# Lymphatus/caesium-clt

Measured on AMD Instinct MI355X. Metric: megapixels/sec JPEG q=80 1920x1080 batch, higher is better.
Workload: dtype int32

## Files before the change

caesium-clt_amd/binding.py:

```python
import ctypes as C
import os

_HERE = os.path.dirname(os.path.abspath(__file__))
NPHASES = 8
NKERNELS = 36
PHASE_NAMES = ["decode", "pixel", "masks_flags_runs", "stats_tables", "sizes_scan", "pack", "stuff_assemble", "reserved"]


class CCSParameters(C.Structure):
    _fields_ = [("keep_metadata", C.c_bool), ("jpeg_quality", C.c_uint32), ("jpeg_chroma_subsampling", C.c_uint32),
                ("jpeg_progressive", C.c_bool), ("jpeg_optimize", C.c_bool), ("jpeg_preserve_icc", C.c_bool),
                ("png_quality", C.c_uint32), ("png_optimization_level", C.c_uint32), ("png_force_zopfli", C.c_bool),
                ("png_optimize", C.c_bool), ("gif_quality", C.c_uint32), ("webp_quality", C.c_uint32), ("webp_lossless", C.c_bool),
                ("tiff_compression", C.c_uint32), ("tiff_deflate_level", C.c_uint32), ("width", C.c_uint32), ("height", C.c_uint32)]


class CCSResult(C.Structure):
    _fields_ = [("success", C.c_bool), ("code", C.c_uint32), ("error_message", C.c_char_p)]


class CByteArray(C.Structure):
    _fields_ = [("data", C.POINTER(C.c_uint8)), ("length", C.c_size_t)]


class Timing(C.Structure):
    _fields_ = [("total_ms", C.c_float), ("phase_ms", C.c_float * NPHASES), ("kernel_ms", C.c_float * NKERNELS), ("in_bytes", C.c_uint64), ("out_bytes", C.c_uint64),
                ("pixels", C.c_uint64), ("coef_bytes", C.c_uint64), ("n_images", C.c_uint32), ("n_failed", C.c_uint32), ("n_seq_decoded", C.c_uint32), ("n_par_fallback", C.c_uint32), ("n_par_short", C.c_uint32), ("n_prog_decoded", C.c_uint32), ("n_refine_chains", C.c_uint32), ("n_search_extra", C.c_uint32)]


class PngTiming(C.Structure):
    _fields_ = [("total_ms", C.c_float), ("kernel_ms", C.c_float * 16), ("in_bytes", C.c_uint64), ("out_bytes", C.c_uint64), ("pixels", C.c_uint64),
                ("raw_bytes", C.c_uint64), ("n_images", C.c_uint32), ("n_failed", C.c_uint32), ("n_trials", C.c_uint32)]


class CaesiumError(RuntimeError):
    def __init__(self, code, message):
        super().__init__(f"[{code}] {message}")
        self.code = code


def library_path():
    return os.path.join(_HERE, "libcaesium_hip.so")


EXPORTS = ["cs_default_parameters", "cs_compress_in_memory", "cs_compress_to_size_in_memory", "cs_convert_in_memory",
           "cs_batch_compress", "cs_batch_extent", "cs_free_bytes", "cs_free_result", "csh_device_count", "csh_last_error", "csh_kernel_name", "csh_kernel_name_webp", "csh_release_cached_memory", "csh_warmup", "csh_batch_create",
           "csh_batch_run", "csh_batch_fetch", "csh_batch_destroy", "csh_batch_retain_dct", "csh_batch_set_quality", "csh_batch_rerun_encode", "cs_batch_compress_to_size", "csh_batch_geometry", "csh_batch_read_coefs",
           "csp_kernel_name", "csp_batch_create", "csp_batch_create_webp", "csp_batch_create_pixels", "csh_batch_create_pixels", "csh_batch_pixels", "csh_batch_create_from_pixels", "csp_png_to_jpeg", "csp_png_to_lossless_webp", "csp_batch_run", "csp_batch_fetch", "csp_batch_destroy", "csp_batch_geometry", "csp_batch_read_rows", "csp_batch_read_stream",
           "csp_batch_trials", "csp_batch_read_scores", "csp_batch_chunk_bits", "csh_batch_create_webp", "cs_batch_convert",
           "cswd_batch_create", "cswd_batch_run", "cswd_batch_pixels", "cswd_batch_read_pixels", "cswd_batch_alpha", "cswd_batch_read_rgba", "cswd_batch_destroy", "cswd_rgba_join", "cswd_rgba_destroy", "csh_batch_create_webp_from_pixels", "csh_batch_create_from_pixels_rgb", "csl_encode_pixels", "csl_attach_alpha"]


def _declare(L):
    P = C.POINTER
    L.cs_default_parameters.argtypes = [P(CCSParameters)]
    L.cs_default_parameters.restype = None
    L.cs_compress_in_memory.argtypes = [C.c_char_p, C.c_size_t, P(CCSParameters), P(CByteArray)]
    L.cs_compress_in_memory.restype = CCSResult
    L.cs_compress_to_size_in_memory.argtypes = [C.c_char_p, C.c_size_t, P(CCSParameters), C.c_size_t, C.c_bool, P(CByteArray)]
    L.cs_compress_to_size_in_memory.restype = CCSResult
    L.cs_convert_in_memory.argtypes = [C.c_char_p, C.c_size_t, P(CCSParameters), C.c_uint32, P(CByteArray)]
    L.cs_convert_in_memory.restype = CCSResult
    L.cs_batch_compress.argtypes = [P(CByteArray), C.c_size_t, P(CCSParameters), C.c_int, P(CByteArray), P(CCSResult)]
    L.cs_batch_extent.argtypes = [P(CByteArray), C.c_size_t]
    L.cs_batch_extent.restype = C.c_size_t
    L.cs_free_bytes.argtypes = [P(CByteArray)]
    L.cs_free_bytes.restype = None
    L.cs_free_result.argtypes = [P(CCSResult)]
    L.cs_free_result.restype = None
    L.csh_last_error.restype = C.c_char_p
    L.csh_kernel_name.argtypes = [C.c_int]
    L.csh_kernel_name.restype = C.c_char_p
    L.csh_kernel_name_webp.argtypes = [C.c_int]
    L.csh_kernel_name_webp.restype = C.c_char_p
    L.csh_batch_create.argtypes = [P(CByteArray), C.c_size_t, P(CCSParameters), C.c_int, P(C.c_void_p)]
    L.csh_batch_run.argtypes = [C.c_void_p, P(Timing)]
    L.csh_batch_fetch.argtypes = [C.c_void_p, P(CByteArray), P(CCSResult)]
    L.csh_batch_retain_dct.argtypes = [C.c_void_p, C.c_int]
    L.csh_batch_set_quality.argtypes = [C.c_void_p, P(C.c_uint32)]
    L.csh_batch_rerun_encode.argtypes = [C.c_void_p, P(Timing)]
# ... 374 lines not shown
```

caesium-clt_amd/csrc/batch.hpp:

```cpp
#pragma once
#include <array>
#include <chrono>
#include <map>
#include <string>
#include <vector>

#include "../../include/caesium_hip.h"
#include "devmem.hpp"
#include "jpeg_host.hpp"
#include "kernels.h"
#include "webp_kernels.h"

namespace csh {

struct Item {
    int code = 0;
    std::string msg;
    JpegInfo in;
    JpegInfo out;
    int image = -1;
    size_t file_size = 0;
    std::vector<uint8_t> meta_out;
};

// ... 1 lines not shown
    PinnedBytes bits_pool;
    std::vector<DecScan> dscans;
    std::vector<DevHuffSet> hsets;
    std::vector<ParHuffSet> phsets;
    std::vector<char> phset_fits;
    std::vector<ParHuffSet4> phsets4;
    std::vector<std::array<int8_t, 8>> slot4;
    bool use4 = true;
    std::vector<ParScan> pscans;
    std::vector<uint32_t> need_seq_init;
    std::vector<ProgChain> chains;
    std::vector<int> chain_scans;
    std::vector<RefineUnit> refine_units;
    uint32_t refine_hist = 0, refine_pos = 0, refine_max_blocks = 0;
    uint32_t total_sub = 0, max_sub = 0, max_par_blocks = 0, dc_total = 0;

    DevBuf<uint8_t> d_bits, d_clean;
    DevBuf<ParScan> d_pscans;
    DevBuf<uint64_t> d_pstate, d_relax_list[2], d_unstuff_off, d_blk_off, d_dc_off;
    DevBuf<uint32_t> d_unstuff_cnt, d_nblk, d_need_seq, d_need_seq_init, d_relax_cnt, d_scan_pending, d_cut_block, d_claim;
    DevBuf<uint16_t> d_hyp;
    DevBuf<int32_t> d_dcdiff;
    DevBuf<DecScan> d_dscans;
    DevBuf<ProgChain> d_chains;
    DevBuf<int> d_chain_scans;
    DevBuf<uint64_t> d_refine_hist;
    DevBuf<uint32_t> d_refine_pos, d_refine_prog;
    DevBuf<RefineUnit> d_refine_units;
    DevBuf<DevHuffSet> d_hsets;
    DevBuf<ParHuffSet> d_phsets;
    DevBuf<ParHuffSet4> d_phsets4;
};

struct PixelPlan {
    std::vector<PlaneWork> pwork;
    std::vector<ResizeWork> rwork;
    std::vector<ResizeTap> rtaps;
    std::vector<float> rweights;
    uint64_t rgb_bytes = 0, tmp_floats = 0, max_tmp = 0, max_dst = 0;
    uint32_t max_row_in = 0, max_out_w = 0, max_nh = 0;
    uint32_t max_src_px = 0;
    uint64_t plane_bytes = 0, oplane_bytes = 0;
    uint32_t max_quads = 0;
    bool any_layout = false, any_layout_rgb = false;

    DevBuf<uint8_t> d_planes, d_oplanes, d_rgb;
    DevBuf<PlaneWork> d_pwork;
    DevBuf<ResizeWork> d_rwork;
    DevBuf<ResizeTap> d_rtaps;
    DevBuf<float> d_rweights, d_rtmp;
    DevBuf<int16_t> d_dct_raw;
};

struct Stage { uint32_t work0 = 0, nwork = 0, slot0 = 0, nslots = 0, ech0 = 0, nech = 0, table0 = 0, ntables = 0, plan0 = 0, nplans = 0, nzc0 = 0, nnzc = 0, ls0 = 0, nls = 0, ts0 = 0, nts = 0; };
struct SearchImg {
    int cand_work[64]; int ncand;
    int Al_luma = 0, Al_chroma = 0;
    uint64_t best_luma = 0, best_chroma = 0;
    int split_luma = 0, split_chroma = 0;
    bool luma_on = false, chroma_on = false;
};

struct EncodePlan {
    std::vector<EncScan> script;
    std::vector<ScanWork> swork;
    uint32_t nslots = 0, nlist_slots = 0, ntok_slots = 0;
    uint64_t total_corr = 0;
    uint64_t total_units = 0, total_words = 0;
    uint32_t max_units = 0;
    int ntables = 0;
    std::vector<TokPlan> plans;
    std::vector<int> plan_comp, plan_image;
    std::vector<EChunk> echunks;
    uint64_t tok_cap = 0;
    uint32_t tok_scale = 1;
    std::vector<TokRegion> regions;
    std::vector<uint32_t> region_est;
    uint32_t hist_rows = 0;
    std::vector<NzList> nzlists;
    std::vector<NzSet> nzsets;
    std::vector<int> nzset_of;
    std::vector<uint32_t> nzset_built;
    std::vector<int> nzset_comp, nzset_image;
    std::vector<NzChunk> nzchunks;
    std::vector<uint32_t> nz_est, nz_worst;
    uint32_t nz_nrec = 0;
    uint64_t nz_cap = 0;
    bool search = false;
    enum { ST_1 = 0, ST_1B = 1, ST_2 = 2, ST_2B = 3, ST_2C = 4, ST_N = 5 };
    Stage stage[ST_N];
    void stage_begin(Stage &sg) {
        sg.work0 = uint32_t(swork.size()); sg.slot0 = nslots; sg.ech0 = uint32_t(echunks.size()); sg.table0 = uint32_t(ntables); sg.plan0 = uint32_t(plans.size());
        sg.nzc0 = uint32_t(nzchunks.size()); sg.ls0 = nlist_slots; sg.ts0 = ntok_slots;
    }
    void stage_end(Stage &sg) {
        sg.nwork = uint32_t(swork.size()) - sg.work0; sg.nslots = nslots - sg.slot0; sg.nech = uint32_t(echunks.size()) - sg.ech0;
        sg.ntables = uint32_t(ntables) - sg.table0; sg.nplans = uint32_t(plans.size()) - sg.plan0;
        sg.nnzc = uint32_t(nzchunks.size()) - sg.nzc0; sg.nls = nlist_slots - sg.ls0; sg.nts = ntok_slots - sg.ts0;
    }
    std::vector<SearchImg> simg;
    std::vector<uint8_t> work_active;
    uint32_t n_gated_runs = 0;
    std::vector<uint32_t> img_list, img_nlist, h_cost;
    std::map<std::array<int, 5>, int> cand_script;
    std::vector<uint8_t> hdr_pool;
    std::vector<uint32_t> hdr_off;

    DevBuf<uint8_t> d_hdr, d_tail, d_scan_tmp, d_work_active;
    DevBuf<EncScan> d_script;
    DevBuf<ScanWork> d_swork;
    DevBuf<uint32_t> d_slot_work;
    DevBuf<EChunk> d_echunks;
    DevBuf<SlotRec> d_slots;
    DevBuf<TokPlan> d_plans;
    DevBuf<uint64_t> d_corr, d_symbits, d_eobbits, d_tok_off, d_chunk_off, d_scan_raw_off;
    DevBuf<uint32_t> d_tok_cursor;
    DevBuf<TokRegion> d_regions;
    DevBuf<uint16_t> d_eobrun, d_slot_hist;
    DevBuf<uint32_t> d_img_list, d_img_nlist, d_scan_cost, d_slot_raw, d_slot_eobh, d_long_runs, d_long_cnt, d_tokens, d_chunk_ntok, d_chunk_bits, d_raw, d_scan_pad, d_chunk_ff, d_hdr_off;
    DevBuf<DevEncTable> d_tables;
    DevBuf<NzList> d_nzlists;
    DevBuf<NzSet> d_nzsets;
    DevBuf<NzChunk> d_nzchunks;
    DevBuf<uint32_t> d_nz_pool, d_nz_cursor, d_nz_chunk_off, d_nz_chunk_cnt, d_list_slots, d_tok_slots;
};

struct TrellisPlan {
    bool trellis = false, dering = false;
    Stage tstage;
    std::vector<TrellisWork> twork;
    std::vector<TrellisRun> truns;
    uint32_t t_units = 0, t_max_rows = 0;
    std::vector<uint32_t> trows;
    bool t_sort = false;
    bool nz_once = false;

    DevBuf<TrellisWork> d_twork;
    DevBuf<TrellisRun> d_truns;
    DevBuf<uint32_t> d_tqueue, d_trows, d_tperm, d_tspill;
    DevBuf<uint8_t> d_tblk_cnt;
    DevBuf<uint16_t> d_tblk_off;
    DevBuf<uint64_t> d_tlambda, d_tdcbt;
};

struct WebpTail {
    uint32_t webp_mb_bytes = 768;
    std::vector<csw::WebpImg> wimgs;
    uint64_t wwork_bytes = 0, wlevels = 0;
    uint32_t wmax_luma = 0, wmax_mbh = 0;

    DevBuf<csw::WebpImg> d_wimgs;
    DevBuf<uint8_t> d_wwork, d_wscratch, d_wprobs, d_wupdate;
    DevBuf<uint32_t> d_wpart, d_wstats;
    DevBuf<int16_t> d_wlevels;
};

struct Outputs {
    uint64_t raw_bytes_cap = 0, out_cap = 0;
    DevBuf<uint8_t> d_out;
    DevBuf<uint64_t> d_img_off;
    DevBuf<uint32_t> d_img_size, d_img_size_pad, d_status, d_overflow;
    std::vector<uint32_t> h_img_size;
    std::vector<uint64_t> h_img_off;
    std::vector<uint32_t> h_status;
    bool ran = false;
};

}

struct csh_batch {
    int device = 0;
    hipStream_t stream = 0;
    bool have_stream = false;
    CCSParameters params;
    std::vector<csh::Item> items;
    int nimg = 0;
// ... 9 lines not shown
    std::vector<csh::ImgDesc> imgs;
    std::vector<csh::DevQuant> quants;
    uint32_t ntiles = 0, ntiles_in = 0, ntiles_out = 0, max_tiles = 0, max_dummy = 0;
    csh::DevBuf<csh::ImgDesc> d_imgs;
    csh::DevBuf<csh::DevQuant> d_quants;
    csh::DevBuf<int16_t> d_coef;

    csh::DecodePlan dec;
    csh::PixelPlan pix;
    csh::EncodePlan enc;
    csh::TrellisPlan tr;
    csh::WebpTail wp;
    csh::Outputs out;

    ~csh_batch() { if (have_stream) { (void)hipStreamSynchronize(stream); (void)hipStreamDestroy(stream); } }
};

namespace csh {

enum KernelSlot {
    KS_MEMSET_COEF, KS_UNSTUFF, KS_DEC_SPEC, KS_DEC_RELAX0, KS_DEC_RELAX, KS_DEC_WRITE, KS_DC_SCATTER, KS_REFINE_CHAINS, KS_DECODE_PROG_SEQ,
    KS_IDCT_PLANE, KS_RESIZE, KS_XFORM_DIRECT, KS_RESAMPLE_FDCT, KS_FIX_DUMMY, KS_MEMSET_ENC, KS_TRELLIS_STATS, KS_TRELLIS_AC, KS_TRELLIS_DC,
    KS_NZLIST, KS_TOKENS, KS_LIST_STATS, KS_AC_RUNS, KS_GEN_TABLES, KS_CHUNK_SIZES, KS_SCAN_CHUNK_BITS, KS_SCAN_LAYOUT, KS_PACK, KS_LIST_PACK,
    KS_FF_COUNT, KS_SCAN_SEARCH, KS_LAYOUT, KS_SCAN_IMAGES, KS_EMIT, KS_SPARE0, KS_SPARE1, KS_SPARE2, KS_COUNT,
    KS_WEBP_YUV = KS_XFORM_DIRECT, KS_WEBP_ENCODE = KS_RESAMPLE_FDCT, KS_WEBP_ASSEMBLE = KS_FIX_DUMMY
};
struct KernelSlotRow { KernelSlot slot; const char *name; int phase; };
constexpr KernelSlotRow kKernelSlots[] = {
    {KS_MEMSET_COEF, "memset_coef", 0},        {KS_UNSTUFF, "unstuff", 0},                 {KS_DEC_SPEC, "k_dec_spec", 0},
    {KS_DEC_RELAX0, "k_dec_relax0", 0},        {KS_DEC_RELAX, "k_dec_relax1_4", 0},        {KS_DEC_WRITE, "k_dec_write", 0},
    {KS_DC_SCATTER, "k_dc_scatter", 0},        {KS_REFINE_CHAINS, "k_refine_chains", 0},   {KS_DECODE_PROG_SEQ, "k_decode_prog+seq", 0},
    {KS_IDCT_PLANE, "k_idct_plane", 1},        {KS_RESIZE, "resize", 1},                   {KS_XFORM_DIRECT, "k_xform_direct", 1},
    {KS_RESAMPLE_FDCT, "k_resample+k_plane_fdct", 1}, {KS_FIX_DUMMY, "k_fix_dummy", 1},    {KS_MEMSET_ENC, "memset_enc", 2},
    {KS_TRELLIS_STATS, "trellis_stats", 1},    {KS_TRELLIS_AC, "k_trellis_ac", 1},         {KS_TRELLIS_DC, "k_trellis_dc", 1},
    {KS_NZLIST, "k_nzlist", 2},                {KS_TOKENS, "k_tokens", 2},                 {KS_LIST_STATS, "k_list_stats", 2},
    {KS_AC_RUNS, "k_ac_runs", 2},              {KS_GEN_TABLES, "k_gen_tables", 3},         {KS_CHUNK_SIZES, "k_chunk_sizes", 4},
    {KS_SCAN_CHUNK_BITS, "scan_chunk_bits", 4}, {KS_SCAN_LAYOUT, "scan_layout", 4},        {KS_PACK, "k_pack", 5},
    {KS_LIST_PACK, "k_list_pack", 5},          {KS_FF_COUNT, "k_ff_count", 6},             {KS_SCAN_SEARCH, "scan_search_stage2", 7},
    {KS_LAYOUT, "k_layout", 6},                {KS_SCAN_IMAGES, "scan_images", 6},         {KS_EMIT, "k_emit", 6},
    {KS_SPARE0, "", 7},                        {KS_SPARE1, "", 7},                         {KS_SPARE2, "", 7}};
constexpr bool kernel_slots_in_order() {
    for (int i = 0; i < int(sizeof kKernelSlots / sizeof kKernelSlots[0]); i++) if (kKernelSlots[i].slot != i) return false;
    return true;
}
static_assert(sizeof kKernelSlots / sizeof kKernelSlots[0] == CSH_NKERNELS && int(KS_COUNT) == int(CSH_NKERNELS), "one row per csh_timing.kernel_ms slot");
static_assert(kernel_slots_in_order(), "row i of kKernelSlots describes slot i");

struct PlanSwitches {
    std::string profile;
    bool nz_once = true;
    bool tr_sort = true;
    int prog_par = -1;
    bool fused_420 = true;
    static PlanSwitches read();
};

struct Laps {
    const bool trace;
    std::chrono::steady_clock::time_point at = std::chrono::steady_clock::now();
    std::string text;
    Laps();
    void lap(const char *what);
};

struct BatchPlanner {
    csh_batch *const b;
    const CByteArray *const inputs;
    const size_t count;
    const CCSParameters *const p;
    const csp_pixels *const px;
    const PlanSwitches sw;
    const bool progressive;
    uint16_t qout_nat[64];
    int script_base3 = 0, script_base1 = 0;
    std::vector<std::pair<std::vector<uint8_t>, int>> hset_keys;
    std::map<std::vector<uint16_t>, int> quant_index;
    uint64_t plane_off = 64, oplane_off = 0;

    BatchPlanner(csh_batch *b, const CByteArray *inputs, size_t count, const CCSParameters *p, const csp_pixels *px);
    void begin();
    void parse();
    int reserve_pinned();
    int plan_image(size_t n);
    int plan_search_stages();
    int plan_trellis();
    void finish_descriptors();
    int upload(Laps &laps);

private:
    void image_geometry(Item &it, ImgDesc &im);
    int decode_scans(Item &it, ImgDesc &im, const uint8_t *d);
    int huff_set(const JScan &js);
    void place_blocks(ParScan &ps, const JpegInfo &in, const JScan &js, uint32_t units, bool dc_rows, bool subseqs);
    int sequential_split(const Item &it, const ImgDesc &im, const uint8_t *d, int img_index, bool &par_ok);
    bool progressive_plan(const Item &it, const ImgDesc &im, int img_index);
    void plane_work(ImgDesc &im, const JpegInfo &in, const JpegInfo &o, int img_index, bool resized);
    void resize_work(const JpegInfo &in, const JpegInfo &o, int img_index);
    void output_scans(Item &it, ImgDesc &im, int img_index, size_t in_len);
    void frame_header(Item &it);
    template <class Fill> int enc_scan(const std::array<int, 5> &key, Fill fill);
    int cand_index(int comp, int Ss, int Se, int Ah, int Al);
    int dc_scan_index(int ncomp);
    int seq1_index(int comp);
    uint32_t nz_list(int img_index, int comp, int Al, const ImgDesc &im, size_t in_len);
    void add_works(Item &it, ImgDesc &im, int img_index, const std::vector<int> &list, size_t in_len, const JpegInfo &o, bool stats_only = false);
    template <class Make> void add_stage(int sid, Make make);
// ... 14 lines not shown
```

caesium-clt_amd/csrc/batch_plan.cpp:

```cpp
#include <algorithm>
#include <atomic>
#include <cmath>
#include <thread>

#include "batch.hpp"
#include "resize_host.h"

namespace csh {

static void build_dev_huff(const HuffSpec &h, DevHuff &d) {
    memset(&d, 0, sizeof d);
    for (int l = 0; l < 18; l++) d.maxcode[l] = -1;
    if (!h.present) return;
    int code = 0, p = 0;
    for (int l = 1; l <= 16; l++) {
        if (h.bits[l]) {
            d.valptr[l] = p - code;
            for (int i = 0; i < h.bits[l]; i++, p++, code++)
                if (l <= 9) {
                    int base = code << (9 - l);
                    for (int k = 0; k < (1 << (9 - l)); k++) d.look[(base + k) & 511] = uint16_t((l << 8) | h.vals[p]);
                }
            d.maxcode[l] = code - 1;
        }
// ... 139 lines not shown
    if (lossless) {
        for (int c = 0; c < in.ncomp; c++) o.comp[c] = in.comp[c];
        jpeg_geometry(o);
        return 0;
    }
    int ss = int(p.jpeg_chroma_subsampling);
    if (ss == 0) ss = 420;
    for (int c = 0; c < in.ncomp; c++) { o.comp[c].id = c + 1; o.comp[c].h = o.comp[c].v = 1; o.comp[c].tq = c ? 1 : 0; }
    if (in.ncomp == 3) {
        int blocks = 0;
        for (int c = 0; c < 3; c++) {
            const JComp &k = in.comp[c];
            blocks += k.h * k.v;
            if (in.hmax % k.h || in.vmax % k.v) { it.msg = "fractional chroma sampling ratio (component factors do not divide the largest ones)"; return CS_ERR_JPEG_FEATURE; }
            if (in.hmax / k.h > 4 || in.vmax / k.v > 4) { it.msg = "chroma sampling ratio above 4"; return CS_ERR_JPEG_FEATURE; }
        }
        if (blocks > 10) { it.msg = "more than 10 blocks per MCU"; return CS_ERR_JPEG_FEATURE; }
        if (ss == 420) { o.comp[0].h = 2; o.comp[0].v = 2; }
        else if (ss == 422) { o.comp[0].h = 2; o.comp[0].v = 1; }
        else if (ss == 411) { o.comp[0].h = 4; o.comp[0].v = 1; }
        else if (ss != 444) { it.msg = "unknown output chroma subsampling"; return CS_ERR_JPEG_FEATURE; }
    }
    jpeg_geometry(o);
    return 0;
}

void layout_token_pool(csh_batch *b) {
    b->enc.regions.resize(b->enc.region_est.size());
    if (b->test_pool_shift < 0) b->test_pool_shift = getenv("CSH_TEST_POOL_SHIFT") ? std::min(16, std::max(0, atoi(getenv("CSH_TEST_POOL_SHIFT")))) : 0;
    const int shift = b->test_pool_shift;
    uint64_t at = 0;
    for (size_t i = 0; i < b->enc.regions.size(); i++) {
        const uint64_t cap = std::min<uint64_t>(std::max<uint64_t>((uint64_t(b->enc.region_est[i]) * b->enc.tok_scale) >> shift, 64), 0xFFFFFFF0ull);
        b->enc.regions[i].base = at; b->enc.regions[i].cap = uint32_t(cap); b->enc.regions[i].pad = 0;
        at += (cap + 3) & ~uint64_t(3);
    }
    b->enc.tok_cap = at + 64;
    at = 0;
    for (size_t i = 0; i < b->enc.nzlists.size(); i++) {
        const uint64_t cap = std::min<uint64_t>(std::max<uint64_t>((uint64_t(b->enc.nz_est[i]) * b->enc.tok_scale) >> shift, 64), b->enc.nz_worst[i]);
        b->enc.nzlists[i].base = at; b->enc.nzlists[i].cap = uint32_t(cap);
        at += (cap + 3) & ~uint64_t(3);
    }
    b->enc.nz_cap = at + 64;
}

PlanSwitches PlanSwitches::read() {
    auto is = [](const char *name, const char *v) { const char *e = getenv(name); return e && !strcmp(e, v); };
    PlanSwitches s;
    const char *penv = getenv("CSH_PROFILE");
    s.profile = penv && *penv ? penv : "mozjpeg";
    s.nz_once = !is("CSH_NZ_ONCE", "0");
    s.tr_sort = !is("CSH_TR_SORT", "0");
    const char *pp = getenv("CSH_PROG_PAR");
    s.prog_par = pp && !strcmp(pp, "0") ? 0 : (pp && !strcmp(pp, "1") ? 1 : -1);
    s.fused_420 = !getenv("CSH_NO_FUSED_420");
    return s;
}

Laps::Laps() : trace(getenv("CSH_TRACE") != nullptr) {}
void Laps::lap(const char *what) {
    if (!trace) return;
    const auto now = std::chrono::steady_clock::now();
    char buf[64];
    snprintf(buf, sizeof buf, " %s %.1f", what, std::chrono::duration<double, std::milli>(now - at).count());
    text += buf; at = now;
}

BatchPlanner::BatchPlanner(csh_batch *b_, const CByteArray *inputs_, size_t count_, const CCSParameters *p_, const csp_pixels *px_)
    : b(b_), inputs(inputs_), count(count_), p(p_), px(px_), sw(PlanSwitches::read()), progressive(p_->jpeg_progressive) {}

void BatchPlanner::begin() {
    b->items.resize(count);
    quality_table(int(p->jpeg_quality), qout_nat);
    DevQuant qo; make_quant(qout_nat, qo);
    b->quants.push_back(qo);
    b->q_base = int(b->quants.size()) - 1;
    for (int q = 1; q <= 100; q++) { uint16_t tq[64]; quality_table(q, tq); DevQuant dq; make_quant(tq, dq); b->quants.push_back(dq); }
    b->progressive = progressive;

    add_script(b->enc.script, 3, true);
    add_script(b->enc.script, 1, true);
    add_script(b->enc.script, 3, false);
    add_script(b->enc.script, 1, false);
    script_base3 = progressive ? 0 : 16; script_base1 = progressive ? 10 : 17;
    const bool webp = b->webp, rgb_out = b->rgb_out;
    const std::string &profile = sw.profile;
    b->enc.search = progressive && !webp && !rgb_out && profile != "plain";
    const bool lossy_jpeg = !b->lossless && !webp && !rgb_out;
    b->tr.trellis = lossy_jpeg && (profile == "mozjpeg" || profile == "mozjpeg-trellis");
    b->tr.dering = lossy_jpeg && (profile == "mozjpeg" || profile == "mozjpeg-dering");
    b->tr.nz_once = b->tr.trellis && progressive && sw.nz_once && sw.tr_sort;
}

template <class Fill>
int BatchPlanner::enc_scan(const std::array<int, 5> &key, Fill fill) {
    auto f = b->enc.cand_script.find(key);
    if (f != b->enc.cand_script.end()) return f->second;
    EncScan e;
    memset(&e, 0, sizeof e);
    fill(e);
    b->enc.script.push_back(e);
    return b->enc.cand_script[key] = int(b->enc.script.size()) - 1;
}
int BatchPlanner::cand_index(int comp, int Ss, int Se, int Ah, int Al) {
    return enc_scan({comp, Ss, Se, Ah, Al}, [&](EncScan &e) {
// ... 379 lines not shown
bool BatchPlanner::progressive_plan(const Item &it, const ImgDesc &im, int img_index) {
    const JpegInfo &in = it.in;
    bool prog_ok = in.progressive && in.restart_interval == 0;
    for (size_t s = 0; s < in.scans.size(); s++) {
        const JScan &js = in.scans[s];
        if (js.has_marker || js.data_len >= (1u << 28) || !b->dec.phset_fits[b->dec.dscans[im.first_scan + s].huff_set]) prog_ok = false;
    }
    if (!prog_ok) return false;
    const bool par_first = regular_progression(in) && sw.prog_par != 0 && uint64_t(in.mcus_x) * uint64_t(in.mcus_y) * 10 < (1u << 24);
    for (size_t s = 0; s < in.scans.size(); s++) {
        const JScan &js = in.scans[s];
        DecScan &ds = b->dec.dscans[im.first_scan + s];
        ParScan ps;
        memset(&ps, 0, sizeof ps);
        ps.bits_off = ds.bits_off; ps.bits_len = ds.bits_len; ps.huff_set = ds.huff_set; ps.image = img_index; ps.ncomp = ds.ncomp; ps.nb_mcu = 1;
        ps.Ss = js.Ss; ps.Se = js.Se; ps.Al = js.Al;
        ps.kind = !par_first ? CSH_PS_UNSTUFF : js.Ss == 0 ? (js.Ah == 0 ? CSH_PS_DC_FIRST : CSH_PS_DC_REFINE) : (js.Ah == 0 ? CSH_PS_AC_FIRST : CSH_PS_UNSTUFF);
        ps.sub_base = b->dec.total_sub; ps.par_index = uint32_t(b->dec.pscans.size());
        if (ps.kind != CSH_PS_UNSTUFF) place_blocks(ps, in, js, scan_units(in, js), ps.kind == CSH_PS_DC_FIRST, ps.kind != CSH_PS_DC_REFINE);
        ds.par_index = int(b->dec.pscans.size());
        b->dec.pscans.push_back(ps);
    }
    const bool refine_split = par_first && sw.prog_par != 1;
    for (int chain = 0; chain <= in.ncomp; chain++) {
        ProgChain pc;
        memset(&pc, 0, sizeof pc);
        pc.image = img_index; pc.first = int(b->dec.chain_scans.size());
        bool all_refine = chain != 0;
        for (size_t s = 0; s < in.scans.size(); s++) {
            const JScan &js = in.scans[s];
            const bool mine = chain == 0 ? js.Ss == 0 : (js.Ss != 0 && js.comp_idx[0] == chain - 1);
            if (mine && b->dec.pscans[size_t(b->dec.dscans[im.first_scan + s].par_index)].kind == CSH_PS_UNSTUFF) {
                b->dec.chain_scans.push_back(im.first_scan + int(s)); pc.count++;
                if (js.Ah == 0 || js.data_len >= (1u << 27)) all_refine = false;
            }
        }
        if (pc.count && refine_split && all_refine) {
            const JComp &jc = in.comp[chain - 1];
            const uint64_t nblocks = uint64_t(jc.real_bw) * uint64_t(jc.real_bh);
            if (nblocks && uint64_t(b->dec.refine_pos) + nblocks * uint64_t(pc.count) < (1ull << 32)) {
                pc.refine = 1; pc.comp = chain - 1; pc.nblocks = uint32_t(nblocks);
                pc.hist_off = b->dec.refine_hist; pc.pos_off = b->dec.refine_pos;
                b->dec.refine_hist += pc.nblocks; b->dec.refine_pos += pc.nblocks * uint32_t(pc.count);
                b->dec.refine_max_blocks = std::max(b->dec.refine_max_blocks, pc.nblocks);
            }
        }
        if (pc.count) b->dec.chains.push_back(pc);
    }
    return true;
}

void BatchPlanner::plane_work(ImgDesc &im, const JpegInfo &in, const JpegInfo &o, int img_index, bool resized) {
    for (int c = 0; c < in.ncomp; c++) {
        PlaneWork w; w.image = img_index; w.comp = c;
        w.up = resized ? up_desc(1, 1, 0) : up_desc(in.hmax / in.comp[c].h, in.vmax / in.comp[c].v, in.comp[c].comp_w);
        w.dn = dn_kind(o.hmax / o.comp[c].h, o.vmax / o.comp[c].v);
        const int in_kind = (w.up.hx == 1 && w.up.vx == 1) ? 0 : (w.up.hx == 2 && w.up.vx == 2) ? 1 : (w.up.hx == 2 && w.up.vx == 1) ? 2 : -1;
        if (in_kind < 0 || w.dn == CSH_DN_H4V1) w.mode = CSH_MODE_ANY;
        else if (resized) w.mode = 1 + w.dn;
        else w.mode = (in_kind == 0 && w.dn == CSH_DN_FULL) ? 0 : 1 + 3 * in_kind + w.dn;
        if (w.mode == CSH_MODE_ANY) b->pix.any_layout = true;
        const bool fused = w.mode == 5 && !resized && im.in[c].comp_w > 2 && im.in[c].real_bw == im.out[c].real_bw && im.in[c].real_bh == im.out[c].real_bh &&
                           im.in[c].comp_w == im.out[c].comp_w && im.in[c].comp_h == im.out[c].comp_h && sw.fused_420;
        if (fused) w.mode = 10;
        if (w.mode) {
            im.plane_off[c] = plane_off;
            plane_off += uint64_t(im.in[c].real_bw * 8) * uint64_t(im.in[c].real_bh * 8);
            plane_off = (plane_off + 63u) & ~uint64_t(63);
            im.splane_off[c] = im.plane_off[c];
            if (resized) {
                JComp full; full.h = full.v = 1;
                JpegInfo tmpj; tmpj.width = o.width; tmpj.height = o.height; tmpj.ncomp = 1; tmpj.comp[0] = full; jpeg_geometry(tmpj);
                uint32_t dummy = 0; fill_geom(tmpj.comp[0], im.src[c], dummy);
                im.splane_off[c] = plane_off;
                plane_off += uint64_t(im.src[c].real_bw * 8) * uint64_t(im.src[c].real_bh * 8);
                plane_off = (plane_off + 63u) & ~uint64_t(63);
            }
            im.oplane_off[c] = oplane_off;
            const uint64_t osz = fused ? 0 : uint64_t(im.out[c].real_bw) * 8 * uint64_t(im.out[c].real_bh) * 8;
            oplane_off = (oplane_off + osz + 63u) & ~uint64_t(63);
            b->pix.max_quads = std::max(b->pix.max_quads, uint32_t(osz / 4));
        }
        b->pix.pwork.push_back(w);
    }
}

void BatchPlanner::resize_work(const JpegInfo &in, const JpegInfo &o, int img_index) {
    ResizeWork rw;
    memset(&rw, 0, sizeof rw);
    rw.image = img_index; rw.nw = o.width; rw.nh = o.height;
    rw.in_kind = in.ncomp == 1 ? 0 : ((in.comp[1].h == in.hmax && in.comp[1].v == in.vmax) ? 0 : (in.comp[1].v == in.vmax ? 2 : 1));
    for (int c = 0; c < in.ncomp; c++) rw.up[c] = up_desc(in.hmax / in.comp[c].h, in.vmax / in.comp[c].v, in.comp[c].comp_w);
    if (in.ncomp == 3) {
        auto same = [&](int c, int hx, int vx) { return rw.up[c].hx == hx && rw.up[c].vx == vx; };
        const bool legacy = same(0, 1, 1) && rw.up[1].hx == rw.up[2].hx && rw.up[1].vx == rw.up[2].vx &&
                            (same(1, 1, 1) || same(1, 2, 2) || same(1, 2, 1));
        if (!legacy) { rw.in_kind = CSH_RZ_ANY; b->pix.any_layout_rgb = true; }
    }
    if (px) rw.in_kind = -1;
    const uint64_t src_bytes = uint64_t(in.width) * in.height * in.ncomp, dst_bytes = uint64_t(o.width) * o.height * in.ncomp;
    rw.rgb_src_off = b->pix.rgb_bytes; b->pix.rgb_bytes += (src_bytes + 63) & ~uint64_t(63);
    rw.rgb_dst_off = b->pix.rgb_bytes; b->pix.rgb_bytes += (dst_bytes + 63) & ~uint64_t(63);
    const uint64_t tmpn = uint64_t(o.height) * in.width * in.ncomp;
    rw.tmp_off = b->pix.tmp_floats; b->pix.tmp_floats += tmpn;
    const bool same = o.width == in.width && o.height == in.height;
    rw.vtap_base = uint32_t(b->pix.rtaps.size()); csh_lanczos_axis(in.height, o.height, same, b->pix.rtaps, b->pix.rweights);
    rw.htap_base = uint32_t(b->pix.rtaps.size()); csh_lanczos_axis(in.width, o.width, same, b->pix.rtaps, b->pix.rweights);
// ... 164 lines not shown
        if (it.image < 0) continue;
        ImgDesc &im = b->imgs[size_t(it.image)];
        std::vector<int> list;
        for (int c = 0; c < im.ncomp; c++) list.push_back(progressive ? cand_index(c, 1, 63, 0, 0) : seq1_index(c));
        const size_t first = b->enc.swork.size();
        add_works(it, im, it.image, list, inputs[n].length, it.out, true);
        for (int c = 0; c < im.ncomp; c++) {
            const ScanWork &w = b->enc.swork[first + size_t(c)];
            TrellisWork tw;
            memset(&tw, 0, sizeof tw);
            tw.image = it.image; tw.comp = c;
            tw.table_ac = w.table_base + (progressive ? 0u : 1u);
            tw.table_dc = progressive ? -1 : int32_t(w.table_base);
            tw.nunits = w.nunits; tw.unit_base = b->tr.t_units;
            b->tr.t_units += w.nunits;
            b->tr.t_max_rows = std::max<uint32_t>(b->tr.t_max_rows, uint32_t((im.out[c].real_bh + im.out[c].v - 1) / im.out[c].v));
            tw.nzset = 0xFFFFFFFFu;
            if (progressive) {
                const int si = b->enc.nzset_of[size_t(it.image) * CSH_MAX_COMPS + size_t(c)];
                b->enc.nzsets[size_t(si)].cnt_base = tw.unit_base;
                if (b->tr.nz_once) tw.nzset = uint32_t(si);
            }
            b->tr.twork.push_back(tw);
        }
    }
    b->enc.stage_end(tg);
    {
        std::vector<uint32_t> nch(b->tr.twork.size());
        uint32_t most = 0;
        for (size_t wi = 0; wi < b->tr.twork.size(); wi++) { nch[wi] = (b->tr.twork[wi].nunits + CSH_TR_WG - 1) / CSH_TR_WG; most = std::max(most, nch[wi]); }
        for (uint32_t j = 0; j < most; j += CSH_TR_RUN)
            for (size_t wi = 0; wi < b->tr.twork.size(); wi++)
                if (j < nch[wi]) b->tr.truns.push_back(TrellisRun{uint32_t(wi), j, std::min<uint32_t>(CSH_TR_RUN, nch[wi] - j)});
    }
    {
        b->tr.t_sort = progressive && sw.tr_sort;
        std::vector<std::pair<uint32_t, uint32_t>> rows;
        for (size_t wi = 0; wi < b->tr.twork.size(); wi++) {
            const CompGeom &g = b->imgs[size_t(b->tr.twork[wi].image)].out[b->tr.twork[wi].comp];
            for (int r = 0; r < (g.real_bh + g.v - 1) / g.v; r++) rows.push_back({uint32_t(g.real_bw * g.v), uint32_t(wi << 16) | uint32_t(r)});
        }
        std::stable_sort(rows.begin(), rows.end(), [](const auto &a, const auto &b2) { return a.first > b2.first; });
        for (const auto &r : rows) b->tr.trows.push_back(r.second);
    }
    if (b->enc.total_units > 0xFFFFFFF0ull) { csh_set_error("csh_batch_create: batch too large (fewer files per batch)"); return CS_ERR_POOL_OVERFLOW; }
    return 0;
}

void BatchPlanner::finish_descriptors() {
    if (!b->lossless)
        for (ImgDesc &im : b->imgs) for (int c = 0; c < im.ncomp; c++) im.out[c].tile_base += b->ntiles_in;
    for (size_t i = 0; i < b->enc.plans.size(); i++) b->enc.plans[i].tile_base = b->imgs[size_t(b->enc.plan_image[i])].out[b->enc.plan_comp[i]].tile_base;
    for (size_t i = 0; i < b->enc.nzsets.size(); i++) b->enc.nzsets[i].tile_base = b->imgs[size_t(b->enc.nzset_image[i])].out[b->enc.nzset_comp[i]].tile_base;
    for (ParScan &ps : b->dec.pscans)
        for (int m = 0; m < ps.nb_mcu && m < 10; m++) {
            int dcs = ps.dct[m] & 3, acs = 4 + (ps.act[m] & 3);
            if (b->dec.use4) { dcs = std::max<int>(0, b->dec.slot4[ps.huff_set][dcs]); acs = std::max<int>(0, b->dec.slot4[ps.huff_set][acs]); }
            ps.sel |= uint64_t(dcs | (acs << 3)) << (6 * m);
        }
    {
        std::vector<int> last(b->dec.chains.size(), -1);
        for (int s = 0;; s++) {
            bool any = false;
            for (size_t c = 0; c < b->dec.chains.size(); c++)
                if (b->dec.chains[c].refine && b->dec.chains[c].count > s) {
                    RefineUnit u; u.chain = int(c); u.s = s; u.prev = last[c];
                    last[c] = int(b->dec.refine_units.size());
                    b->dec.refine_units.push_back(u);
                    any = true;
                }
            if (!any) break;
        }
    }
    b->ntiles = b->ntiles_in + b->ntiles_out;
    b->pix.plane_bytes = plane_off;
    b->pix.oplane_bytes = oplane_off;
    b->out.out_cap = b->out.raw_bytes_cap;
    layout_token_pool(b);
}

int BatchPlanner::upload(Laps &laps) {
    hipStream_t st = b->stream;
    if (!b->nimg) return 0;
    b->dec.bits_pool.flush_copies();
    laps.lap("copy_in");
    if (b->dec.d_bits.alloc(b->dec.bits_pool.size()) || (b->dec.bits_pool.size() && hipMemcpyAsync(b->dec.d_bits.p, b->dec.bits_pool.p, b->dec.bits_pool.size(), hipMemcpyHostToDevice, st) != hipSuccess) ||
        b->d_imgs.upload(b->imgs, st) || b->dec.d_dscans.upload(b->dec.dscans, st) || b->dec.d_chains.upload(b->dec.chains, st) || b->dec.d_chain_scans.upload(b->dec.chain_scans, st) ||
        b->dec.d_hsets.upload(b->dec.hsets, st) || b->dec.d_phsets.upload(b->dec.phsets, st) || (b->dec.use4 && b->dec.d_phsets4.upload(b->dec.phsets4, st)) || b->d_quants.upload(b->quants, st) || b->pix.d_pwork.upload(b->pix.pwork, st) ||
        b->enc.d_script.upload(b->enc.script, st) || b->enc.d_swork.upload(b->enc.swork, st) || b->enc.d_slot_work.alloc(size_t(b->enc.nslots) + 1) || b->enc.d_slots.alloc(size_t(b->enc.nslots) + 1) || b->enc.d_plans.upload(b->enc.plans, st) || b->enc.d_echunks.upload(b->enc.echunks, st) || b->enc.d_hdr.upload(b->enc.hdr_pool, st) ||
        b->enc.d_hdr_off.upload(b->enc.hdr_off, st) || b->dec.d_pscans.upload(b->dec.pscans, st) || b->pix.d_rwork.upload(b->pix.rwork, st) || b->pix.d_rtaps.upload(b->pix.rtaps, st) ||
        b->pix.d_rweights.upload(b->pix.rweights, st) || b->pix.d_rgb.alloc(b->pix.rgb_bytes + 64) || b->pix.d_rtmp.alloc((resize_is_fused(b->pix.max_row_in) ? 0 : b->pix.tmp_floats) + 16) || b->dec.d_need_seq_init.upload(b->dec.need_seq_init, st))
        return CS_ERR_NO_DEVICE;
    size_t nchunks = b->dec.bits_pool.size() / 64 + 1, nst = size_t(b->dec.total_sub) + b->dec.pscans.size() + 1;
    if (b->dec.d_clean.alloc(b->dec.bits_pool.size() + 64) || b->dec.d_unstuff_cnt.alloc(nchunks + 1) || b->dec.d_unstuff_off.alloc(nchunks + 2) ||
        b->dec.d_pstate.alloc(nst) || b->dec.d_relax_list[0].alloc(nst) || b->dec.d_relax_list[1].alloc(nst) || b->dec.d_relax_cnt.alloc(512) || b->dec.d_scan_pending.alloc(b->dec.pscans.size() + 1) || b->dec.d_cut_block.alloc(b->dec.pscans.size() + 1) || b->dec.d_claim.alloc(size_t(b->dec.total_sub) + 1) || b->dec.d_hyp.alloc((size_t(b->dec.total_sub) + 1) * 10) ||
        b->dec.d_nblk.alloc(size_t(b->dec.total_sub) + 1) || b->dec.d_blk_off.alloc(size_t(b->dec.total_sub) + 2) || b->dec.d_need_seq.alloc(b->nimg + 1) ||
        b->dec.d_dcdiff.alloc(size_t(b->dec.dc_total) + 1) || b->dec.d_dc_off.alloc(size_t(b->dec.dc_total) + 2) ||
        b->dec.d_refine_hist.alloc(size_t(b->dec.refine_hist) + 1) || b->dec.d_refine_pos.alloc(size_t(b->dec.refine_pos) + 1) || b->dec.d_refine_units.upload(b->dec.refine_units, st) ||
        b->dec.d_refine_prog.alloc(b->dec.refine_units.size() + 1))
        return CS_ERR_NO_DEVICE;
    if (b->d_coef.alloc(size_t(b->ntiles) * CSH_TILE_I16) || b->pix.d_planes.alloc(b->pix.plane_bytes + 64) || b->pix.d_oplanes.alloc(b->pix.oplane_bytes + 64) ||
        b->enc.d_symbits.alloc(b->enc.total_words + 1) || b->enc.d_eobbits.alloc(b->enc.total_words + 1) ||
        b->enc.d_long_runs.alloc(2 * (b->enc.total_units / 512 + b->enc.swork.size() + 16)) || b->enc.d_long_cnt.alloc(4) || b->enc.d_tail.alloc(b->enc.total_units + 1) || b->enc.d_eobrun.alloc(b->enc.total_units + 1) || b->enc.d_corr.alloc(b->enc.total_corr + 1) ||
        b->enc.d_tok_off.alloc(4 * size_t(b->enc.nslots) + 4) || b->enc.d_chunk_ntok.alloc(4 * size_t(b->enc.nslots) + 4) || b->enc.d_slot_hist.alloc(size_t(b->enc.hist_rows) * 256 + 256) ||
        b->enc.d_slot_raw.alloc(size_t(b->enc.nslots) + 1) || b->enc.d_img_list.upload(b->enc.img_list, st) || b->enc.d_img_nlist.upload(b->enc.img_nlist, st) || b->enc.d_scan_cost.alloc(b->enc.swork.size() + 1) || b->enc.d_slot_eobh.alloc(16 * size_t(b->enc.nslots) + 16) || b->enc.d_chunk_bits.alloc(size_t(b->enc.nslots) + 1) || b->enc.d_chunk_off.alloc(size_t(b->enc.nslots) + 2) || b->enc.d_tok_cursor.alloc(b->enc.region_est.size() + 1) || b->enc.d_regions.upload(b->enc.regions, st) ||
        b->enc.d_tables.alloc(b->enc.ntables) || b->enc.d_scan_pad.alloc(b->enc.swork.size() + 1) ||
        b->enc.d_nzlists.upload(b->enc.nzlists, st) || b->enc.d_nzsets.upload(b->enc.nzsets, st) || b->enc.d_nzchunks.upload(b->enc.nzchunks, st) || b->enc.d_list_slots.alloc(size_t(b->enc.nlist_slots) + 1) || b->enc.d_tok_slots.alloc(size_t(b->enc.ntok_slots) + 1) ||
        b->enc.d_nz_cursor.alloc(b->enc.nzlists.size() + 1) || b->enc.d_nz_chunk_off.alloc(size_t(b->enc.nz_nrec) + 1) || b->enc.d_nz_chunk_cnt.alloc(size_t(b->enc.nz_nrec) + 1) ||
        b->enc.d_scan_raw_off.alloc(b->enc.swork.size() + 2) || b->out.d_img_size.alloc(b->nimg + 1) || b->out.d_img_size_pad.alloc(b->nimg + 1) ||
        b->out.d_img_off.alloc(b->nimg + 2) || b->out.d_status.alloc(b->nimg) || b->out.d_overflow.alloc(4))
        return CS_ERR_NO_DEVICE;
    if (hipMemsetAsync(b->enc.d_slots.p, 0, (size_t(b->enc.nslots) + 1) * sizeof(SlotRec), st) != hipSuccess ||
        hipMemsetAsync(b->enc.d_slot_work.p, 0, (size_t(b->enc.nslots) + 1) * sizeof(uint32_t), st) != hipSuccess) { csh_set_error("hipMemsetAsync failed"); return CS_ERR_NO_DEVICE; }
    launch_make_slots(st, b->enc.d_swork.p, uint32_t(b->enc.swork.size()), b->enc.d_script.p, b->enc.d_nzlists.p, b->enc.d_slots.p, b->enc.d_slot_work.p, b->enc.d_list_slots.p, b->enc.d_tok_slots.p);
    if (b->tr.trellis && (b->tr.d_trows.upload(b->tr.trows, st) || (b->tr.t_sort && (b->tr.d_tperm.alloc(size_t(b->tr.t_units) + 1) || b->tr.d_tblk_cnt.alloc(size_t(b->tr.t_units) + 1) || (b->tr.nz_once && b->tr.d_tblk_off.alloc(size_t(b->tr.t_units) + 1)))))) return CS_ERR_NO_DEVICE;
    if (b->tr.trellis && (b->tr.d_twork.upload(b->tr.twork, st) || b->tr.d_truns.upload(b->tr.truns, st) || b->tr.d_tqueue.alloc(1) || b->tr.d_tlambda.alloc(size_t(b->tr.t_units) + 1) || b->tr.d_tdcbt.alloc(size_t(b->tr.t_units) + 1) ||
                       b->tr.d_tspill.alloc(trellis_spill_words(trellis_ac_slots())) || b->pix.d_dct_raw.alloc(size_t(b->ntiles_out) * CSH_TILE_I16)))
        return CS_ERR_NO_DEVICE;
    for (size_t n = 0; px && n < count; n++) {
        const Item &it = b->items[n];
        if (it.image < 0) continue;
        const ResizeWork &rw = b->pix.rwork[size_t(it.image)];
        if (rw.image != it.image) { csh_set_error("internal: resize work out of order"); return CS_ERR_NO_DEVICE; }
        if (hipMemcpyAsync(b->pix.d_rgb.p + rw.rgb_src_off, px[n].device_pixels, size_t(px[n].width) * px[n].height * px[n].channels, hipMemcpyDeviceToDevice, st) != hipSuccess) { csh_set_error("pixel copy failed"); return CS_ERR_NO_DEVICE; }
    }
    laps.lap("alloc+enqueue");
    if (hipStreamSynchronize(st) != hipSuccess) { csh_set_error("upload failed"); return CS_ERR_NO_DEVICE; }
    laps.lap("upload_wait");
    return 0;
}

}
```

caesium-clt_amd/csrc/batch_run.cpp:

```cpp
#include <algorithm>

#include "batch.hpp"

namespace csh {
namespace {

class KernelMarks {
    hipEvent_t ev[CSH_NKERNELS + 1];
    int created = 0, next = 0;
    const hipStream_t st;

public:
    explicit KernelMarks(hipStream_t s) : st(s) {}
    KernelMarks(const KernelMarks &) = delete;
    KernelMarks &operator=(const KernelMarks &) = delete;
    ~KernelMarks() { for (int i = 0; i < created; i++) (void)hipEventDestroy(ev[i]); }
    int start() {
        for (; created <= CSH_NKERNELS; created++) CSH_CHECK(hipEventCreate(&ev[created]));
        CSH_CHECK(hipEventRecord(ev[0], st));
        return 0;
    }
    int claim(KernelSlot slot, hipEvent_t *e) {
        if (int(slot) != next || next >= CSH_NKERNELS) {
            csh_set_error("internal: timing mark '%s' out of order (slot %d is next)", slot < KS_COUNT ? kKernelSlots[slot].name : "?", next);
            return -1;
        }
        *e = ev[++next];
        return 0;
    }
    int mark(KernelSlot slot) {
        hipEvent_t e;
        if (claim(slot, &e)) return -1;
        CSH_CHECK(hipEventRecord(e, st));
        return 0;
    }
    int skip_to(KernelSlot slot) {
        while (next < int(slot)) if (mark(KernelSlot(next))) return -1;
        return int(slot) == next ? 0 : mark(slot);
    }
    int read(csh_timing *t, bool phases) const {
        if (phases) {
            for (int i = 0; i < CSH_NPHASES; i++) t->phase_ms[i] = 0;
            for (int i = 0; i < CSH_NKERNELS; i++) t->kernel_ms[i] = 0;
        }
        for (int i = 0; i < next; i++) {
            CSH_CHECK(hipEventElapsedTime(&t->kernel_ms[i], ev[i], ev[i + 1]));
            if (phases) t->phase_ms[kKernelSlots[i].phase] += t->kernel_ms[i];
        }
        CSH_CHECK(hipEventElapsedTime(&t->total_ms, ev[0], ev[next]));
        return 0;
    }
};
#define MARK(slot) do { if (marks.mark(slot)) return -1; } while (0)

struct Run {
    csh_batch *const b;
    csh_timing *const t;
    const hipStream_t st;
    const int nimg;
    KernelMarks marks;
    uint64_t raw_chunks = 0;
    bool eobrun_cleared = false;
    EncCtx c;
    AsmCtx a;

    Run(csh_batch *b_, csh_timing *t_) : b(b_), t(t_), st(b_->stream), nimg(b_->nimg), marks(b_->stream) {}

    int pools() {
        raw_chunks = (b->out.raw_bytes_cap + 63) / 64;
        if (b->enc.d_raw.n != raw_chunks * 16) {
            if (b->enc.d_raw.alloc(raw_chunks * 16) || b->enc.d_chunk_ff.alloc(raw_chunks + 1) || b->out.d_out.alloc(b->out.out_cap + 64))
                return -1;
            const uint64_t longest = std::max({uint64_t(size_t(b->enc.nslots)), uint64_t(b->enc.swork.size()), uint64_t(b->dec.dc_total), uint64_t(b->dec.total_sub), uint64_t(b->dec.bits_pool.size() / 64), uint64_t(nimg)});
            size_t tmp = exclusive_scan_tmp_bytes(longest + 1);
            if (b->enc.d_scan_tmp.alloc(tmp)) return -1;
        }
        if (b->enc.d_tokens.n < b->enc.tok_cap && b->enc.d_tokens.alloc(b->enc.tok_cap)) return -1;
        if (b->enc.d_nz_pool.n < b->enc.nz_cap && b->enc.d_nz_pool.alloc(b->enc.nz_cap)) return -1;
        return 0;
    }

    int requant() {
        if (b->out.d_status.zero(st) || b->out.d_overflow.zero(st)) return -1;
        launch_requant(st, b->d_imgs.p, b->pix.d_pwork.p, int(b->pix.pwork.size()), b->max_tiles, b->d_quants.p, b->pix.d_dct_raw.p, b->ntiles_in, b->d_coef.p);
        launch_fix_dummy(st, b->d_imgs.p, nimg, b->max_dummy, b->d_coef.p);
        return marks.skip_to(KS_MEMSET_ENC);
    }
    int skip_decode() {
        if (b->out.d_status.zero(st) || b->out.d_overflow.zero(st)) return -1;
        return marks.skip_to(KS_IDCT_PLANE);
    }

    int decode() {
        const bool zero_in_spec = !b->dec.pscans.empty() && b->dec.max_sub != 0;
        if (!zero_in_spec) CSH_CHECK(hipMemsetAsync(b->d_coef.p, 0, size_t(b->ntiles_in) * CSH_TILE_I16 * sizeof(int16_t), st));
        if (b->out.d_status.zero(st) || b->out.d_overflow.zero(st)) return -1;
        CSH_CHECK(hipMemcpyAsync(b->dec.d_need_seq.p, b->dec.d_need_seq_init.p, size_t(nimg) * sizeof(uint32_t), hipMemcpyDeviceToDevice, st));
        MARK(KS_MEMSET_COEF);
        {
            int nps = int(b->dec.pscans.size());
            uint32_t nchunks = uint32_t(b->dec.bits_pool.size() / 64);
            if (nps) {
                launch_unstuff_count(st, b->dec.d_bits.p, b->dec.d_pscans.p, nps, nchunks, b->dec.d_unstuff_cnt.p);
                launch_exclusive_scan(st, b->dec.d_unstuff_cnt.p, b->dec.d_unstuff_off.p, nchunks, b->enc.d_scan_tmp.p, b->enc.d_scan_tmp.n);
                launch_unstuff_copy(st, b->dec.d_bits.p, b->dec.d_clean.p, b->dec.d_pscans.p, nps, nchunks, b->dec.d_unstuff_off.p);
            }
            MARK(KS_UNSTUFF);
            DenseArgs da;
            memset(&da, 0, sizeof da);
            da.clean = b->dec.d_clean.p; da.pss = b->dec.d_pscans.p; da.huffs = b->dec.use4 ? static_cast<const void *>(b->dec.d_phsets4.p) : static_cast<const void *>(b->dec.d_phsets.p); da.compact = b->dec.use4 ? 1 : 0; da.state = b->dec.d_pstate.p; da.nblk = b->dec.d_nblk.p;
            da.list_out = b->dec.d_relax_list[0].p; da.cnt_out = b->dec.d_relax_cnt.p; da.blk_off = b->dec.d_blk_off.p; da.imgs = b->d_imgs.p;
            da.coef = b->d_coef.p; da.dcdiff = b->dec.d_dcdiff.p; da.need_seq = b->dec.d_need_seq.p; da.cut_block = b->dec.d_cut_block.p;
            CSH_CHECK(hipMemsetAsync(b->dec.d_cut_block.p, 0xFF, b->dec.d_cut_block.n * sizeof(uint32_t), st));
            const uint64_t zero_all = uint64_t(b->ntiles_in) * CSH_TILE_I16 * sizeof(int16_t), zero_half = (zero_all / 2) & ~uint64_t(15);
            const uint64_t eob_all = (uint64_t(b->enc.d_eobrun.n) * sizeof(uint16_t)) & ~uint64_t(15), eob_half = (eob_all / 2) & ~uint64_t(15);
// ... 11 lines not shown
            }
            launch_dec_dense(st, 1, nps, b->dec.max_sub, da);
            da.zero_bytes = 0; da.zero2_bytes = 0;
            MARK(KS_DEC_RELAX0);
            const int kMaxRounds = int(b->dec.d_relax_cnt.n) - 2;
            int R = 0;
            for (int group = 12; nps && R < kMaxRounds; group = 8) {
                for (int g = 0; g < group && R < kMaxRounds; g++, R++)
                    launch_dec_relax_list(st, b->dec.d_clean.p, b->dec.d_pscans.p, b->dec.total_sub, da.huffs, da.compact, b->dec.d_pstate.p, b->dec.d_nblk.p, b->dec.d_relax_list[R & 1].p,
                                          b->dec.d_relax_cnt.p + R, b->dec.d_relax_list[(R & 1) ^ 1].p, b->dec.d_relax_cnt.p + R + 1, b->dec.d_pstate.n, b->dec.d_claim.p, uint32_t(R + 1));
                uint32_t left = 0;
                CSH_CHECK(hipMemcpyAsync(&left, b->dec.d_relax_cnt.p + R, sizeof left, hipMemcpyDeviceToHost, st));
                CSH_CHECK(hipStreamSynchronize(st));
                if (!left) break;
            }
            if (nps) {
                if (b->dec.d_scan_pending.zero(st)) return -1;
                launch_dec_mark_pending(st, b->dec.d_pscans.p, b->dec.total_sub, b->dec.d_relax_list[R & 1].p, b->dec.d_relax_cnt.p + R, b->dec.d_scan_pending.p);
                da.hyp = b->dec.d_hyp.p; da.scan_pending = b->dec.d_scan_pending.p;
                launch_dec_dense(st, 3, nps, b->dec.max_sub, da);
                launch_dec_chain(st, b->dec.d_pscans.p, nps, b->dec.d_pstate.p, b->dec.d_nblk.p, b->dec.d_hyp.p, b->dec.d_scan_pending.p, b->dec.d_need_seq.p);
            }
            MARK(KS_DEC_RELAX);
            if (nps) launch_exclusive_scan(st, b->dec.d_nblk.p, b->dec.d_blk_off.p, b->dec.total_sub, b->enc.d_scan_tmp.p, b->enc.d_scan_tmp.n);
            launch_dec_dense(st, 2, nps, b->dec.max_sub, da);
            MARK(KS_DEC_WRITE);
            if (nps) launch_exclusive_scan(st, reinterpret_cast<uint32_t *>(b->dec.d_dcdiff.p), b->dec.d_dc_off.p, b->dec.dc_total, b->enc.d_scan_tmp.p, b->enc.d_scan_tmp.n);
            launch_dc_scatter(st, b->dec.d_pscans.p, nps, b->dec.max_par_blocks, b->d_imgs.p, b->dec.d_dc_off.p, b->d_coef.p, b->dec.d_need_seq.p, b->dec.d_cut_block.p);
            launch_dc_refine(st, b->dec.d_clean.p, b->dec.d_pscans.p, nps, b->dec.max_par_blocks, b->d_imgs.p, b->d_coef.p, b->dec.d_need_seq.p);
            MARK(KS_DC_SCATTER);
        }
        launch_refine_chains(st, b->dec.d_clean.p, b->dec.d_pscans.p, b->dec.d_phsets.p, b->dec.d_dscans.p, b->dec.d_chains.p, b->dec.d_chain_scans.p, int(b->dec.chains.size()), b->dec.d_refine_units.p,
                             int(b->dec.refine_units.size()), b->dec.refine_max_blocks, b->d_imgs.p, b->d_coef.p, b->dec.d_need_seq.p, b->dec.d_refine_hist.p, b->dec.d_refine_pos.p, b->dec.d_refine_prog.p);
        MARK(KS_REFINE_CHAINS);
        launch_decode_prog(st, b->dec.d_clean.p, b->dec.d_pscans.p, b->dec.d_phsets.p, b->dec.d_dscans.p, b->dec.d_chains.p, b->dec.d_chain_scans.p, int(b->dec.chains.size()), b->d_imgs.p,
                           b->d_coef.p, b->dec.d_need_seq.p);
        launch_decode_seq(st, b->dec.d_bits.p, b->d_imgs.p, b->dec.d_dscans.p, b->dec.d_hsets.p, b->d_coef.p, nimg, b->dec.d_need_seq.p);
        MARK(KS_DECODE_PROG_SEQ);
        return 0;
    }

    int planes() {
        int nw = b->lossless ? 0 : int(b->pix.pwork.size());
        launch_idct_plane(st, b->d_imgs.p, b->pix.d_pwork.p, nw, b->max_tiles, b->d_quants.p, b->d_coef.p, b->pix.d_planes.p);
        MARK(KS_IDCT_PLANE);
        launch_resize(st, b->d_imgs.p, b->pix.d_rwork.p, int(b->pix.rwork.size()), b->pix.d_rtaps.p, b->pix.d_rweights.p, b->pix.d_planes.p, b->pix.d_rgb.p, b->pix.d_rtmp.p,
                      b->pix.max_src_px, b->pix.max_tmp, b->pix.max_dst, b->pix.max_row_in, b->pix.max_out_w, b->pix.max_nh, !(b->webp || b->rgb_out), b->pix.any_layout_rgb);
        MARK(KS_RESIZE);
        return 0;
    }
    int pixels() {
        const int nw = b->lossless ? 0 : int(b->pix.pwork.size());
        int16_t *rawp = ((b->retain_dct || b->tr.trellis) && !b->lossless) ? b->pix.d_dct_raw.p : nullptr;
        launch_xform_direct(st, b->d_imgs.p, b->pix.d_pwork.p, nw, b->max_tiles, b->d_quants.p, b->d_coef.p, b->d_coef.p, rawp, b->ntiles_in, b->tr.dering);
        MARK(KS_XFORM_DIRECT);
        launch_resample_plane(st, b->d_imgs.p, b->pix.d_pwork.p, nw, b->pix.max_quads, b->pix.d_planes.p, b->pix.d_oplanes.p);
        if (b->pix.any_layout) launch_resample_any(st, b->d_imgs.p, b->pix.d_pwork.p, nw, b->pix.max_quads, b->pix.d_planes.p, b->pix.d_oplanes.p);
        launch_plane_fdct(st, b->d_imgs.p, b->pix.d_pwork.p, nw, b->max_tiles, b->d_quants.p, b->pix.d_oplanes.p, b->d_coef.p, rawp, b->ntiles_in, b->tr.dering);
        launch_resample_fdct_420(st, b->d_imgs.p, b->pix.d_pwork.p, nw, b->max_tiles, b->d_quants.p, b->pix.d_planes.p, b->d_coef.p, rawp, b->ntiles_in, b->tr.dering);
        MARK(KS_RESAMPLE_FDCT);
        if (!b->lossless) launch_fix_dummy(st, b->d_imgs.p, nimg, b->max_dummy, b->d_coef.p);
        MARK(KS_FIX_DUMMY);
        return 0;
    }

    void fill_enc_ctx() {
        memset(&c, 0, sizeof c);
        c.imgs = b->d_imgs.p; c.script = b->enc.d_script.p; c.work = b->enc.d_swork.p; c.nwork = int(b->enc.swork.size());
        c.echunks = b->enc.d_echunks.p; c.plans = b->enc.d_plans.p; c.nechunks = uint32_t(b->enc.echunks.size()); c.slot_work = b->enc.d_slot_work.p; c.slots = b->enc.d_slots.p; c.nslots = b->enc.nslots;
        c.coef = b->d_coef.p; c.sym_bits = b->enc.d_symbits.p; c.eob_bits = b->enc.d_eobbits.p; c.tail = b->enc.d_tail.p;
        c.eobrun = b->enc.d_eobrun.p; c.long_runs = b->enc.d_long_runs.p; c.long_cnt = b->enc.d_long_cnt.p; c.corr = b->enc.d_corr.p;
        c.tokens = b->enc.d_tokens.p; c.regions = b->enc.d_regions.p; c.tok_cursor = b->enc.d_tok_cursor.p; c.tok_off = b->enc.d_tok_off.p; c.chunk_ntok = b->enc.d_chunk_ntok.p; c.slot_hist = b->enc.d_slot_hist.p; c.slot_raw = b->enc.d_slot_raw.p; c.slot_eobh = b->enc.d_slot_eobh.p;
        c.chunk_bits = b->enc.d_chunk_bits.p; c.chunk_off = b->enc.d_chunk_off.p; c.tables = b->enc.d_tables.p;
        c.raw = b->enc.d_raw.p; c.raw_words = raw_chunks * 16; c.status = b->out.d_status.p; c.overflow = b->out.d_overflow.p;
        c.nzlists = b->enc.d_nzlists.p; c.nzsets = b->enc.d_nzsets.p; c.nz_pool = b->enc.d_nz_pool.p; c.nz_cursor = b->enc.d_nz_cursor.p; c.nz_chunk_off = b->enc.d_nz_chunk_off.p; c.nz_chunk_cnt = b->enc.d_nz_chunk_cnt.p;
        c.debug = getenv("CSH_DEBUG") ? uint32_t(atoi(getenv("CSH_DEBUG"))) : 0u;
    }
    void fill_asm_ctx() {
        memset(&a, 0, sizeof a);
        a.imgs = b->d_imgs.p; a.script = b->enc.d_script.p; a.work = b->enc.d_swork.p; a.nimg = nimg;
        a.nwork = b->tr.trellis ? int(b->tr.tstage.work0) : c.nwork;
        a.tables = b->enc.d_tables.p; a.chunk_off = b->enc.d_chunk_off.p; a.scan_pad_bytes = b->enc.d_scan_pad.p; a.scan_raw_off = b->enc.d_scan_raw_off.p;
        a.raw = b->enc.d_raw.p; a.raw_chunks = raw_chunks; a.chunk_ff = b->enc.d_chunk_ff.p;
        a.hdr_pool = b->enc.d_hdr.p; a.hdr_off = b->enc.d_hdr_off.p; a.img_size = b->out.d_img_size.p; a.img_size_pad = b->out.d_img_size_pad.p;
        a.img_off = b->out.d_img_off.p; a.out = b->out.d_out.p; a.out_cap = b->out.out_cap; a.status = b->out.d_status.p; a.overflow = b->out.d_overflow.p;
        a.img_list = b->enc.d_img_list.p; a.img_nlist = b->enc.d_img_nlist.p; a.scan_cost = b->enc.d_scan_cost.p;
    }
    void fill_trellis_ctx(TrellisCtx &tc) {
        memset(&tc, 0, sizeof tc);
        tc.imgs = b->d_imgs.p; tc.quant = b->d_quants.p; tc.work = b->tr.d_twork.p; tc.nwork = int(b->tr.twork.size()); tc.runs = b->tr.d_truns.p; tc.nruns = uint32_t(b->tr.truns.size());
        tc.tables = b->enc.d_tables.p; tc.raw = b->pix.d_dct_raw.p; tc.raw_tile0 = b->ntiles_in; tc.coef = b->d_coef.p; tc.dcrec = b->tr.d_tlambda.p; tc.dcbt = b->tr.d_tdcbt.p;
        tc.spill = b->tr.d_tspill.p; tc.nslots = uint32_t(b->tr.d_tspill.n / trellis_spill_words(1)); tc.max_rows = b->tr.t_max_rows;
        tc.queue = b->tr.d_tqueue.p;
        tc.rows = b->tr.d_trows.p; tc.nrows = uint32_t(b->tr.trows.size());
        if (b->tr.t_sort) { tc.blk_cnt = b->tr.d_tblk_cnt.p; tc.perm = b->tr.d_tperm.p; }
        if (b->tr.t_sort && b->tr.nz_once) {
            tc.nz_pool = b->enc.d_nz_pool.p; tc.nzlists = b->enc.d_nzlists.p; tc.nzsets = b->enc.d_nzsets.p; tc.nz_chunk_off = b->enc.d_nz_chunk_off.p; tc.nz_chunk_cnt = b->enc.d_nz_chunk_cnt.p;
            tc.blk_off = b->tr.d_tblk_off.p;
        }
        tc.debug = getenv("CSH_TR_DEBUG") ? uint32_t(atoi(getenv("CSH_TR_DEBUG"))) : 0u;
    }

    int encode_begin() {
        fill_enc_ctx();
        launch_reset_works(st, b->enc.d_swork.p, c.nwork);
        if (b->enc.d_nz_cursor.zero(st) || b->enc.d_nz_chunk_cnt.zero(st)) return -1;
        if (b->enc.d_symbits.zero(st) || b->enc.d_eobbits.zero(st) || (!eobrun_cleared && b->enc.d_eobrun.zero(st)) || b->enc.d_tables.zero(st) || b->enc.d_tok_cursor.zero(st) || b->enc.d_slot_eobh.zero(st) || b->enc.d_scan_pad.zero(st)) return -1;
#ifdef CSH_EMUL
        if (b->enc.d_raw.zero(st)) return -1;
#else
        if ((c.debug & 8192u) && b->enc.d_raw.zero(st)) return -1;
#endif
        MARK(KS_MEMSET_ENC);
        return 0;
    }

    void set_stage(const Stage &sg) {
        c.echunks = b->enc.d_echunks.p + sg.ech0; c.nechunks = sg.nech; c.slot0 = sg.slot0; c.nslots = sg.nslots;
        c.nzchunks = b->enc.d_nzchunks.p + sg.nzc0; c.nnzchunks = sg.nnzc;
        c.list_slots = b->enc.d_list_slots.p + sg.ls0; c.nlist_slots = sg.nls; c.tok_slots = b->enc.d_tok_slots.p + sg.ts0; c.ntok_slots = sg.nts;
    }

    int trellis() {
        const Stage &tg = b->tr.tstage;
        set_stage(tg);
        c.stats_only = 1;
        if (b->enc.d_long_cnt.zero(st)) return -1;
        c.nz_blk_cnt = b->tr.t_sort ? b->tr.d_tblk_cnt.p : nullptr;
        c.nz_blk_off = (b->tr.t_sort && b->tr.nz_once) ? b->tr.d_tblk_off.p : nullptr;
        launch_nzlist(st, c);
        c.nz_blk_cnt = nullptr; c.nz_blk_off = nullptr;
        if (b->tr.t_sort) {
            TrellisCtx ts;
            memset(&ts, 0, sizeof ts);
            ts.work = b->tr.d_twork.p; ts.nwork = int(b->tr.twork.size()); ts.blk_cnt = b->tr.d_tblk_cnt.p; ts.perm = b->tr.d_tperm.p;
            launch_trellis_sort(st, ts);
        }
        launch_tokens(st, c);
        launch_list_stats(st, c);
        launch_ac_runs(st, c);
        launch_gen_tables(st, b->enc.d_tables.p + tg.table0, int(tg.ntables));
        c.stats_only = 0;
        if (b->enc.d_nz_cursor.zero(st)) return -1;
        MARK(KS_TRELLIS_STATS);
        TrellisCtx tc;
        fill_trellis_ctx(tc);
        if (b->tr.d_tqueue.zero(st)) return -1;
        launch_trellis_ac(st, tc);
        MARK(KS_TRELLIS_AC);
        launch_trellis_dc(st, tc);
        launch_fix_dummy(st, b->d_imgs.p, nimg, b->max_dummy, b->d_coef.p);
        MARK(KS_TRELLIS_DC);
        return 0;
    }

    int stage(const Stage &sg, bool mark, bool gate) {
#define SMARK(slot) do { if (mark) MARK(slot); } while (0)
        set_stage(sg);
        c.work_active = gate ? b->enc.d_work_active.p : nullptr;
        a.work0 = int(sg.work0); a.nwork_run = int(sg.nwork);
        if (b->enc.d_long_cnt.zero(st)) return -1;
        launch_nzlist(st, c);
        SMARK(KS_NZLIST);
        launch_tokens(st, c);
        SMARK(KS_TOKENS);
        launch_list_stats(st, c);
        SMARK(KS_LIST_STATS);
        launch_ac_runs(st, c);
        SMARK(KS_AC_RUNS);
        launch_gen_tables(st, b->enc.d_tables.p + sg.table0, int(sg.ntables));
        SMARK(KS_GEN_TABLES);
        launch_chunk_sizes(st, c);
// ... 40 lines not shown
        MARK(KS_LAYOUT);
        launch_exclusive_scan(st, b->out.d_img_size_pad.p, b->out.d_img_off.p, uint64_t(nimg), b->enc.d_scan_tmp.p, b->enc.d_scan_tmp.n);
        MARK(KS_SCAN_IMAGES);
        launch_emit(st, a);
        MARK(KS_EMIT);
        return 0;
    }

    int finish(bool phases) {
        CSH_CHECK(hipStreamSynchronize(st));
        CSH_CHECK(hipGetLastError());
        if (t && marks.read(t, phases)) return -1;
        if (t && !phases) t->n_images = uint32_t(nimg);
        return 0;
    }

    int webp() {
        const int nwimg = int(b->wp.wimgs.size());
        uint64_t out_bytes = 0;
        std::vector<uint64_t> off(size_t(b->nimg) + 1, 0);
        for (auto &wi : b->wp.wimgs) {
            const uint64_t cap = 4096 + uint64_t(wi.mbw) * wi.mbh * (b->wp.webp_mb_bytes + 2);
            wi.out_cap = uint32_t(std::min<uint64_t>(cap, 0xFFFFFF00u)); wi.out_off = out_bytes;
            off[wi.image] = out_bytes;
            out_bytes += (wi.out_cap + 63) & ~uint64_t(63);
            const int q = int(b->params.webp_quality);
            wi.quality = q < 0 ? 0 : q > 100 ? 100 : q;
        }
        off[b->nimg] = out_bytes;
        if (b->out.d_out.n < out_bytes + 64 && b->out.d_out.alloc(out_bytes + 64)) return -1;
        if ((b->wp.d_wscratch.n < out_bytes + 64 && b->wp.d_wscratch.alloc(out_bytes + 64)) || (b->wp.d_wpart.n < size_t(b->nimg) * 9 + 9 && b->wp.d_wpart.alloc(size_t(b->nimg) * 9 + 9)) ||
            (b->wp.d_wstats.n < size_t(b->nimg) * 2112 + 8 && (b->wp.d_wstats.alloc(size_t(b->nimg) * 2112 + 8) || b->wp.d_wprobs.alloc(size_t(b->nimg) * 1056 + 8) || b->wp.d_wupdate.alloc(size_t(b->nimg) * 1056 + 8))))
            return -1;
        if (b->wp.d_wstats.zero(st)) return -1;
        if (b->wp.d_wimgs.upload(b->wp.wimgs, st) || (b->wp.d_wwork.n < b->wp.wwork_bytes + 64 && b->wp.d_wwork.alloc(b->wp.wwork_bytes + 64)) ||
            (b->wp.d_wlevels.n < b->wp.wlevels + 64 && b->wp.d_wlevels.alloc(b->wp.wlevels + 64)))
            return -1;
        CSH_CHECK(hipMemcpyAsync(b->out.d_img_off.p, off.data(), off.size() * sizeof(uint64_t), hipMemcpyHostToDevice, st));
        if (b->out.d_img_size.zero(st)) return -1;
        csw::launch_webp_yuv(st, b->wp.d_wimgs.p, nwimg, b->wp.wmax_luma, b->pix.d_rgb.p, b->wp.d_wwork.p);
        MARK(KS_WEBP_YUV);
        hipEvent_t mid;
        if (marks.claim(KS_WEBP_ENCODE, &mid)) return -1;
        if (csw::launch_webp_encode(st, b->wp.wimgs.data(), nwimg, b->wp.d_wimgs.p, b->wp.d_wwork.p, b->wp.d_wlevels.p, b->wp.d_wscratch.p, b->wp.d_wpart.p, b->out.d_out.p, b->out.d_img_size.p, b->out.d_status.p, mid)) return -1;
        MARK(KS_WEBP_ASSEMBLE);
        return finish(false);
    }
};

}

int run_once(csh_batch *b, csh_timing *t, bool requant_only) {
    Run r(b, t);
    if (r.pools() || r.marks.start()) return -1;
    const bool from_pixels = requant_only && b->tr.dering;
    if (requant_only && !from_pixels) {
        if (r.requant()) return -1;
    } else {
        if (from_pixels ? r.skip_decode() : r.decode()) return -1;
        if (r.planes()) return -1;
        if (b->webp) return r.webp();
        if (b->rgb_out) return (r.marks.mark(KS_XFORM_DIRECT) || r.finish(false)) ? -1 : 0;
        if (r.pixels()) return -1;
    }
    if (r.encode_begin()) return -1;
    if (b->tr.trellis ? r.trellis() : r.marks.skip_to(KS_NZLIST)) return -1;
    r.fill_asm_ctx();
    if (r.stage(b->enc.stage[0], true, false)) return -1;
    if (b->enc.search && r.search()) return -1;
    return (r.emit() || r.finish(true)) ? -1 : 0;
}

}
```

caesium-clt_amd/csrc/k_aclist.hip:

```cpp
#include "kernels.h"
#include "wave.h"

namespace csh {

#define CSH_LP_WORDS 1024

__device__ __forceinline__ static uint32_t lbitlen(uint32_t v) { return 32u - uint32_t(__clz(v)); }
__device__ __forceinline__ static int lwave() { return int(threadIdx.x) / CSP_WAVE_THREADS; }

#define CSH_NZ_HALF 16
__device__ __forceinline__ static uint4 nz_load(const EncCtx &c, const NzSet &S, uint32_t u, int bx, int by, uint32_t oct) {
    uint4 q; q.x = q.y = q.z = q.w = 0u;
    if (u < S.nunits) {
        const int b = by * S.bw + bx;
        q = *reinterpret_cast<const uint4 *>(c.coef + (size_t(S.tile_base) + size_t(b >> 6)) * CSH_TILE_I16 + size_t((b & 63) * CSH_BLK_STRIDE) + size_t(oct) * CSH_OCT_STRIDE);
    }
    return q;
}
__device__ __forceinline__ static uint32_t nz_mask8(const uint4 &q, uint32_t oct) {
    uint32_t m = 0;
    m |= (q.x & 0xFFFFu) ? 1u : 0u;   m |= (q.x >> 16) ? 2u : 0u;
    m |= (q.y & 0xFFFFu) ? 4u : 0u;   m |= (q.y >> 16) ? 8u : 0u;
    m |= (q.z & 0xFFFFu) ? 16u : 0u;  m |= (q.z >> 16) ? 32u : 0u;
    m |= (q.w & 0xFFFFu) ? 64u : 0u;  m |= (q.w >> 16) ? 128u : 0u;
// ... 340 lines not shown
                } else if (ev.term) {
                    const uint32_t run = eobrun[ev.blk];
                    if (run) {
                        const uint32_t nb = lbitlen(run) - 1u, t = lut[nb << 4];
                        v[q] = ((t & 0xFFFFu) << nb) | (run & ((1u << nb) - 1u)); n[q] = (t >> 16) + nb;
                    }
                }
                ln += n[q];
            }
            v0[l] = v[0]; v1[l] = v[1]; v2[l] = v[2]; v3[l] = v[3]; n0[l] = n[0]; n1[l] = n[1]; n2[l] = n[2]; n3[l] = n[3]; z[l] = zz; len[l] = ln;
        }
        uint32_t tot;
        const LV<uint32_t> ex = lscan(len, tot);
        LFOR(l) {
            uint64_t at = pos + ex[l] - uint64_t(ww) * 32u;
            const uint32_t v[4] = {v0[l], v1[l], v2[l], v3[l]}, n[4] = {n0[l], n1[l], n2[l], n3[l]};
            CSH_UNROLL
            for (int q = 0; q < 4; q++) {
                for (uint32_t t = (z[l] >> (2 * q)) & 3u; t; t--) { lor_bits(buf, at, zc, zl); at += zl; }
                if (n[q]) { lor_bits(buf, at, v[q], n[q]); at += n[q]; }
            }
        }
        pos += tot;
        const uint32_t done = uint32_t(pos >> 5) - ww;
        if (done > CSH_LP_WORDS - 640) {
            CSP_WAVE_SYNC();
            LFOR(l) for (uint32_t q = uint32_t(l); q < done; q += 64) {
                const uint32_t v = buf[q];
                if (first_flush && q == 0) { if (v) atomicOr(out + ww, v); } else out[ww + q] = v;
            }
            const uint32_t partial = buf[done];
            CSP_WAVE_SYNC();
            LFOR(l) for (int q = l; q < CSH_LP_WORDS; q += 64) buf[q] = (q == 0) ? partial : 0u;
            CSP_WAVE_SYNC();
            ww += done; first_flush = false;
        }
    }
    CSP_WAVE_SYNC();
    const uint32_t last = uint32_t((pos + 31) >> 5) - ww;
    LFOR(l) for (uint32_t q = uint32_t(l); q < last; q += 64) {
        const uint32_t v = buf[q];
        if ((first_flush && q == 0) || q == last - 1) { if (v) atomicOr(out + ww + q, v); } else out[ww + q] = v;
    }
}

__global__ void k_reset_works(ScanWork *work, int nwork) {
    const int j = int(blockIdx.x * blockDim.x + threadIdx.x);
    if (j >= nwork) return;
    work[j].out_off = 0xFFFFFFFFu; work[j].raw_bytes = 0; work[j].hdr_bytes = 0; work[j].ff_bytes = 0; work[j].no_room = 0;
}

void launch_nzlist(hipStream_t st, const EncCtx &c) {
    if (!c.nnzchunks) return;
    CSH_LAUNCH_PHASED(k_nzlist, 3, dim3(c.nnzchunks), dim3(2 * CSP_WAVE_THREADS), st, c);
    CSH_LAUNCH(k_nzfilter, dim3(c.nnzchunks), dim3(CSP_WAVE_THREADS), st, c);
}
void launch_list_stats(hipStream_t st, const EncCtx &c) { if (c.nlist_slots) CSH_LAUNCH(k_list_stats, dim3((c.nlist_slots + 3) / 4), dim3(4 * CSP_WAVE_THREADS), st, c); }
void launch_list_pack(hipStream_t st, const EncCtx &c) { if (c.nlist_slots) CSH_LAUNCH(k_list_pack, dim3((c.nlist_slots + 3) / 4), dim3(4 * CSP_WAVE_THREADS), st, c); }
__global__ void __launch_bounds__(64) k_make_slots(const ScanWork *works, uint32_t nworks, const EncScan *script, const NzList *nzlists, SlotRec *slots, uint32_t *slot_work, uint32_t *list_slots,
                                                   uint32_t *tok_slots) {
    const uint32_t wi = blockIdx.x;
    if (wi >= nworks) return;
    const ScanWork &w = works[wi];
    const EncScan &e = script[w.scan];
    const uint32_t nch = (w.nunits + 255u) / 256u;
    const bool prog_ac = e.Ss > 0 && !e.sequential, listed = w.list != 0xFFFFFFFFu;
    for (uint32_t j = threadIdx.x; j < nch; j += blockDim.x) {
        SlotRec r;
        r.work = wi; r.j = j; r.nch = nch; r.first_chunk = w.first_chunk; r.unit0 = w.unit_base + 256u * j;
        r.nun = w.nunits - 256u * j < 256u ? w.nunits - 256u * j : 256u; r.table_base = w.table_base; r.ntables = uint16_t(e.ntables);
        r.flags = uint16_t((prog_ac ? 1 : 0) | (prog_ac && e.Ah ? 2 : 0) | (listed ? 4 : 0));
        r.hist_row = w.hist_row0 + j * uint32_t(e.ntables);
        r.word_base = w.word_base; r.unit_base = w.unit_base; r.nunits_work = w.nunits;
        r.Ss = uint8_t(e.Ss); r.Se = uint8_t(e.Se); r.Ah = uint8_t(e.Ah); r.Al = uint8_t(e.Al); r.corr0 = w.corr_base == 0xFFFFFFFFu ? 0u : w.corr_base + 256u * j;
        r.nzlist = listed ? w.list : 0u; r.nzrec = listed ? nzlists[w.list].chunk0 + j : 0u;
        slots[w.first_chunk + j] = r;
        slot_work[w.first_chunk + j] = wi;
        (listed ? list_slots : tok_slots)[w.ls_base + j] = w.first_chunk + j;
    }
}
__global__ void __launch_bounds__(64) k_rebind_slots(const ScanWork *works, uint32_t nworks, const NzList *nzlists, SlotRec *slots) {
    const uint32_t wi = blockIdx.x;
    if (wi >= nworks) return;
    const ScanWork &w = works[wi];
    if (w.list == 0xFFFFFFFFu) return;
    const uint32_t nch = (w.nunits + 255u) / 256u, chunk0 = nzlists[w.list].chunk0;
    for (uint32_t j = threadIdx.x; j < nch; j += blockDim.x) { slots[w.first_chunk + j].nzlist = w.list; slots[w.first_chunk + j].nzrec = chunk0 + j; }
}
void launch_rebind_slots(hipStream_t st, const ScanWork *works, uint32_t nworks, const NzList *nzlists, SlotRec *slots) {
    if (nworks) CSH_LAUNCH(k_rebind_slots, dim3(nworks), dim3(64), st, works, nworks, nzlists, slots);
}
void launch_make_slots(hipStream_t st, const ScanWork *works, uint32_t nworks, const EncScan *script, const NzList *nzlists, SlotRec *slots, uint32_t *slot_work, uint32_t *list_slots,
                       uint32_t *tok_slots) {
    if (!nworks) return;
    CSH_LAUNCH(k_make_slots, dim3(nworks), dim3(64), st, works, nworks, script, nzlists, slots, slot_work, list_slots, tok_slots);
}

void launch_reset_works(hipStream_t st, ScanWork *work, int nwork) { if (nwork) CSH_LAUNCH(k_reset_works, dim3((nwork + 255) / 256), dim3(256), st, work, nwork); }

}
```

caesium-clt_amd/csrc/k_pixel.hip:

```cpp
#include <cmath>
#include <utility>

#include "kernels.h"

namespace csh {

static constexpr uint8_t kZ2N[64] = {0,  1,  8,  16, 9,  2,  3,  10, 17, 24, 32, 25, 18, 11, 4,  5,  12, 19, 26, 33, 40, 48,
                                     41, 34, 27, 20, 13, 6,  7,  14, 21, 28, 35, 42, 49, 56, 57, 50, 43, 36, 29, 22, 15, 23,
                                     30, 37, 44, 51, 58, 59, 52, 45, 38, 31, 39, 46, 53, 60, 61, 54, 47, 55, 62, 63};
template <int I>
__device__ __forceinline__ static int half_of(const uint4 &v) {
    uint32_t w = (I / 2 == 0) ? v.x : (I / 2 == 1) ? v.y : (I / 2 == 2) ? v.z : v.w;
    return (I & 1) ? (int(w) >> 16) : (int(w << 16) >> 16);
}
using Oct = std::integer_sequence<int, 0, 1, 2, 3, 4, 5, 6, 7>;
#ifndef CSH_EMUL
typedef uint32_t nt_u32x4 __attribute__((ext_vector_type(4)));
__device__ __forceinline__ static void nt_store16(void *p, const uint4 &v) { nt_u32x4 x; x.x = v.x; x.y = v.y; x.z = v.z; x.w = v.w; __builtin_nontemporal_store(x, reinterpret_cast<nt_u32x4 *>(p)); }
__device__ __forceinline__ static uint4 nt_load16(const void *p) { const nt_u32x4 x = __builtin_nontemporal_load(reinterpret_cast<const nt_u32x4 *>(p)); uint4 v; v.x = x.x; v.y = x.y; v.z = x.z; v.w = x.w; return v; }
#else
__device__ __forceinline__ static void nt_store16(void *p, const uint4 &v) { *reinterpret_cast<uint4 *>(p) = v; }
__device__ __forceinline__ static uint4 nt_load16(const void *p) { return *reinterpret_cast<const uint4 *>(p); }
#endif


#define FIX_0_298 2446
#define FIX_0_390 3196
#define FIX_0_541 4433
#define FIX_0_765 6270
#define FIX_0_899 7373
#define FIX_1_175 9633
#define FIX_1_501 12299
#define FIX_1_847 15137
#define FIX_1_961 16069
#define FIX_2_053 16819
#define FIX_2_562 20995
#define FIX_3_072 25172
#define MUL(a, c) __mul24((a), (c))
#define MAD(a, c, b) (__mul24((a), (c)) + (b))


template <int SH>
__device__ __forceinline__ static void idct1d(int &x0, int &x1, int &x2, int &x3, int &x4, int &x5, int &x6, int &x7) {
    const int R = 1 << (SH - 1);
    const int z1 = MUL(x2 + x6, FIX_0_541), tmp2 = MAD(x6, -FIX_1_847, z1), tmp3 = MAD(x2, FIX_0_765, z1);
    const int tmp0 = ((x0 + x4) << 13) + R, tmp1 = ((x0 - x4) << 13) + R;
    const int t10 = tmp0 + tmp3, t13 = tmp0 - tmp3, t11 = tmp1 + tmp2, t12 = tmp1 - tmp2;
    int a0 = x7, a1 = x5, a2 = x3, a3 = x1;
    const int y1 = a0 + a3, y2 = a1 + a2;
    int y3 = a0 + a2, y4 = a1 + a3;
    const int y5 = MUL(y3 + y4, FIX_1_175);
    y3 = MAD(y3, -FIX_1_961, y5); y4 = MAD(y4, -FIX_0_390, y5);
    const int p1 = MUL(y1, -FIX_0_899), p2 = MUL(y2, -FIX_2_562);
    a0 = MAD(a0, FIX_0_298, p1) + y3; a1 = MAD(a1, FIX_2_053, p2) + y4; a2 = MAD(a2, FIX_3_072, p2) + y3; a3 = MAD(a3, FIX_1_501, p1) + y4;
    x0 = (t10 + a3) >> SH; x7 = (t10 - a3) >> SH;
    x1 = (t11 + a2) >> SH; x6 = (t11 - a2) >> SH;
// ... 28 lines not shown
    return __builtin_amdgcn_perm(hi, lo, 0x05040100u);
#endif
}
__device__ __forceinline__ static uint32_t float_bits(float f) { uint32_t u; __builtin_memcpy(&u, &f, 4); return u; }

template <int J, int... I>
__device__ __forceinline__ static void dequant_octet(int x[64], const uint4 &v, const DevQuant &q, std::integer_sequence<int, I...>) {
    ((x[kZ2N[8 * J + I]] = MUL(half_of<I>(v), int(q.q[8 * J + I]))), ...);
}
template <int... J>
__device__ __forceinline__ static void load_dequant(const int16_t *__restrict__ blk, const DevQuant &q, int x[64], std::integer_sequence<int, J...>) {
    const uint4 v[8] = {nt_load16(blk + CSH_OCT_STRIDE * J)...};
    (dequant_octet<J>(x, v[J], q, Oct()), ...);
}
template <bool CENTRED = false>
__device__ __forceinline__ static void load_idct(const int16_t *__restrict__ blk, const DevQuant &q, int x[64]) {
    load_dequant(blk, q, x, Oct());
    CSH_SCHED_FENCE();
    CSH_UNROLL
    for (int c = 0; c < 8; c++) idct1d<11>(x[c], x[8 + c], x[16 + c], x[24 + c], x[32 + c], x[40 + c], x[48 + c], x[56 + c]);
    CSH_SCHED_FENCE();
    CSH_UNROLL
    for (int r = 0; r < 8; r++) {
        idct1d<18>(x[8 * r], x[8 * r + 1], x[8 * r + 2], x[8 * r + 3], x[8 * r + 4], x[8 * r + 5], x[8 * r + 6], x[8 * r + 7]);
        CSH_UNROLL
        for (int c = 0; c < 8; c++) {
            if (CENTRED) { const int v = x[8 * r + c]; x[8 * r + c] = v < -128 ? -128 : (v > 127 ? 127 : v); }
            else { const int v = x[8 * r + c] + 128; x[8 * r + c] = v < 0 ? 0 : (v > 255 ? 255 : v); }
        }
    }
    CSH_SCHED_FENCE();
}

__device__ __forceinline__ static void replicate_edges(int x[64], int vc, int vr) {
    CSH_UNROLL
    for (int c = 1; c < 8; c++) {
        const bool keep = c < vc;
        CSH_UNROLL
        for (int r = 0; r < 8; r++) x[8 * r + c] = keep ? x[8 * r + c] : x[8 * r + c - 1];
    }
    CSH_UNROLL
    for (int r = 1; r < 8; r++) {
        const bool keep = r < vr;
        CSH_UNROLL
        for (int c = 0; c < 8; c++) x[8 * r + c] = keep ? x[8 * r + c] : x[8 * (r - 1) + c];
    }
}

template <int K>
__device__ __forceinline__ static uint32_t quant_one(const int x[64], const DevQuant &q) {
    return float_bits(__builtin_fmaf(float(x[kZ2N[K]]), q.rcp[K], 12582912.0f));
}
template <int J>
__device__ __forceinline__ static void quant_store_octet(const int x[64], const DevQuant &q, int16_t *__restrict__ blk) {
    uint4 v;
    v.x = pack_halves(quant_one<8 * J + 0>(x, q), quant_one<8 * J + 1>(x, q));
    v.y = pack_halves(quant_one<8 * J + 2>(x, q), quant_one<8 * J + 3>(x, q));
    v.z = pack_halves(quant_one<8 * J + 4>(x, q), quant_one<8 * J + 5>(x, q));
    v.w = pack_halves(quant_one<8 * J + 6>(x, q), quant_one<8 * J + 7>(x, q));
    nt_store16(blk + CSH_OCT_STRIDE * J, v);
}
template <int... J>
__device__ __forceinline__ static void quant_store_all(const int x[64], const DevQuant &q, int16_t *__restrict__ blk, std::integer_sequence<int, J...>) {
    ((quant_store_octet<J>(x, q, blk), CSH_SCHED_FENCE()), ...);
}
template <int J>
__device__ __forceinline__ static void raw_store_octet(const int x[64], int16_t *__restrict__ raw) {
    uint4 v;
    v.x = pack_halves(uint32_t(x[kZ2N[8 * J + 0]]), uint32_t(x[kZ2N[8 * J + 1]]));
    v.y = pack_halves(uint32_t(x[kZ2N[8 * J + 2]]), uint32_t(x[kZ2N[8 * J + 3]]));
    v.z = pack_halves(uint32_t(x[kZ2N[8 * J + 4]]), uint32_t(x[kZ2N[8 * J + 5]]));
    v.w = pack_halves(uint32_t(x[kZ2N[8 * J + 6]]), uint32_t(x[kZ2N[8 * J + 7]]));
    *reinterpret_cast<uint4 *>(raw + CSH_RAW_OCT * J) = v;
}
template <int... J>
__device__ __forceinline__ static void raw_store_all(const int x[64], int16_t *__restrict__ raw, std::integer_sequence<int, J...>) {
    (raw_store_octet<J>(x, raw), ...);
}
#ifdef CSH_EMUL
#define CSH_RAW_VIA_LDS 0
#else
#define CSH_RAW_VIA_LDS 1
#endif
template <int J>
__device__ __forceinline__ static void raw_put_octet(const int x[64], int16_t (*tr)[256], int tid) {
    uint4 v;
    v.x = pack_halves(uint32_t(x[kZ2N[8 * J + 0]]), uint32_t(x[kZ2N[8 * J + 1]]));
    v.y = pack_halves(uint32_t(x[kZ2N[8 * J + 2]]), uint32_t(x[kZ2N[8 * J + 3]]));
    v.z = pack_halves(uint32_t(x[kZ2N[8 * J + 4]]), uint32_t(x[kZ2N[8 * J + 5]]));
    v.w = pack_halves(uint32_t(x[kZ2N[8 * J + 6]]), uint32_t(x[kZ2N[8 * J + 7]]));
    const int l = tid & 63;
    *reinterpret_cast<uint4 *>(&tr[l][(tid & ~63) + 8 * (J ^ (l & 7))]) = v;
}
template <int... J>
__device__ __forceinline__ static void raw_put_all(const int x[64], int16_t (*tr)[256], int tid, std::integer_sequence<int, J...>) {
    (raw_put_octet<J>(x, tr, tid), ...);
}
__device__ __forceinline__ static void raw_copy_out(int16_t *__restrict__ tile_raw, bool has_raw, int16_t (*tr)[256], int tid) {
#if CSH_RAW_VIA_LDS
    const uint64_t mask = __ballot(has_raw);
    if (!mask) return;
    __builtin_amdgcn_fence(__ATOMIC_ACQ_REL, "wavefront");
    __builtin_amdgcn_wave_barrier();
    const int l = tid & 63;
    CSH_UNROLL
    for (int j = 0; j < 8; j++) {
        const int src = 8 * j + (l >> 3);
        if ((mask >> src) & 1ull) {
            const uint4 v = *reinterpret_cast<const uint4 *>(&tr[src][(tid & ~63) + 8 * ((l & 7) ^ (src & 7))]);
            nt_store16(tile_raw + src * 64 + (l & 7) * CSH_RAW_OCT, v);
        }
    }
#else
    (void)tile_raw; (void)has_raw; (void)tr; (void)tid;
#endif
}
#define CSH_DERING_LDS int16_t (*dr_col)[256]
// ... 75 lines not shown
#ifdef CSH_EMUL
    o0 = dot2(P, KE0P, dot2(Q, KE0Q, R0)); o4 = dot2(P, KE4P, dot2(Q, KE4Q, R4));
    o2 = dot2(P, KE2P, dot2(Q, KE2Q, R)); o6 = dot2(P, KE6P, dot2(Q, KE6Q, R));
    o7 = dot2(M, PK(kO7[3], kO7[2]), dot2(N, PK(kO7[1], kO7[0]), R));
    o5 = dot2(M, PK(kO5[3], kO5[2]), dot2(N, PK(kO5[1], kO5[0]), R));
    o3 = dot2(M, PK(kO3[3], kO3[2]), dot2(N, PK(kO3[1], kO3[0]), R));
    o1 = dot2(M, PK(kO1[3], kO1[2]), dot2(N, PK(kO1[1], kO1[0]), R));
#else
    asm("v_dot2_i32_i16 %0, %5, %8, %11\n\tv_dot2_i32_i16 %1, %5, %10, %12\n\tv_dot2_i32_i16 %2, %5, %14, %7\n\tv_dot2_i32_i16 %3, %5, %16, %7\n\t"
        "v_dot2_i32_i16 %0, %4, %6, %0\n\tv_dot2_i32_i16 %1, %4, %9, %1\n\tv_dot2_i32_i16 %2, %4, %13, %2\n\tv_dot2_i32_i16 %3, %4, %15, %3\n\ts_nop 2"
        : "=&v"(o0), "=&v"(o4), "=&v"(o2), "=&v"(o6)
        : "v"(P), "v"(Q), "s"(KE0P), "v"(R), "s"(KE0Q), "s"(KE4P), "s"(KE4Q), "v"(R0), "v"(R4), "s"(KE2P), "s"(KE2Q), "s"(KE6P), "s"(KE6Q));
    asm("v_dot2_i32_i16 %0, %5, %8, %6\n\tv_dot2_i32_i16 %1, %5, %10, %6\n\tv_dot2_i32_i16 %2, %5, %12, %6\n\tv_dot2_i32_i16 %3, %5, %14, %6\n\t"
        "v_dot2_i32_i16 %0, %4, %7, %0\n\tv_dot2_i32_i16 %1, %4, %9, %1\n\tv_dot2_i32_i16 %2, %4, %11, %2\n\tv_dot2_i32_i16 %3, %4, %13, %3\n\ts_nop 2"
        : "=&v"(o7), "=&v"(o5), "=&v"(o3), "=&v"(o1)
        : "v"(M), "v"(N), "v"(R), "s"(PK(kO7[3], kO7[2])), "s"(PK(kO7[1], kO7[0])), "s"(PK(kO5[3], kO5[2])), "s"(PK(kO5[1], kO5[0])),
          "s"(PK(kO3[3], kO3[2])), "s"(PK(kO3[1], kO3[0])), "s"(PK(kO1[3], kO1[2])), "s"(PK(kO1[1], kO1[0])));
#endif
    if (!FIRST) { o0 >>= 2; o4 >>= 2; }
    o2 >>= SH; o6 >>= SH; o7 >>= SH; o5 >>= SH; o3 >>= SH; o1 >>= SH;
}
template <bool CENTRED>
__device__ __forceinline__ static void dering_block_pk(uint32_t pr[8][4], int dc_quant, CSH_DERING_LDS) {
    uint32_t m = pr[0][0];
    CSH_UNROLL
    for (int i = 1; i < 32; i++) m = pk_max(m, pr[i >> 2][i & 3]);
    const int top = CENTRED ? 127 : 255, off = CENTRED ? 0 : 128;
    const bool any = int(int16_t(m)) >= top || int(int16_t(m >> 16)) >= top;
#ifndef CSH_EMUL
    if (!__ballot(any)) return;
#endif
    if (!any) return;
    int x[64];
    CSH_UNROLL
    for (int r = 0; r < 8; r++) {
        const uint32_t A = pr[r][0], B = pr[r][1], C = pr[r][2], D = pr[r][3];
        x[8 * r + 0] = int(int16_t(A)) - off; x[8 * r + 1] = int(int16_t(A >> 16)) - off; x[8 * r + 2] = int(int16_t(C)) - off; x[8 * r + 3] = int(int16_t(C >> 16)) - off;
        x[8 * r + 4] = int(int16_t(D >> 16)) - off; x[8 * r + 5] = int(int16_t(D)) - off; x[8 * r + 6] = int(int16_t(B >> 16)) - off; x[8 * r + 7] = int(int16_t(B)) - off;
    }
    int cnt = 0, sum = 0;
    CSH_UNROLL
    for (int i = 0; i < 64; i++) { sum += x[i]; cnt += x[i] >= 127 ? 1 : 0; }
    if (cnt == 64) return;
    int16_t *col = &dr_col[0][threadIdx.x];
    CSH_UNROLL
    for (int i = 0; i < 64; i++) col[i * 256] = int16_t(x[i]);
    dering_walk(col, dc_quant, cnt, sum);
    CSH_UNROLL
    for (int r = 0; r < 8; r++) {
        auto at = [&](int c) { return uint32_t(int(col[(8 * r + c) * 256]) + off); };
        pr[r][0] = pack_halves(at(0), at(1)); pr[r][1] = pack_halves(at(7), at(6)); pr[r][2] = pack_halves(at(2), at(3)); pr[r][3] = pack_halves(at(5), at(4));
    }
}
template <bool DERING, bool CENTRED>
__device__ __forceinline__ static void fdct_quant_store_pk(uint32_t pr[8][4], const DevQuant &q, int16_t *__restrict__ blk, int16_t *__restrict__ raw, CSH_DERING_LDS) {
    CSH_SCHED_FENCE();
    if (DERING) { dering_block_pk<CENTRED>(pr, int(q.q[0]), dr_col); CSH_SCHED_FENCE(); }
    int x[64];
    int R = 1 << 10, Z = 0;
    CSH_PIN(R); CSH_PIN(Z);
    CSH_UNROLL
    for (int r = 0; r < 8; r++)
        fdct1d_pk<true>(pr[r][0], pr[r][1], pr[r][2], pr[r][3], R, Z, Z, x[8 * r], x[8 * r + 1], x[8 * r + 2], x[8 * r + 3], x[8 * r + 4], x[8 * r + 5], x[8 * r + 6], x[8 * r + 7]);
    CSH_SCHED_FENCE();
    int R2 = 1 << 14, TWO = 2, RDC = 2 - 32768;
    CSH_PIN(R2); CSH_PIN(TWO); CSH_PIN(RDC);
    CSH_UNROLL
    for (int c = 0; c < 8; c++) {
        const uint32_t A = pack_halves(uint32_t(x[c]), uint32_t(x[8 + c])), B = pack_halves(uint32_t(x[56 + c]), uint32_t(x[48 + c]));
        const uint32_t C = pack_halves(uint32_t(x[16 + c]), uint32_t(x[24 + c])), D = pack_halves(uint32_t(x[40 + c]), uint32_t(x[32 + c]));
        fdct1d_pk<false>(A, B, C, D, R2, (c == 0 && !CENTRED) ? RDC : TWO, TWO, x[c], x[8 + c], x[16 + c], x[24 + c], x[32 + c], x[40 + c], x[48 + c], x[56 + c]);
    }
    CSH_SCHED_FENCE();
    if (raw) {
        if (CSH_RAW_VIA_LDS) raw_put_all(x, dr_col, int(threadIdx.x), Oct()); else raw_store_all(x, raw, Oct());
    }
    quant_store_all(x, q, blk, Oct());
}
__device__ __forceinline__ static void pack_rows(const int x[64], uint32_t pr[8][4]) {
    CSH_UNROLL
    for (int r = 0; r < 8; r++) {
        pr[r][0] = pack_halves(uint32_t(x[8 * r]), uint32_t(x[8 * r + 1])); pr[r][1] = pack_halves(uint32_t(x[8 * r + 7]), uint32_t(x[8 * r + 6]));
        pr[r][2] = pack_halves(uint32_t(x[8 * r + 2]), uint32_t(x[8 * r + 3])); pr[r][3] = pack_halves(uint32_t(x[8 * r + 5]), uint32_t(x[8 * r + 4]));
    }
}
template <bool DERING, bool CENTRED = false>
__device__ __forceinline__ static void fdct_quant_store(int x[64], const DevQuant &q, int16_t *__restrict__ blk, int16_t *__restrict__ raw, CSH_DERING_LDS) {
    uint32_t pr[8][4];
    pack_rows(x, pr);
    fdct_quant_store_pk<DERING, CENTRED>(pr, q, blk, raw, dr_col);
}

template <int J, int... I>
__device__ __forceinline__ static void raw_to_nat(int x[64], const uint4 &v, std::integer_sequence<int, I...>) {
    ((x[kZ2N[8 * J + I]] = half_of<I>(v)), ...);
}
template <int... J>
__device__ __forceinline__ static void requant_block(const int16_t *__restrict__ raw, const DevQuant &q, int16_t *__restrict__ blk, std::integer_sequence<int, J...>) {
    const uint4 v[8] = {*reinterpret_cast<const uint4 *>(raw + CSH_RAW_OCT * J)...};
    int x[64];
    (raw_to_nat<J>(x, v[J], Oct()), ...);
    quant_store_all(x, q, blk, Oct());
}

__device__ __forceinline__ static void store_zero_block(int16_t *__restrict__ blk) {
    uint4 z; z.x = z.y = z.z = z.w = 0;
    CSH_UNROLL
    for (int j = 0; j < 8; j++) *reinterpret_cast<uint4 *>(blk + CSH_OCT_STRIDE * j) = z;
}

template <bool DERING>
__global__ void __launch_bounds__(256) k_xform_direct(const ImgDesc *__restrict__ imgs, const PlaneWork *__restrict__ work, const DevQuant *__restrict__ quant,
                                                       const int16_t *__restrict__ coef_in, int16_t *__restrict__ coef_out, int16_t *__restrict__ dct_raw, uint32_t raw_tile0) {
    CSH_SHARED int16_t s_dr[64][256];
    const PlaneWork w = work[blockIdx.y];
    if (w.mode != 0) return;
    const ImgDesc &im = imgs[w.image];
    const CompGeom gi = im.in[w.comp], go = im.out[w.comp];
    int tile = blockIdx.x * (blockDim.x >> 6) + (threadIdx.x >> 6);
    int lane = threadIdx.x & 63;
    int b = tile * 64 + lane;
    bool has_raw = false;
    do {
        if (b >= go.bw * go.bh) break;
        int by = b / go.bw, bx = b - by * go.bw;
        int16_t *dst = coef_out + coef_index(go.tile_base, b, 0);
        if (by >= go.real_bh || bx >= go.real_bw) { store_zero_block(dst); break; }
        int x[64];
        load_idct<true>(coef_in + coef_index(gi.tile_base, by * gi.bw + bx, 0), quant[CSH_UNIFORM(im.qt_in[w.comp])], x);
        int vc = gi.comp_w - bx * 8, vr = gi.comp_h - by * 8;
        if (vc < 8 || vr < 8) replicate_edges(x, vc, vr);
        fdct_quant_store<DERING, true>(x, quant[CSH_UNIFORM(im.qt_out[w.comp])], dst, dct_raw ? dct_raw + raw_index(go.tile_base - raw_tile0, b) : nullptr, s_dr);
        has_raw = dct_raw != nullptr;
    } while (0);
    if (dct_raw) raw_copy_out(dct_raw + raw_index(go.tile_base - raw_tile0, tile * 64), has_raw, s_dr, int(threadIdx.x));
}

__global__ void __launch_bounds__(256) k_idct_plane(const ImgDesc *__restrict__ imgs, const PlaneWork *__restrict__ work, const DevQuant *__restrict__ quant,
                                                     const int16_t *__restrict__ coef_in, uint8_t *__restrict__ planes) {
    const PlaneWork w = work[blockIdx.y];
    if (w.mode == 0) return;
    const ImgDesc &im = imgs[w.image];
    const CompGeom gi = im.in[w.comp];
    int tile = blockIdx.x * (blockDim.x >> 6) + (threadIdx.x >> 6);
    int lane = threadIdx.x & 63;
    int b = tile * 64 + lane;
    if (b >= gi.bw * gi.bh) return;
    int by = b / gi.bw, bx = b - by * gi.bw;
    if (by >= gi.real_bh || bx >= gi.real_bw) return;
    int x[64];
    load_idct(coef_in + coef_index(gi.tile_base, b, 0), quant[CSH_UNIFORM(im.qt_in[w.comp])], x);
    int vc = gi.comp_w - bx * 8, vr = gi.comp_h - by * 8;
    if (vc < 8 || vr < 8) replicate_edges(x, vc, vr);
    int pitch = gi.real_bw * 8;
    uint8_t *p = planes + im.plane_off[w.comp] + size_t(by * 8) * pitch + bx * 8;
    CSH_UNROLL
    for (int r = 0; r < 8; r++) {
        uint32_t lo = uint32_t(x[8 * r]) | (uint32_t(x[8 * r + 1]) << 8) | (uint32_t(x[8 * r + 2]) << 16) | (uint32_t(x[8 * r + 3]) << 24);
        uint32_t hi = uint32_t(x[8 * r + 4]) | (uint32_t(x[8 * r + 5]) << 8) | (uint32_t(x[8 * r + 6]) << 16) | (uint32_t(x[8 * r + 7]) << 24);
        uint2 v; v.x = lo; v.y = hi;
        *reinterpret_cast<uint2 *>(p + size_t(r) * pitch) = v;
    }
}

struct PlaneView { const uint8_t *p; int pitch, cw, ch; };

__device__ __forceinline__ static int pv(const PlaneView &v, int y, int x) {
    y = y < 0 ? 0 : (y > v.ch - 1 ? v.ch - 1 : y);
    x = x < 0 ? 0 : (x > v.cw - 1 ? v.cw - 1 : x);
    return v.p[size_t(y) * v.pitch + x];
}
__device__ static int up_h2v2(const PlaneView &v, int r, int xx) {
    int cy = r >> 1, cx = xx >> 1;
    if (v.cw <= 2) return pv(v, cy, cx);
    int fy = (r & 1) ? cy + 1 : cy - 1;
    int nb = (xx & 1) ? cx + 1 : cx - 1;
    int cs = 3 * pv(v, cy, cx) + pv(v, fy, cx);
    int cn = 3 * pv(v, cy, nb) + pv(v, fy, nb);
    return (3 * cs + cn + ((xx & 1) ? 7 : 8)) >> 4;
}

__device__ static int up_h2v1(const PlaneView &v, int r, int xx) {
    int cx = xx >> 1;
    if (v.cw <= 2) return pv(v, r, cx);
    int nb = (xx & 1) ? cx + 1 : cx - 1;
    return (3 * pv(v, r, cx) + pv(v, r, nb) + ((xx & 1) ? 2 : 1)) >> 2;
}

// ... 135 lines not shown
    const bool last = 2 * x0 + 8 >= v.pitch;
    Quad420 n[2], f[2];
    {
        const uint32_t *rp = reinterpret_cast<const uint32_t *>(v.p + size_t(cy) * v.pitch + 2 * x0);
        const uint32_t a = rp[-1], b = rp[0], c = rp[1], d = last ? c >> 24 : rp[2];
        n[0] = quad420_fields(a, b, c); n[1] = quad420_fields(b, c, d);
    }
    {
        const uint32_t *rp = reinterpret_cast<const uint32_t *>(v.p + size_t(fy) * v.pitch + 2 * x0);
        const uint32_t a = rp[-1], b = rp[0], c = rp[1], d = last ? c >> 24 : rp[2];
        f[0] = quad420_fields(a, b, c); f[1] = quad420_fields(b, c, d);
    }
    const uint32_t M = 0x00FF00FFu;
    uint32_t res[2];
    CSH_UNROLL
    for (int k = 0; k < 2; k++) {
        const uint32_t E = 3u * n[k].E + f[k].E, O = 3u * n[k].O + f[k].O, L = 3u * n[k].L + f[k].L, R = 3u * n[k].R + f[k].R;
        const uint32_t s = ((3u * E + L + 0x00080008u) >> 4 & M) + ((3u * E + O + 0x00070007u) >> 4 & M) +
                           ((3u * O + E + 0x00080008u) >> 4 & M) + ((3u * O + R + 0x00070007u) >> 4 & M);
        res[k] = ((s + 0x00020002u) >> 2) & M;
    }
    return (res[0] & 0xFFu) | ((res[0] >> 8) & 0xFF00u) | ((res[1] & 0xFFu) << 16) | ((res[1] << 8) & 0xFF000000u);
}
__global__ void __launch_bounds__(256) k_resample_any(const ImgDesc *imgs, const PlaneWork *work, const uint8_t *planes, uint8_t *oplanes) {
    const PlaneWork w = work[blockIdx.y];
    if (w.mode != CSH_MODE_ANY) return;
    const ImgDesc &im = imgs[w.image];
    const CompGeom gi = im.src[w.comp], go = im.out[w.comp];
    const int pitch_o = go.real_bw * 8, rows_o = go.real_bh * 8;
    int q = blockIdx.x * blockDim.x + threadIdx.x;
    if (q >= (pitch_o >> 2) * rows_o) return;
    int y = q / (pitch_o >> 2), x0 = (q - y * (pitch_o >> 2)) * 4;
    PlaneView v;
    v.p = planes + im.splane_off[w.comp]; v.pitch = gi.real_bw * 8; v.cw = gi.comp_w; v.ch = gi.comp_h;
    const int W = im.enc_w, H = im.enc_h, och = go.comp_h;
    const UpDesc u = w.up;
    uint32_t out;
    if (u.cls == CSH_UP_H2V2 && w.dn == CSH_DN_H4V1 && x0 >= 4 && 2 * x0 + 8 <= v.pitch && 4 * x0 + 15 <= W - 1) {
        const int ye = y < och - 1 ? y : och - 1;
        out = resample_quad_420_411(v, ye > H - 1 ? H - 1 : ye, x0);
    } else {
        switch (w.dn) {
        case CSH_DN_FULL: out = resample_any_quad<CSH_DN_FULL>(v, u, W, H, och, y, x0); break;
        case CSH_DN_H2V2: out = resample_any_quad<CSH_DN_H2V2>(v, u, W, H, och, y, x0); break;
        case CSH_DN_H2V1: out = resample_any_quad<CSH_DN_H2V1>(v, u, W, H, och, y, x0); break;
        default: out = resample_any_quad<CSH_DN_H4V1>(v, u, W, H, och, y, x0); break;
        }
    }
    *reinterpret_cast<uint32_t *>(oplanes + im.oplane_off[w.comp] + size_t(y) * pitch_o + x0) = out;
}

template <bool DERING>
__global__ void __launch_bounds__(256) k_plane_fdct(const ImgDesc *__restrict__ imgs, const PlaneWork *__restrict__ work, const DevQuant *__restrict__ quant, const uint8_t *__restrict__ oplanes,
                                                     int16_t *__restrict__ coef_out, int16_t *__restrict__ dct_raw, uint32_t raw_tile0) {
    CSH_SHARED int16_t s_dr[64][256];
    const PlaneWork w = work[blockIdx.y];
    if (w.mode == 0 || w.mode == 10) return;
    const ImgDesc &im = imgs[w.image];
    const CompGeom go = im.out[w.comp];
    int tile = blockIdx.x * (blockDim.x >> 6) + (threadIdx.x >> 6);
    int lane = threadIdx.x & 63;
    int b = tile * 64 + lane;
    bool has_raw = false;
    do {
    if (b >= go.bw * go.bh) break;
    int by = b / go.bw, bx = b - by * go.bw;
    int16_t *dst = coef_out + coef_index(go.tile_base, b, 0);
    if (by >= go.real_bh || bx >= go.real_bw) { store_zero_block(dst); break; }
    const int pitch = go.real_bw * 8;
    const uint8_t *p = oplanes + im.oplane_off[w.comp] + size_t(by * 8) * pitch + bx * 8;
    uint32_t pr[8][4];
    CSH_UNROLL
    for (int r = 0; r < 8; r++) {
        const uint2 v = *reinterpret_cast<const uint2 *>(p + size_t(r) * pitch);
        pr[r][0] = bytes_to_halves<0, 1>(v.x); pr[r][2] = bytes_to_halves<2, 3>(v.x); pr[r][1] = bytes_to_halves<3, 2>(v.y); pr[r][3] = bytes_to_halves<1, 0>(v.y);
    }
    fdct_quant_store_pk<DERING, false>(pr, quant[CSH_UNIFORM(im.qt_out[w.comp])], dst, dct_raw ? dct_raw + raw_index(go.tile_base - raw_tile0, b) : nullptr, s_dr);
    has_raw = dct_raw != nullptr;
    } while (0);
    if (dct_raw) raw_copy_out(dct_raw + raw_index(go.tile_base - raw_tile0, tile * 64), has_raw, s_dr, int(threadIdx.x));
}

struct Row16 { uint32_t a, b, c, d; };
__device__ __forceinline__ static Row16 load_row16(const uint8_t *p) {
    Row16 r;
#ifdef CSH_EMUL
    __builtin_memcpy(&r, p, 16);
#else
    typedef uint32_t u32x4_a4 __attribute__((ext_vector_type(4), aligned(4)));
    const u32x4_a4 v = *reinterpret_cast<const u32x4_a4 *>(p);
    r.a = v.x; r.b = v.y; r.c = v.z; r.d = v.w;
#endif
    return r;
}
template <bool DERING>
__global__ void __launch_bounds__(256) k_resample_fdct_420(const ImgDesc *__restrict__ imgs, const PlaneWork *__restrict__ work, const DevQuant *__restrict__ quant, const uint8_t *__restrict__ planes,
                                                            int16_t *__restrict__ coef_out, int16_t *__restrict__ dct_raw, uint32_t raw_tile0) {
    CSH_SHARED int16_t s_dr[64][256];
    const PlaneWork w = work[blockIdx.y];
    if (w.mode != 10) return;
    const ImgDesc &im = imgs[w.image];
    const CompGeom gi = im.src[w.comp], go = im.out[w.comp];
    int tile = blockIdx.x * (blockDim.x >> 6) + (threadIdx.x >> 6);
    int lane = threadIdx.x & 63;
    int b = tile * 64 + lane;
    bool has_raw = false;
    do {
    if (b >= go.bw * go.bh) break;
    int by = b / go.bw, bx = b - by * go.bw;
    int16_t *dst = coef_out + coef_index(go.tile_base, b, 0);
    if (by >= go.real_bh || bx >= go.real_bw) { store_zero_block(dst); break; }
    const int pitch = gi.real_bw * 8, rows_alloc = gi.real_bh * 8;
    const uint8_t *pl = planes + im.splane_off[w.comp];
    const int x0 = bx * 8, y0 = by * 8, W = im.enc_w, H = im.enc_h, och = go.comp_h;
    const bool first = bx == 0, last = x0 + 12 > pitch, hodd = (H & 1) != 0;
    const int kt = ((W - 1) >> 1) - x0;
    uint32_t mA[2], mB[2], mC[2], mD[2];
    const bool wodd = (W & 1) != 0;
    CSH_UNROLL
    for (int q = 0; q < 2; q++) {
        auto even_gone = [&](int k) { return k > kt ? 0xFFFFu : 0u; };
        auto odd_gone = [&](int k) { return (k > kt || (wodd && k == kt)) ? 0xFFFFu : 0u; };
        mA[q] = even_gone(4 * q) | (even_gone(4 * q + 2) << 16);
        mB[q] = odd_gone(4 * q) | (odd_gone(4 * q + 2) << 16);
        mC[q] = even_gone(4 * q + 1) | (even_gone(4 * q + 3) << 16);
        mD[q] = odd_gone(4 * q + 1) | (odd_gone(4 * q + 3) << 16);
    }
    Row16 rows[10];
    CSH_UNROLL
    for (int j = 0; j < 10; j++) {
        int yy = y0 - 1 + j;
        if (hodd && yy == och) yy = och - 2;
        yy = yy < 0 ? 0 : (yy > rows_alloc - 1 ? rows_alloc - 1 : yy);
        rows[j] = load_row16(pl + size_t(yy) * pitch + x0 - 4);
    }
    const bool patch = kt < 8 && ((mA[0] | mB[0] | mC[0] | mD[0] | mA[1] | mB[1] | mC[1] | mD[1]) != 0u);
#ifdef CSH_EMUL
    const bool any_patch = patch;
#else
    const bool any_patch = __ballot(patch) != 0ull;
#endif
    uint32_t pr[8][4];
    Quad420 win[3][2];
    auto row_fields = [&](int j, Quad420 out[2]) {
        const uint32_t bq = rows[j].b, cq = rows[j].c;
        const uint32_t aq = first ? bq << 24 : rows[j].a;
        const uint32_t dq = last ? cq >> 24 : rows[j].d;
        out[0] = quad420_fields(aq, bq, cq);
        out[1] = quad420_fields(bq, cq, dq);
    };
    row_fields(0, win[0]);
    row_fields(1, win[1]);
    CSH_UNROLL
    for (int r = 0; r < 8; r++) {
        Quad420 *p = win[r % 3], *c = win[(r + 1) % 3], *n = win[(r + 2) % 3];
        row_fields(r + 2, n);
        Sums420 s[2] = {quad420_sums(p[0], c[0], n[0]), quad420_sums(p[1], c[1], n[1])};
        if (any_patch && patch) {
            const int odd_col = kt & 1;
            const Sums420 &sq = (kt >> 2) ? s[1] : s[0];
            const uint32_t sqA = (kt >> 2) ? s[1].A : s[0].A, sqB = (kt >> 2) ? s[1].B : s[0].B, sqC = (kt >> 2) ? s[1].C : s[0].C, sqD = (kt >> 2) ? s[1].D : s[0].D;
            (void)sq;
            uint32_t sl = wodd ? (odd_col ? sqC : sqA) : (odd_col ? sqD : sqB);
            sl = (kt & 2) ? sl >> 16 : sl & 0xFFFFu;
            sl |= sl << 16;
            CSH_UNROLL
            for (int qq = 0; qq < 2; qq++) {
                s[qq].A = (s[qq].A & ~mA[qq]) | (sl & mA[qq]);
                s[qq].B = (s[qq].B & ~mB[qq]) | (sl & mB[qq]);
                s[qq].C = (s[qq].C & ~mC[qq]) | (sl & mC[qq]);
                s[qq].D = (s[qq].D & ~mD[qq]) | (sl & mD[qq]);
            }
        }
        uint32_t e0, o0, e1, o1;
        quad420_finish(s[0], e0, o0);
        quad420_finish(s[1], e1, o1);
        pr[r][0] = pack_halves(e0, o0); pr[r][2] = pack_hi_halves(e0, o0); pr[r][1] = pack_hi_halves(o1, e1); pr[r][3] = pack_halves(o1, e1);
    }
    const int ylast = och - 1 - y0;
    if (ylast < 7) {
        CSH_UNROLL
        for (int r = 1; r < 8; r++)
            if (r > ylast) {
                CSH_UNROLL
                for (int cc = 0; cc < 4; cc++) pr[r][cc] = pr[r - 1][cc];
            }
    }
    fdct_quant_store_pk<DERING, false>(pr, quant[CSH_UNIFORM(im.qt_out[w.comp])], dst, dct_raw ? dct_raw + raw_index(go.tile_base - raw_tile0, b) : nullptr, s_dr);
    has_raw = dct_raw != nullptr;
    } while (0);
    if (dct_raw) raw_copy_out(dct_raw + raw_index(go.tile_base - raw_tile0, tile * 64), has_raw, s_dr, int(threadIdx.x));
}

__global__ void __launch_bounds__(256) k_requant(const ImgDesc *__restrict__ imgs, const PlaneWork *__restrict__ work, const DevQuant *__restrict__ quant, const int16_t *__restrict__ dct_raw, uint32_t raw_tile0,
                                                  int16_t *__restrict__ coef_out) {
    const PlaneWork w = work[blockIdx.y];
    const ImgDesc &im = imgs[w.image];
    const CompGeom go = im.out[w.comp];
    int tile = blockIdx.x * (blockDim.x >> 6) + (threadIdx.x >> 6);
    int lane = threadIdx.x & 63;
    int b = tile * 64 + lane;
    if (b >= go.bw * go.bh) return;
    int by = b / go.bw, bx = b - by * go.bw;
    if (by >= go.real_bh || bx >= go.real_bw) return;
    requant_block(dct_raw + raw_index(go.tile_base - raw_tile0, b), quant[CSH_UNIFORM(im.qt_out[w.comp])], coef_out + coef_index(go.tile_base, b, 0), Oct());
}

__global__ void k_fix_dummy(const ImgDesc *imgs, int nimg, int16_t *coef_out) {
    int i = blockIdx.y;
    if (i >= nimg) return;
    const ImgDesc &im = imgs[i];
    int t = blockIdx.x * blockDim.x + threadIdx.x;
    for (int c = 0; c < im.ncomp; c++) {
        const CompGeom &g = im.out[c];
        int ndummy_cols = g.bw - g.real_bw, ndummy_rows = g.bh - g.real_bh;
        int n_right = ndummy_cols * g.real_bh, n_bottom = ndummy_rows * g.bw;
        if (t < n_right) {
            int by = t / ndummy_cols, bx = g.real_bw + t % ndummy_cols;
            coef_out[coef_index(g.tile_base, by * g.bw + bx, 0)] = coef_out[coef_index(g.tile_base, by * g.bw + g.real_bw - 1, 0)];
        } else if (t - n_right < n_bottom) {
            int u = t - n_right;
            int by = g.real_bh + u / g.bw, bx = u % g.bw;
            int sx = (bx / g.h) * g.h + g.h - 1;
            if (sx > g.real_bw - 1) sx = g.real_bw - 1;
            coef_out[coef_index(g.tile_base, by * g.bw + bx, 0)] = coef_out[coef_index(g.tile_base, (g.real_bh - 1) * g.bw + sx, 0)];
        }
    }
}

static dim3 tile_grid(int max_tiles, int nwork) { return dim3((max_tiles + 3) / 4, nwork); }

void launch_xform_direct(hipStream_t st, const ImgDesc *imgs, const PlaneWork *work, int nwork, int max_tiles, const DevQuant *quant,
                         const int16_t *coef_in, int16_t *coef_out, int16_t *dct_raw, uint32_t raw_tile0, bool dering) {
    if (!nwork) return;
    if (dering) CSH_LAUNCH(k_xform_direct<true>, tile_grid(max_tiles, nwork), dim3(256), st, imgs, work, quant, coef_in, coef_out, dct_raw, raw_tile0);
    else CSH_LAUNCH(k_xform_direct<false>, tile_grid(max_tiles, nwork), dim3(256), st, imgs, work, quant, coef_in, coef_out, dct_raw, raw_tile0);
}
void launch_idct_plane(hipStream_t st, const ImgDesc *imgs, const PlaneWork *work, int nwork, int max_tiles, const DevQuant *quant,
                       const int16_t *coef_in, uint8_t *planes) {
    if (nwork) CSH_LAUNCH(k_idct_plane, tile_grid(max_tiles, nwork), dim3(256), st, imgs, work, quant, coef_in, planes);
}
void launch_resample_plane(hipStream_t st, const ImgDesc *imgs, const PlaneWork *work, int nwork, uint32_t max_quads, const uint8_t *planes, uint8_t *oplanes) {
    if (nwork && max_quads) CSH_LAUNCH(k_resample_plane, dim3((max_quads + 255) / 256, nwork), dim3(256), st, imgs, work, planes, oplanes);
}
void launch_resample_any(hipStream_t st, const ImgDesc *imgs, const PlaneWork *work, int nwork, uint32_t max_quads, const uint8_t *planes, uint8_t *oplanes) {
    if (nwork && max_quads) CSH_LAUNCH(k_resample_any, dim3((max_quads + 255) / 256, nwork), dim3(256), st, imgs, work, planes, oplanes);
}
void launch_plane_fdct(hipStream_t st, const ImgDesc *imgs, const PlaneWork *work, int nwork, int max_tiles, const DevQuant *quant,
                       const uint8_t *oplanes, int16_t *coef_out, int16_t *dct_raw, uint32_t raw_tile0, bool dering) {
    if (!nwork) return;
    if (dering) CSH_LAUNCH(k_plane_fdct<true>, tile_grid(max_tiles, nwork), dim3(256), st, imgs, work, quant, oplanes, coef_out, dct_raw, raw_tile0);
    else CSH_LAUNCH(k_plane_fdct<false>, tile_grid(max_tiles, nwork), dim3(256), st, imgs, work, quant, oplanes, coef_out, dct_raw, raw_tile0);
}
void launch_resample_fdct_420(hipStream_t st, const ImgDesc *imgs, const PlaneWork *work, int nwork, int max_tiles, const DevQuant *quant,
                              const uint8_t *planes, int16_t *coef_out, int16_t *dct_raw, uint32_t raw_tile0, bool dering) {
    if (!nwork) return;
    if (dering) CSH_LAUNCH(k_resample_fdct_420<true>, tile_grid(max_tiles, nwork), dim3(256), st, imgs, work, quant, planes, coef_out, dct_raw, raw_tile0);
    else CSH_LAUNCH(k_resample_fdct_420<false>, tile_grid(max_tiles, nwork), dim3(256), st, imgs, work, quant, planes, coef_out, dct_raw, raw_tile0);
}
void launch_requant(hipStream_t st, const ImgDesc *imgs, const PlaneWork *work, int nwork, int max_tiles, const DevQuant *quant, const int16_t *dct_raw,
                    uint32_t raw_tile0, int16_t *coef_out) {
    if (nwork) CSH_LAUNCH(k_requant, tile_grid(max_tiles, nwork), dim3(256), st, imgs, work, quant, dct_raw, raw_tile0, coef_out);
}
void launch_fix_dummy(hipStream_t st, const ImgDesc *imgs, int nimg, int max_blocks, int16_t *coef_out) {
    if (nimg && max_blocks) CSH_LAUNCH(k_fix_dummy, dim3((max_blocks + 255) / 256, nimg), dim3(256), st, imgs, nimg, coef_out);
}

}
```

caesium-clt_amd/csrc/kernels.h:

```cpp
#pragma once
#include "gpu_rt.h"
#include "types.h"

namespace csh {

__host__ __device__ static inline int coef_off(int k) { return (k >> 3) * CSH_OCT_STRIDE + (k & 7); }
__host__ __device__ static inline size_t coef_index(uint32_t tile_base, int b, int k) {
    return (size_t(tile_base) + size_t(b >> 6)) * CSH_TILE_I16 + size_t((b & 63) * CSH_BLK_STRIDE) + size_t(coef_off(k));
}

#define CSH_RAW_OCT 8
__host__ __device__ static inline size_t raw_index(uint32_t tile_base, int b) { return size_t(tile_base) * CSH_TILE_I16 + size_t(b) * 64; }

__device__ __forceinline__ static int csh_plane_at(const uint8_t *p, int pitch, int cw, int ch, int y, int x) {
    y = y < 0 ? 0 : (y > ch - 1 ? ch - 1 : y);
    x = x < 0 ? 0 : (x > cw - 1 ? cw - 1 : x);
    return p[size_t(y) * pitch + x];
}
__device__ __forceinline__ static int csh_upsample_at(const uint8_t *p, int pitch, int cw, int ch, UpDesc u, int r, int xx) {
    switch (u.cls) {
    case CSH_UP_COPY: return csh_plane_at(p, pitch, cw, ch, r, xx);
    case CSH_UP_H2V1: {
        const int cx = xx >> 1, nb = (xx & 1) ? cx + 1 : cx - 1;
        return (3 * csh_plane_at(p, pitch, cw, ch, r, cx) + csh_plane_at(p, pitch, cw, ch, r, nb) + ((xx & 1) ? 2 : 1)) >> 2;
    }
    case CSH_UP_H1V2: {
        const int cy = r >> 1, fy = (r & 1) ? cy + 1 : cy - 1;
        return (3 * csh_plane_at(p, pitch, cw, ch, cy, xx) + csh_plane_at(p, pitch, cw, ch, fy, xx) + ((r & 1) ? 2 : 1)) >> 2;
    }
    case CSH_UP_H2V2: {
        const int cy = r >> 1, cx = xx >> 1, fy = (r & 1) ? cy + 1 : cy - 1, nb = (xx & 1) ? cx + 1 : cx - 1;
        const int cs = 3 * csh_plane_at(p, pitch, cw, ch, cy, cx) + csh_plane_at(p, pitch, cw, ch, fy, cx);
        const int cn = 3 * csh_plane_at(p, pitch, cw, ch, cy, nb) + csh_plane_at(p, pitch, cw, ch, fy, nb);
        return (3 * cs + cn + ((xx & 1) ? 7 : 8)) >> 4;
    }
    default: return csh_plane_at(p, pitch, cw, ch, r / int(u.vx), xx / int(u.hx));
    }
}

void launch_decode_seq(hipStream_t st, const uint8_t *bits, ImgDesc *imgs, const DecScan *scans, const DevHuffSet *huffs,
                       int16_t *coef, int nimg, const uint32_t *need_seq);

void launch_unstuff_count(hipStream_t st, const uint8_t *raw, const ParScan *ps, int nps, uint32_t nchunks, uint32_t *cnt);
void launch_unstuff_copy(hipStream_t st, const uint8_t *raw, uint8_t *clean, ParScan *ps, int nps, uint32_t nchunks, const uint64_t *off);
struct DenseArgs {
    const uint8_t *clean; const ParScan *pss; const void *huffs; int compact;
    uint64_t *state; uint32_t *nblk; uint64_t *list_out; uint32_t *cnt_out;
    uint16_t *hyp; const uint32_t *scan_pending;
    const uint64_t *blk_off; const ImgDesc *imgs; int16_t *coef; int32_t *dcdiff; uint32_t *need_seq;
    uint32_t *cut_block;
    uint8_t *zero_ptr; uint64_t zero_bytes;
    uint8_t *zero2_ptr; uint64_t zero2_bytes;
};
void launch_dec_dense(hipStream_t st, int mode , int nps, uint32_t max_sub, const DenseArgs &a);
void launch_dec_relax_list(hipStream_t st, const uint8_t *clean, const ParScan *ps, uint32_t total_sub, const void *huffs, int compact, uint64_t *state, uint32_t *nblk,
                           const uint64_t *list_in, const uint32_t *cnt_in, uint64_t *list_out, uint32_t *cnt_out, size_t nstate, uint32_t *claim, uint32_t epoch);
void launch_refine_chains(hipStream_t st, const uint8_t *clean, const ParScan *pss, const ParHuffSet *huffs, const DecScan *scans, const ProgChain *chains,
                          const int *chain_scans, int nchains, const RefineUnit *units, int nunits, uint32_t max_blocks, const ImgDesc *imgs, int16_t *coef,
                          uint32_t *need_seq, uint64_t *hist, uint32_t *posv, uint32_t *prog);
void launch_rebind_slots(hipStream_t st, const ScanWork *works, uint32_t nworks, const NzList *nzlists, SlotRec *slots);
void launch_make_slots(hipStream_t st, const ScanWork *works, uint32_t nworks, const EncScan *script, const NzList *nzlists, SlotRec *slots, uint32_t *slot_work, uint32_t *list_slots,
                       uint32_t *tok_slots);
void launch_decode_prog(hipStream_t st, const uint8_t *clean, const ParScan *pss, const ParHuffSet *huffs, const DecScan *scans, const ProgChain *chains,
                        const int *chain_scans, int nchains, const ImgDesc *imgs, int16_t *coef, uint32_t *need_seq);
void launch_dec_mark_pending(hipStream_t st, const ParScan *ps, uint32_t total_sub, const uint64_t *list_in, const uint32_t *cnt_in, uint32_t *scan_pending);
void launch_dec_chain(hipStream_t st, const ParScan *ps, int nps, uint64_t *state, uint32_t *nblk, const uint16_t *hyp, const uint32_t *scan_pending, uint32_t *need_seq);
void launch_dc_refine(hipStream_t st, const uint8_t *clean, const ParScan *ps, int nps, uint32_t max_blocks, const ImgDesc *imgs, int16_t *coef, const uint32_t *need_seq);
void launch_dc_scatter(hipStream_t st, const ParScan *ps, int nps, uint32_t max_blocks, const ImgDesc *imgs, const uint64_t *dc_off, int16_t *coef,
                       const uint32_t *need_seq, const uint32_t *cut_block);

void launch_xform_direct(hipStream_t st, const ImgDesc *imgs, const PlaneWork *work, int nwork, int max_tiles, const DevQuant *quant,
                         const int16_t *coef_in, int16_t *coef_out, int16_t *dct_raw, uint32_t raw_tile0, bool dering);
void launch_requant(hipStream_t st, const ImgDesc *imgs, const PlaneWork *work, int nwork, int max_tiles, const DevQuant *quant, const int16_t *dct_raw,
                    uint32_t raw_tile0, int16_t *coef_out);
void launch_idct_plane(hipStream_t st, const ImgDesc *imgs, const PlaneWork *work, int nwork, int max_tiles, const DevQuant *quant,
                       const int16_t *coef_in, uint8_t *planes);
void launch_resample_plane(hipStream_t st, const ImgDesc *imgs, const PlaneWork *work, int nwork, uint32_t max_quads, const uint8_t *planes, uint8_t *oplanes);
void launch_plane_fdct(hipStream_t st, const ImgDesc *imgs, const PlaneWork *work, int nwork, int max_tiles, const DevQuant *quant,
                       const uint8_t *oplanes, int16_t *coef_out, int16_t *dct_raw, uint32_t raw_tile0, bool dering);
void launch_resample_fdct_420(hipStream_t st, const ImgDesc *imgs, const PlaneWork *work, int nwork, int max_tiles, const DevQuant *quant,
                              const uint8_t *planes, int16_t *coef_out, int16_t *dct_raw, uint32_t raw_tile0, bool dering);
void launch_resample_any(hipStream_t st, const ImgDesc *imgs, const PlaneWork *work, int nwork, uint32_t max_quads, const uint8_t *planes, uint8_t *oplanes);
void launch_fix_dummy(hipStream_t st, const ImgDesc *imgs, int nimg, int max_blocks, int16_t *coef_out);

bool resize_is_fused(uint32_t max_row_in);
void launch_resize(hipStream_t st, const ImgDesc *imgs, const ResizeWork *work, int nwork, const ResizeTap *taps, const float *weights,
                   uint8_t *planes, uint8_t *rgb, float *tmp, uint32_t max_src_px, uint64_t max_tmp, uint64_t max_dst, uint32_t max_row_in, uint32_t max_out_w, uint32_t max_nh, bool to_planes,
                   bool any_layout = false);

struct EncCtx {
    const ImgDesc *imgs;
    const EncScan *script;
    const ScanWork *work;
    int nwork;
    const EChunk *echunks;
    uint32_t nechunks;
    const TokPlan *plans;
    const uint32_t *slot_work;
    const SlotRec *slots;
    uint32_t slot0, nslots;
    const int16_t *coef;
    uint64_t *sym_bits;
    uint64_t *eob_bits;
    uint8_t *tail;
    uint16_t *eobrun;
    uint32_t *long_runs, *long_cnt;
    uint64_t *corr;
    uint32_t *tokens;
    const TokRegion *regions;
    uint32_t *tok_cursor;
    uint64_t *tok_off;
    uint32_t *chunk_ntok;
    uint16_t *slot_hist;
    uint32_t *slot_raw;
    uint32_t *slot_eobh;
    uint32_t *chunk_bits;
    const uint64_t *chunk_off;
    DevEncTable *tables;
    uint32_t *raw;
    uint64_t raw_words;
    uint32_t *status;
    uint32_t *overflow;
    uint32_t debug;
    uint32_t stats_only;
    const uint8_t *work_active;
    const NzList *nzlists;
    const NzSet *nzsets;
    const NzChunk *nzchunks;
    uint32_t nnzchunks;
    uint32_t *nz_pool;
    uint32_t *nz_cursor;
    uint32_t *nz_chunk_off;
    uint32_t *nz_chunk_cnt;
    uint8_t *nz_blk_cnt;
    uint16_t *nz_blk_off;
    const uint32_t *list_slots;
    uint32_t nlist_slots;
    const uint32_t *tok_slots;
    uint32_t ntok_slots;
};
void launch_tokens(hipStream_t st, const EncCtx &c);
void launch_ac_runs(hipStream_t st, const EncCtx &c);
void launch_gen_tables(hipStream_t st, DevEncTable *tables, int ntables);
void launch_chunk_sizes(hipStream_t st, const EncCtx &c);
void launch_zero_edges(hipStream_t st, const EncCtx &c);
void launch_pack(hipStream_t st, const EncCtx &c);
void launch_nzlist(hipStream_t st, const EncCtx &c);
void launch_list_stats(hipStream_t st, const EncCtx &c);
void launch_list_pack(hipStream_t st, const EncCtx &c);
void launch_reset_works(hipStream_t st, ScanWork *work, int nwork);

#ifndef CSH_TR_WG
#define CSH_TR_WG 256
#endif
#ifndef CSH_TR_RUN
#define CSH_TR_RUN 8
#endif
struct TrellisCtx {
    const ImgDesc *imgs;
    const DevQuant *quant;
    const TrellisWork *work;
    int nwork;
    const TrellisRun *runs;
    uint32_t nruns;
    uint32_t *queue;
    uint32_t nslots;
    const DevEncTable *tables;
    const int16_t *raw;
    uint32_t raw_tile0;
    int16_t *coef;
    uint64_t *dcrec;
    uint64_t *dcbt;
    uint32_t *spill;
    uint32_t max_rows;
    const uint8_t *blk_cnt;
    uint32_t *perm;
    const uint32_t *rows;
    uint32_t nrows;
    uint32_t debug;
    uint32_t *nz_pool;
    const NzList *nzlists;
    const NzSet *nzsets;
    const uint32_t *nz_chunk_off, *nz_chunk_cnt;
    const uint16_t *blk_off;
};
void launch_trellis_sort(hipStream_t st, const TrellisCtx &c);
void launch_trellis_ac(hipStream_t st, const TrellisCtx &c);
void launch_trellis_dc(hipStream_t st, const TrellisCtx &c);
uint32_t trellis_ac_slots();
size_t trellis_spill_words(uint32_t nslots);

void launch_exclusive_scan(hipStream_t st, const uint32_t *in, uint64_t *out, uint64_t n, void *tmp, size_t tmp_bytes);
// ... 37 lines not shown
```

caesium-clt_amd/csrc/pipeline.cpp:

```cpp
#include <algorithm>
#include <atomic>
#include <cmath>
#include <cstdarg>
#include <memory>
#include <thread>

#include "batch.hpp"
#include "../../include/vp8_tables.h"
#include "resize_host.h"

static thread_local char g_err[512];
void csh_set_error(const char *fmt, ...) {
    va_list ap;
    va_start(ap, fmt);
    vsnprintf(g_err, sizeof g_err, fmt, ap);
    va_end(ap);
}
extern "C" const char *csh_last_error(void) { return g_err; }

#ifdef CSH_EMUL
thread_local dim3 threadIdx, blockIdx, blockDim, gridDim;
int csh_emul_reverse = 0;
thread_local int csh_emul_phase = 0;
extern "C" void csh_emul_set_reverse(int r) { csh_emul_reverse = r; }
// ... 169 lines not shown
    if (hipSetDevice(b->device) != hipSuccess) return -1;
    if (b->d_imgs.upload(b->imgs, b->stream) || b->enc.d_hdr.upload(b->enc.hdr_pool, b->stream) || b->enc.d_hdr_off.upload(b->enc.hdr_off, b->stream)) return -1;
    CSH_CHECK(hipStreamSynchronize(b->stream));
    return 0;
}
extern "C" int csh_batch_rerun_encode(csh_batch *b, csh_timing *t) {
    if (!b->have_dct) { csh_set_error("rerun_encode needs a completed csh_batch_run after csh_batch_retain_dct(1)"); return -1; }
    return batch_run(b, t, true);
}

static int batch_run(csh_batch *b, csh_timing *t, bool requant_only) {
    if (t) memset(t, 0, sizeof *t);
    if (!b->nimg) { b->out.ran = true; return 0; }
    if (hipSetDevice(b->device) != hipSuccess) { csh_set_error("hipSetDevice failed"); return CS_ERR_NO_DEVICE; }
    for (int attempt = 0; attempt < 4; attempt++) {
        if (run_once(b, t, requant_only)) return CS_ERR_NO_DEVICE;
        uint32_t ovf[4] = {0, 0, 0, 0};
        if (csh_copy_wait(ovf, b->out.d_overflow.p, sizeof ovf, hipMemcpyDeviceToHost, b->stream) != hipSuccess) { csh_set_error("D2H failed"); return CS_ERR_NO_DEVICE; }
        b->out.h_status.resize(b->nimg);
        if (csh_copy_wait(b->out.h_status.data(), b->out.d_status.p, b->nimg * sizeof(uint32_t), hipMemcpyDeviceToHost, b->stream) != hipSuccess) return CS_ERR_NO_DEVICE;
        bool pool = ovf[0] != 0;
        if (ovf[1]) {
            pool = true; b->enc.tok_scale *= 4;
            layout_token_pool(b);
            if (b->enc.d_regions.upload(b->enc.regions, b->stream) || b->enc.d_nzlists.upload(b->enc.nzlists, b->stream) || hipStreamSynchronize(b->stream) != hipSuccess) return CS_ERR_NO_DEVICE;
        }
        for (uint32_t s : b->out.h_status) if (s == CS_ERR_POOL_OVERFLOW) pool = true;
        if (!pool) break;
        if (attempt == 3) { csh_set_error("device pools overflowed after 3 retries"); return CS_ERR_POOL_OVERFLOW; }
        b->out.raw_bytes_cap *= 4; b->out.out_cap = b->out.raw_bytes_cap;
        b->wp.webp_mb_bytes *= 4;
    }
    b->out.h_img_size.resize(b->nimg);
    b->out.h_img_off.resize(b->nimg + 1);
    if (csh_copy_wait(b->out.h_img_size.data(), b->out.d_img_size.p, b->nimg * sizeof(uint32_t), hipMemcpyDeviceToHost, b->stream) != hipSuccess ||
        csh_copy_wait(b->out.h_img_off.data(), b->out.d_img_off.p, (b->nimg + 1) * sizeof(uint64_t), hipMemcpyDeviceToHost, b->stream) != hipSuccess) {
        csh_set_error("D2H of sizes failed"); return CS_ERR_NO_DEVICE;
    }
    if (t) {
        std::vector<uint32_t> ns(b->nimg);
        if (csh_copy_wait(ns.data(), b->dec.d_need_seq.p, b->nimg * sizeof(uint32_t), hipMemcpyDeviceToHost, b->stream) != hipSuccess) return CS_ERR_NO_DEVICE;
        if (getenv("CSH_TRACE") && b->dec.d_relax_cnt.n) {
            std::vector<uint32_t> rc(b->dec.d_relax_cnt.n);
            if (csh_copy_wait(rc.data(), b->dec.d_relax_cnt.p, rc.size() * sizeof(uint32_t), hipMemcpyDeviceToHost, b->stream) == hipSuccess) {
                fprintf(stderr, "[csh] relax list sizes (of %u sub-sequences):", b->dec.total_sub);
                for (size_t i = 0; i < rc.size() && (i < 16 || rc[i]); i++) fprintf(stderr, " %u", rc[i]);
                fprintf(stderr, "\n");
            }
        }
        for (const ProgChain &pc : b->dec.chains) if (pc.refine && ns[size_t(pc.image)] == 4) t->n_refine_chains++;
        for (uint32_t v : ns) { if (v == 4) { t->n_prog_decoded++; continue; } if (v) t->n_seq_decoded++; if (v == 2 || v == 3) t->n_par_fallback++; if (v == 3) t->n_par_short++; }
        t->n_images = uint32_t(b->nimg);
        t->n_search_extra = b->enc.search ? b->enc.n_gated_runs : 0u;
        for (const Item &it : b->items) if (it.image < 0) t->n_failed++;
        for (int i = 0; i < b->nimg; i++) { t->out_bytes += b->out.h_img_size[i]; t->pixels += uint64_t(b->imgs[i].width) * b->imgs[i].height; }
        t->in_bytes = b->dec.bits_pool.size();
        uint64_t in_tiles = 0;
        for (const ImgDesc &im : b->imgs) for (int c = 0; c < im.ncomp; c++) in_tiles += im.in[c].ntiles;
        t->coef_bytes = in_tiles * CSH_TILE_I16 * 2;
    }
    b->out.ran = true;
    if (!requant_only) b->have_dct = (b->retain_dct || b->tr.trellis) && !b->lossless;
    return 0;
}

static void set_result(CCSResult *r, int code, const std::string &msg) {
    r->success = code == 0;
    r->code = uint32_t(code);
    r->error_message = nullptr;
    if (code) { char *m = (char *)malloc(msg.size() + 1); memcpy(m, msg.c_str(), msg.size() + 1); r->error_message = m; }
}

extern "C" int csh_batch_pixels(csh_batch *b, size_t image, const uint8_t **device_pixels, uint32_t *width, uint32_t *height, uint32_t *channels, const char **message) {
    *device_pixels = nullptr; *width = *height = *channels = 0;
    if (message) *message = "";
    if (!b || !b->out.ran || !b->rgb_out || image >= b->items.size()) { csh_set_error("csh_batch_pixels: not a pixel batch that has run"); if (message) *message = "not a pixel batch that has run"; return CS_ERR_NO_DEVICE; }
    const Item &it = b->items[image];
    if (it.code) { if (message) *message = it.msg.c_str(); return it.code; }
    if (b->out.h_status[it.image]) { if (message) *message = "device reported a malformed stream"; return int(b->out.h_status[it.image]); }
    if (size_t(it.image) < b->pix.rwork.size() && b->pix.rwork[size_t(it.image)].image == it.image) {
        const ResizeWork &rw = b->pix.rwork[size_t(it.image)];
        *device_pixels = b->pix.d_rgb.p + rw.rgb_dst_off; *width = uint32_t(rw.nw); *height = uint32_t(rw.nh); *channels = uint32_t(b->imgs[it.image].ncomp);
        return 0;
    }
    if (message) *message = "image has no pixel output";
    return CS_ERR_NO_DEVICE;
}

extern "C" int csh_batch_fetch(csh_batch *b, CByteArray *outputs, CCSResult *results) {
    if (!b->out.ran) { csh_set_error("csh_batch_fetch before csh_batch_run"); return -1; }
    if (b->rgb_out) { csh_set_error("csh_batch_fetch: a pixel batch has no files (csh_batch_pixels)"); return -1; }
    struct PinnedOut { uint8_t *p = nullptr; size_t cap = 0; ~PinnedOut() { if (p) pinned_cache().put(p, cap); } uint8_t *data() const { return p; } } host;
    if (b->nimg && b->out.h_img_off[b->nimg]) {
        host.p = static_cast<uint8_t *>(pinned_cache().get(b->out.h_img_off[b->nimg], host.cap));
        if (!host.p) { csh_set_error("out of pinned host memory"); return -1; }
        if (csh_copy_wait(host.p, b->out.d_out.p, b->out.h_img_off[b->nimg], hipMemcpyDeviceToHost, b->stream) != hipSuccess) { csh_set_error("D2H of output failed"); return -1; }
    }
    std::atomic<int> failed{0};
    std::atomic<size_t> next{0};
    auto worker = [&]() {
        for (size_t n; (n = next++) < b->items.size();) {
            Item &it = b->items[n];
            outputs[n].data = nullptr; outputs[n].length = 0;
            int code = it.code;
            std::string msg = it.msg;
            if (!code && it.image >= 0 && b->out.h_status[it.image]) { code = int(b->out.h_status[it.image]); msg = "device reported a malformed stream"; }
// ... 38 lines not shown
```

caesium-clt_amd/csrc/types.h:

```cpp
#pragma once
#include <cstdint>

#define CSH_TILE_BLOCKS 64
#define CSH_TILE_I16 4096
#ifndef CSH_BLOCK_MAJOR
#define CSH_BLOCK_MAJOR 0
#endif
#if CSH_BLOCK_MAJOR
#define CSH_OCT_STRIDE 8
#define CSH_BLK_STRIDE 64
#else
#define CSH_OCT_STRIDE 512
#define CSH_BLK_STRIDE 8
#endif
#define CSH_MAX_COMPS 3
#define CSH_MASK_PLANES 6
#define CSH_MASK_TILE (CSH_MASK_PLANES * 64)
#define CSH_MAX_SCANS 20
#define CSH_LIST_MAX 16

namespace csh {

struct CompGeom {
    int h, v;
// ... 44 lines not shown
    int progressive_in;
    CompGeom in[CSH_MAX_COMPS];
    CompGeom out[CSH_MAX_COMPS];
    int qt_in[CSH_MAX_COMPS];
    int qt_out[CSH_MAX_COMPS];
    uint64_t plane_off[CSH_MAX_COMPS];
    uint64_t oplane_off[CSH_MAX_COMPS];
    CompGeom src[CSH_MAX_COMPS];
    uint64_t splane_off[CSH_MAX_COMPS];
    int enc_w, enc_h;
    int first_scan, nscans_in;
    int comp_id[CSH_MAX_COMPS];
    int first_work, nscans_out;
    uint32_t status;
};

#define CSH_SUBSEQ_BYTES 128
struct ParScan {
    uint32_t bits_off, bits_len;
    uint32_t clean_len;
    int huff_set, image, ncomp;
    int nb_mcu;
    int comp_of[10], by_of[10], bx_of[10], dct[10], act[10];
    uint32_t total_blocks;
    uint32_t sub_base;
    uint32_t par_index;
    uint32_t dc_base[10], dc_per_mcu[10], dc_idx[10];
    uint64_t sel;
    uint32_t first_mcu;
    int kind;
    int Ss, Se, Al;
};
enum { CSH_PS_SEQ = 0, CSH_PS_UNSTUFF = 1, CSH_PS_DC_FIRST = 2, CSH_PS_AC_FIRST = 3, CSH_PS_DC_REFINE = 4 };

struct DevQuant {
    uint16_t q[64];
    int32_t div[64];
    float rcp[64];
    float lt[64];
    uint32_t mul[64];
    uint32_t sh[64];
};

enum { CSH_UP_COPY = 0, CSH_UP_H2V2 = 1, CSH_UP_H2V1 = 2, CSH_UP_H1V2 = 3, CSH_UP_REP = 4 };
enum { CSH_DN_FULL = 0, CSH_DN_H2V2 = 1, CSH_DN_H2V1 = 2, CSH_DN_H4V1 = 3 };
struct UpDesc { uint8_t cls, hx, vx, pad; };

#define CSH_MODE_ANY 11
struct PlaneWork {
    int image, comp;
    int mode;
    UpDesc up;
    int dn;
};

#define CSH_RZ_ANY (-2)
struct ResizeWork {
    int image, in_kind;
    UpDesc up[CSH_MAX_COMPS];
    int nw, nh;
    uint64_t rgb_src_off, rgb_dst_off;
    uint64_t tmp_off;
    uint32_t vtap_base, htap_base;
};
struct ResizeTap { int left, n; uint32_t woff; };

struct EncScan {
    int ncomp, comp[CSH_MAX_COMPS];
    int Ss, Se, Ah, Al;
    int dc_tbl[CSH_MAX_COMPS];
    int ac_tbl[CSH_MAX_COMPS];
    int sequential;
    int ntables;
    int dht_id[4];
    int sos_tdta[CSH_MAX_COMPS];
};

struct ScanWork {
    int image, scan;
    uint32_t nunits;
    uint32_t unit_base;
    uint32_t first_chunk;
    uint32_t word_base;
    uint32_t table_base;
    uint32_t ff_bytes;
    uint64_t raw_off;
    uint32_t raw_bytes;
    uint32_t out_off;
    uint32_t hdr_bytes;
    uint32_t no_room;
    uint32_t list;
    uint32_t corr_base;
    uint32_t hist_row0;
    uint32_t ls_base;
};

struct EChunk { uint32_t a; uint16_t comp, kind; uint32_t j; uint32_t plan; uint32_t region; };
struct TokRegion { uint64_t base; uint32_t cap, pad; };
#define CSH_TK_MAXSLOT 12
struct AcSlot { uint32_t unit_base, word_base, first_chunk, table_base, nunits_work; uint8_t Ss, Se, Ah, Al; uint32_t corr_base, pad; };
struct TokPlan {
    uint32_t nslot, nunits;
    int32_t real_bw, bw;
    uint32_t tile_base;
    uint32_t work0;
    uint32_t pad[2];
// ... 55 lines not shown
```

include/caesium_hip.h:

```cpp
#ifndef CAESIUM_HIP_H
#define CAESIUM_HIP_H
#include <stdbool.h>
#include <stddef.h>
#include <stdint.h>
#ifdef __cplusplus
extern "C" {
#endif

enum { CS_TYPE_JPEG = 0, CS_TYPE_PNG = 1, CS_TYPE_GIF = 2, CS_TYPE_WEBP = 3, CS_TYPE_TIFF = 4, CS_TYPE_UNKN = 5 };

enum {
    CS_OK = 0,
    CS_ERR_NO_DEVICE = 10001,
    CS_ERR_UNKNOWN_TYPE = 10200,
    CS_ERR_UNSUPPORTED = 10201,
    CS_ERR_BAD_JPEG = 20100,
    CS_ERR_JPEG_FEATURE = 20101,
    CS_ERR_POOL_OVERFLOW = 20200,
    CS_ERR_BAD_PNG = 30100,
    CS_ERR_BAD_WEBP = 40100,
    CS_ERR_SAME_FORMAT = 10407,
    CS_ERR_TOO_BIG = 10500
};

// ... 13 lines not shown
    bool webp_lossless;
    uint32_t tiff_compression;
    uint32_t tiff_deflate_level;
    uint32_t width;
    uint32_t height;
} CCSParameters;

typedef struct {
    bool success;
    uint32_t code;
    const char *error_message;
} CCSResult;

typedef struct {
    uint8_t *data;
    size_t length;
} CByteArray;

void cs_default_parameters(CCSParameters *p);

CCSResult cs_compress_in_memory(const uint8_t *in, size_t n, const CCSParameters *p, CByteArray *out);
CCSResult cs_compress_to_size_in_memory(const uint8_t *in, size_t n, CCSParameters *p, size_t max_output_size,
                                        bool return_smallest, CByteArray *out);
CCSResult cs_convert_in_memory(const uint8_t *in, size_t n, const CCSParameters *p, uint32_t format, CByteArray *out);
int cs_batch_convert(const CByteArray *inputs, size_t count, const CCSParameters *p, uint32_t format, int device, CByteArray *outputs, CCSResult *results);

int cs_batch_compress(const CByteArray *inputs, size_t count, const CCSParameters *p, int device,
                      CByteArray *outputs, CCSResult *results);
int cs_batch_compress_to_size(const CByteArray *inputs, size_t count, CCSParameters *p, size_t max_output_size, bool return_smallest,
                              int device, CByteArray *outputs, CCSResult *results);

size_t cs_batch_extent(const CByteArray *inputs, size_t count);

void cs_free_bytes(CByteArray *b);
void cs_free_result(CCSResult *r);

typedef struct csh_batch csh_batch;

enum { CSH_NPHASES = 8, CSH_NKERNELS = 36 };
typedef struct {
    float total_ms;
    float phase_ms[CSH_NPHASES];
    float kernel_ms[CSH_NKERNELS];
    uint64_t in_bytes, out_bytes;
    uint64_t pixels;
    uint64_t coef_bytes;
    uint32_t n_images, n_failed;
    uint32_t n_seq_decoded;
    uint32_t n_par_fallback;
    uint32_t n_par_short;
    uint32_t n_prog_decoded;
    uint32_t n_refine_chains;
    uint32_t n_search_extra;
} csh_timing;

int csh_device_count(void);
const char *csh_last_error(void);
void csh_warmup(int device);
void csh_release_cached_memory(void);
const char *csh_kernel_name(int slot);
const char *csh_kernel_name_webp(int slot);
int csh_batch_create(const CByteArray *inputs, size_t count, const CCSParameters *p, int device, csh_batch **out);
int csh_batch_create_webp(const CByteArray *inputs, size_t count, const CCSParameters *p, int device, csh_batch **out);
int csh_batch_create_pixels(const CByteArray *inputs, size_t count, const CCSParameters *p, int device, csh_batch **out);
int csh_batch_pixels(csh_batch *b, size_t image, const uint8_t **device_pixels, uint32_t *width, uint32_t *height, uint32_t *channels, const char **message);
struct csp_pixels_s;
int csh_batch_create_from_pixels(const struct csp_pixels_s *sources, size_t count, const CCSParameters *p, int device, csh_batch **out);
int csh_batch_run(csh_batch *b, csh_timing *t);
int csh_batch_fetch(csh_batch *b, CByteArray *outputs, CCSResult *results);
void csh_batch_destroy(csh_batch *b);

int csh_batch_retain_dct(csh_batch *b, int on);
int csh_batch_set_quality(csh_batch *b, const uint32_t *quality);
int csh_batch_rerun_encode(csh_batch *b, csh_timing *t);

int csh_batch_geometry(csh_batch *b, size_t image, int comp, int which, int *bw, int *bh, int *real_bw, int *real_bh);
int csh_batch_read_coefs(csh_batch *b, size_t image, int comp, int which, int16_t *dst);

typedef struct csp_batch csp_batch;
enum { CSP_NKERNELS = 16 };
typedef struct {
    float total_ms;
    float kernel_ms[CSP_NKERNELS];
    uint64_t in_bytes, out_bytes;
    uint64_t pixels, raw_bytes;
    uint32_t n_images, n_failed, n_trials;
} csp_timing;
const char *csp_kernel_name(int slot);
int csp_batch_create(const CByteArray *inputs, size_t count, const CCSParameters *p, int device, csp_batch **out);
int csp_batch_create_webp(const CByteArray *inputs, size_t count, const CCSParameters *p, int device, csp_batch **out);
typedef struct csp_pixels_s { const uint8_t *device_pixels; uint32_t width, height, channels; } csp_pixels;
int csp_batch_create_pixels(const csp_pixels *sources, size_t count, const CCSParameters *p, int device, csp_batch **out);
int csp_png_to_jpeg(const CByteArray *inputs, size_t count, const CCSParameters *p, int device, CByteArray *outputs, CCSResult *results);
int csp_png_to_lossless_webp(const CByteArray *inputs, size_t count, const CCSParameters *p, int device, CByteArray *outputs, CCSResult *results);
int csp_batch_run(csp_batch *b, csp_timing *t);
int csp_batch_fetch(csp_batch *b, CByteArray *outputs, CCSResult *results);
void csp_batch_destroy(csp_batch *b);
int csp_batch_geometry(csp_batch *b, size_t image, uint32_t *width, uint32_t *height, uint32_t *rowbytes);
int csp_batch_read_rows(csp_batch *b, size_t image, uint8_t *dst);
int csp_batch_read_stream(csp_batch *b, size_t image, int strategy, uint8_t *dst);
int csp_batch_read_scores(csp_batch *b, size_t image, uint64_t *dst, int *have);
int csp_batch_trials(csp_batch *b, size_t image, int *strategies, uint64_t *zlib_bytes, int *ntrials, int *winner);
int csp_batch_chunk_bits(csp_batch *b, size_t image, int trial, uint64_t *dst, size_t cap, size_t *nchunks);

int csl_encode_pixels(const struct csp_pixels_s *sources, size_t count, int device, CByteArray *outputs, CCSResult *results);
int csl_attach_alpha(CByteArray *lossy, const CByteArray *alpha_vp8l, uint32_t width, uint32_t height);
// ... 20 lines not shown
```

Before: 39940.

## Fuse nonzero-list construction into the FDCT/quantize pixel kernels

Builds each plane's nonzero-coefficient block lists inside the forward-DCT/quantize kernels, using the quantized octets still held in registers. This removes the separate k_nzlist pass, and k_nzfilter when no filtering levels remain, which would otherwise re-read all coefficients. The host planner marks eligible nzsets (full-width, non-lossless, non-webp) and uploads a modified chunk table with the build level cleared. The cost is more register pressure and atomics in the pixel kernels, now launched as phased kernels, and more control paths to keep correct.

```diff
diff --git a/caesium-clt_amd/binding.py b/caesium-clt_amd/binding.py
--- a/caesium-clt_amd/binding.py
+++ b/caesium-clt_amd/binding.py
@@ -25,7 +25,7 @@
 
 class Timing(C.Structure):
     _fields_ = [("total_ms", C.c_float), ("phase_ms", C.c_float * NPHASES), ("kernel_ms", C.c_float * NKERNELS), ("in_bytes", C.c_uint64), ("out_bytes", C.c_uint64),
-                ("pixels", C.c_uint64), ("coef_bytes", C.c_uint64), ("n_images", C.c_uint32), ("n_failed", C.c_uint32), ("n_seq_decoded", C.c_uint32), ("n_par_fallback", C.c_uint32), ("n_par_short", C.c_uint32), ("n_prog_decoded", C.c_uint32), ("n_refine_chains", C.c_uint32), ("n_search_extra", C.c_uint32)]
+                ("pixels", C.c_uint64), ("coef_bytes", C.c_uint64), ("n_images", C.c_uint32), ("n_failed", C.c_uint32), ("n_seq_decoded", C.c_uint32), ("n_par_fallback", C.c_uint32), ("n_par_short", C.c_uint32), ("n_prog_decoded", C.c_uint32), ("n_refine_chains", C.c_uint32), ("n_search_extra", C.c_uint32), ("n_fused_lists", C.c_uint32)]
 
 
 class PngTiming(C.Structure):
diff --git a/caesium-clt_amd/csrc/batch.hpp b/caesium-clt_amd/csrc/batch.hpp
--- a/caesium-clt_amd/csrc/batch.hpp
+++ b/caesium-clt_amd/csrc/batch.hpp
@@ -77,7 +77,10 @@
     DevBuf<int16_t> d_dct_raw;
 };
 
-struct Stage { uint32_t work0 = 0, nwork = 0, slot0 = 0, nslots = 0, ech0 = 0, nech = 0, table0 = 0, ntables = 0, plan0 = 0, nplans = 0, nzc0 = 0, nnzc = 0, ls0 = 0, nls = 0, ts0 = 0, nts = 0; };
+struct Stage {
+    uint32_t work0 = 0, nwork = 0, slot0 = 0, nslots = 0, ech0 = 0, nech = 0, table0 = 0, ntables = 0, plan0 = 0, nplans = 0, nzc0 = 0, nnzc = 0, ls0 = 0, nls = 0, ts0 = 0, nts = 0;
+    bool nz_build[2] = {true, true}, nz_filter[2] = {true, true};
+};
 struct SearchImg {
     int cand_work[64]; int ncand;
     int Al_luma = 0, Al_chroma = 0;
@@ -108,6 +111,9 @@
     std::vector<uint32_t> nzset_built;
     std::vector<int> nzset_comp, nzset_image;
     std::vector<NzChunk> nzchunks;
+    std::vector<NzChunk> nzchunks_fused;
+    uint32_t n_fused = 0;
+    uint32_t last_run_fused = 0;
     std::vector<uint32_t> nz_est, nz_worst;
     uint32_t nz_nrec = 0;
     uint64_t nz_cap = 0;
@@ -146,7 +152,7 @@
     DevBuf<DevEncTable> d_tables;
     DevBuf<NzList> d_nzlists;
     DevBuf<NzSet> d_nzsets;
-    DevBuf<NzChunk> d_nzchunks;
+    DevBuf<NzChunk> d_nzchunks, d_nzchunks_fused;
     DevBuf<uint32_t> d_nz_pool, d_nz_cursor, d_nz_chunk_off, d_nz_chunk_cnt, d_list_slots, d_tok_slots;
 };
 
@@ -262,6 +268,7 @@
     bool tr_sort = true;
     int prog_par = -1;
     bool fused_420 = true;
+    bool nz_fused = true;
     static PlanSwitches read();
 };
 
diff --git a/caesium-clt_amd/csrc/batch_plan.cpp b/caesium-clt_amd/csrc/batch_plan.cpp
--- a/caesium-clt_amd/csrc/batch_plan.cpp
+++ b/caesium-clt_amd/csrc/batch_plan.cpp
@@ -215,6 +215,7 @@
     s.profile = penv && *penv ? penv : "mozjpeg";
     s.nz_once = !is("CSH_NZ_ONCE", "0");
     s.tr_sort = !is("CSH_TR_SORT", "0");
+    s.nz_fused = !is("CSH_NZ_FUSED", "0");
     const char *pp = getenv("CSH_PROG_PAR");
     s.prog_par = pp && !strcmp(pp, "0") ? 0 : (pp && !strcmp(pp, "1") ? 1 : -1);
     s.fused_420 = !getenv("CSH_NO_FUSED_420");
@@ -700,7 +701,7 @@
 
 void BatchPlanner::plane_work(ImgDesc &im, const JpegInfo &in, const JpegInfo &o, int img_index, bool resized) {
     for (int c = 0; c < in.ncomp; c++) {
-        PlaneWork w; w.image = img_index; w.comp = c;
+        PlaneWork w; w.image = img_index; w.comp = c; w.nzset = 0xFFFFFFFFu;
         w.up = resized ? up_desc(1, 1, 0) : up_desc(in.hmax / in.comp[c].h, in.vmax / in.comp[c].v, in.comp[c].comp_w);
         w.dn = dn_kind(o.hmax / o.comp[c].h, o.vmax / o.comp[c].v);
         const int in_kind = (w.up.hx == 1 && w.up.vx == 1) ? 0 : (w.up.hx == 2 && w.up.vx == 2) ? 1 : (w.up.hx == 2 && w.up.vx == 1) ? 2 : -1;
@@ -971,6 +972,29 @@
         for (ImgDesc &im : b->imgs) for (int c = 0; c < im.ncomp; c++) im.out[c].tile_base += b->ntiles_in;
     for (size_t i = 0; i < b->enc.plans.size(); i++) b->enc.plans[i].tile_base = b->imgs[size_t(b->enc.plan_image[i])].out[b->enc.plan_comp[i]].tile_base;
     for (size_t i = 0; i < b->enc.nzsets.size(); i++) b->enc.nzsets[i].tile_base = b->imgs[size_t(b->enc.nzset_image[i])].out[b->enc.nzset_comp[i]].tile_base;
+    {
+        b->enc.nzchunks_fused = b->enc.nzchunks;
+        const bool allowed = sw.nz_fused && !b->lossless && !b->webp && !b->rgb_out && !(b->tr.trellis && progressive && !b->tr.nz_once);
+        std::vector<uint8_t> fused(b->enc.nzsets.size(), 0);
+        for (PlaneWork &w : b->pix.pwork) {
+            const size_t at = size_t(w.image) * CSH_MAX_COMPS + size_t(w.comp);
+            const int si = allowed && at < b->enc.nzset_of.size() ? b->enc.nzset_of[at] : -1;
+            if (si < 0) continue;
+            const NzSet &S = b->enc.nzsets[size_t(si)];
+            if (S.real_bw != S.bw || S.list[0] == 0xFFFFFFFFu) continue;
+            w.nzset = uint32_t(si); fused[size_t(si)] = 1; b->enc.n_fused++;
+        }
+        for (NzChunk &ch : b->enc.nzchunks_fused) if (fused[ch.set]) ch.levels &= ~1u;
+        auto flags = [&](Stage &sg) {
+            for (int f = 0; f < 2; f++) {
+                const std::vector<NzChunk> &v = f ? b->enc.nzchunks_fused : b->enc.nzchunks;
+                sg.nz_build[f] = sg.nz_filter[f] = false;
+                for (uint32_t i = sg.nzc0; i < sg.nzc0 + sg.nnzc; i++) { sg.nz_build[f] |= (v[i].levels & 1u) != 0u; sg.nz_filter[f] |= (v[i].levels & ~1u) != 0u; }
+            }
+        };
+        for (Stage &sg : b->enc.stage) flags(sg);
+        flags(b->tr.tstage);
+    }
     for (ParScan &ps : b->dec.pscans)
         for (int m = 0; m < ps.nb_mcu && m < 10; m++) {
             int dcs = ps.dct[m] & 3, acs = 4 + (ps.act[m] & 3);
@@ -1024,7 +1048,7 @@
         b->enc.d_tok_off.alloc(4 * size_t(b->enc.nslots) + 4) || b->enc.d_chunk_ntok.alloc(4 * size_t(b->enc.nslots) + 4) || b->enc.d_slot_hist.alloc(size_t(b->enc.hist_rows) * 256 + 256) ||
         b->enc.d_slot_raw.alloc(size_t(b->enc.nslots) + 1) || b->enc.d_img_list.upload(b->enc.img_list, st) || b->enc.d_img_nlist.upload(b->enc.img_nlist, st) || b->enc.d_scan_cost.alloc(b->enc.swork.size() + 1) || b->enc.d_slot_eobh.alloc(16 * size_t(b->enc.nslots) + 16) || b->enc.d_chunk_bits.alloc(size_t(b->enc.nslots) + 1) || b->enc.d_chunk_off.alloc(size_t(b->enc.nslots) + 2) || b->enc.d_tok_cursor.alloc(b->enc.region_est.size() + 1) || b->enc.d_regions.upload(b->enc.regions, st) ||
         b->enc.d_tables.alloc(b->enc.ntables) || b->enc.d_scan_pad.alloc(b->enc.swork.size() + 1) ||
-        b->enc.d_nzlists.upload(b->enc.nzlists, st) || b->enc.d_nzsets.upload(b->enc.nzsets, st) || b->enc.d_nzchunks.upload(b->enc.nzchunks, st) || b->enc.d_list_slots.alloc(size_t(b->enc.nlist_slots) + 1) || b->enc.d_tok_slots.alloc(size_t(b->enc.ntok_slots) + 1) ||
+        b->enc.d_nzlists.upload(b->enc.nzlists, st) || b->enc.d_nzsets.upload(b->enc.nzsets, st) || b->enc.d_nzchunks.upload(b->enc.nzchunks, st) || (b->enc.n_fused && b->enc.d_nzchunks_fused.upload(b->enc.nzchunks_fused, st)) || b->enc.d_list_slots.alloc(size_t(b->enc.nlist_slots) + 1) || b->enc.d_tok_slots.alloc(size_t(b->enc.ntok_slots) + 1) ||
         b->enc.d_nz_cursor.alloc(b->enc.nzlists.size() + 1) || b->enc.d_nz_chunk_off.alloc(size_t(b->enc.nz_nrec) + 1) || b->enc.d_nz_chunk_cnt.alloc(size_t(b->enc.nz_nrec) + 1) ||
         b->enc.d_scan_raw_off.alloc(b->enc.swork.size() + 2) || b->out.d_img_size.alloc(b->nimg + 1) || b->out.d_img_size_pad.alloc(b->nimg + 1) ||
         b->out.d_img_off.alloc(b->nimg + 2) || b->out.d_status.alloc(b->nimg) || b->out.d_overflow.alloc(4))
diff --git a/caesium-clt_amd/csrc/batch_run.cpp b/caesium-clt_amd/csrc/batch_run.cpp
--- a/caesium-clt_amd/csrc/batch_run.cpp
+++ b/caesium-clt_amd/csrc/batch_run.cpp
@@ -61,6 +61,7 @@
     KernelMarks marks;
     uint64_t raw_chunks = 0;
     bool eobrun_cleared = false;
+    bool fused = false;
     EncCtx c;
     AsmCtx a;
 
@@ -178,12 +179,22 @@
     int pixels() {
         const int nw = b->lossless ? 0 : int(b->pix.pwork.size());
         int16_t *rawp = ((b->retain_dct || b->tr.trellis) && !b->lossless) ? b->pix.d_dct_raw.p : nullptr;
-        launch_xform_direct(st, b->d_imgs.p, b->pix.d_pwork.p, nw, b->max_tiles, b->d_quants.p, b->d_coef.p, b->d_coef.p, rawp, b->ntiles_in, b->tr.dering);
+        NzFuse nzf;
+        memset(&nzf, 0, sizeof nzf);
+        fused = nw && b->enc.n_fused;
+        if (fused) {
+            if (b->enc.d_nz_cursor.zero(st) || b->enc.d_nz_chunk_cnt.zero(st)) return -1;
+            nzf.nzsets = b->enc.d_nzsets.p; nzf.nzlists = b->enc.d_nzlists.p; nzf.nz_pool = b->enc.d_nz_pool.p; nzf.nz_cursor = b->enc.d_nz_cursor.p;
+            nzf.nz_chunk_off = b->enc.d_nz_chunk_off.p; nzf.nz_chunk_cnt = b->enc.d_nz_chunk_cnt.p; nzf.overflow = b->out.d_overflow.p;
+            nzf.blk_cnt = (b->tr.trellis && b->tr.t_sort) ? b->tr.d_tblk_cnt.p : nullptr;
+            nzf.blk_off = (nzf.blk_cnt && b->tr.nz_once) ? b->tr.d_tblk_off.p : nullptr;
+        }
+        launch_xform_direct(st, b->d_imgs.p, b->pix.d_pwork.p, nw, b->max_tiles, b->d_quants.p, b->d_coef.p, b->d_coef.p, rawp, b->ntiles_in, b->tr.dering, nzf);
         MARK(KS_XFORM_DIRECT);
         launch_resample_plane(st, b->d_imgs.p, b->pix.d_pwork.p, nw, b->pix.max_quads, b->pix.d_planes.p, b->pix.d_oplanes.p);
         if (b->pix.any_layout) launch_resample_any(st, b->d_imgs.p, b->pix.d_pwork.p, nw, b->pix.max_quads, b->pix.d_planes.p, b->pix.d_oplanes.p);
-        launch_plane_fdct(st, b->d_imgs.p, b->pix.d_pwork.p, nw, b->max_tiles, b->d_quants.p, b->pix.d_oplanes.p, b->d_coef.p, rawp, b->ntiles_in, b->tr.dering);
-        launch_resample_fdct_420(st, b->d_imgs.p, b->pix.d_pwork.p, nw, b->max_tiles, b->d_quants.p, b->pix.d_planes.p, b->d_coef.p, rawp, b->ntiles_in, b->tr.dering);
+        launch_plane_fdct(st, b->d_imgs.p, b->pix.d_pwork.p, nw, b->max_tiles, b->d_quants.p, b->pix.d_oplanes.p, b->d_coef.p, rawp, b->ntiles_in, b->tr.dering, nzf);
+        launch_resample_fdct_420(st, b->d_imgs.p, b->pix.d_pwork.p, nw, b->max_tiles, b->d_quants.p, b->pix.d_planes.p, b->d_coef.p, rawp, b->ntiles_in, b->tr.dering, nzf);
         MARK(KS_RESAMPLE_FDCT);
         if (!b->lossless) launch_fix_dummy(st, b->d_imgs.p, nimg, b->max_dummy, b->d_coef.p);
         MARK(KS_FIX_DUMMY);
@@ -230,7 +241,7 @@
     int encode_begin() {
         fill_enc_ctx();
         launch_reset_works(st, b->enc.d_swork.p, c.nwork);
-        if (b->enc.d_nz_cursor.zero(st) || b->enc.d_nz_chunk_cnt.zero(st)) return -1;
+        if (!fused && (b->enc.d_nz_cursor.zero(st) || b->enc.d_nz_chunk_cnt.zero(st))) return -1;
         if (b->enc.d_symbits.zero(st) || b->enc.d_eobbits.zero(st) || (!eobrun_cleared && b->enc.d_eobrun.zero(st)) || b->enc.d_tables.zero(st) || b->enc.d_tok_cursor.zero(st) || b->enc.d_slot_eobh.zero(st) || b->enc.d_scan_pad.zero(st)) return -1;
 #ifdef CSH_EMUL
         if (b->enc.d_raw.zero(st)) return -1;
@@ -243,7 +254,8 @@
 
     void set_stage(const Stage &sg) {
         c.echunks = b->enc.d_echunks.p + sg.ech0; c.nechunks = sg.nech; c.slot0 = sg.slot0; c.nslots = sg.nslots;
-        c.nzchunks = b->enc.d_nzchunks.p + sg.nzc0; c.nnzchunks = sg.nnzc;
+        c.nzchunks = (fused ? b->enc.d_nzchunks_fused.p : b->enc.d_nzchunks.p) + sg.nzc0; c.nnzchunks = sg.nnzc;
+        c.nz_build = sg.nz_build[fused ? 1 : 0]; c.nz_filter = sg.nz_filter[fused ? 1 : 0];
         c.list_slots = b->enc.d_list_slots.p + sg.ls0; c.nlist_slots = sg.nls; c.tok_slots = b->enc.d_tok_slots.p + sg.ts0; c.ntok_slots = sg.nts;
     }
 
@@ -390,6 +402,7 @@
 
 int run_once(csh_batch *b, csh_timing *t, bool requant_only) {
     Run r(b, t);
+    b->enc.last_run_fused = 0;
     if (r.pools() || r.marks.start()) return -1;
     const bool from_pixels = requant_only && b->tr.dering;
     if (requant_only && !from_pixels) {
@@ -402,6 +415,7 @@
         if (r.pixels()) return -1;
     }
     if (r.encode_begin()) return -1;
+    b->enc.last_run_fused = r.fused ? b->enc.n_fused : 0u;
     if (b->tr.trellis ? r.trellis() : r.marks.skip_to(KS_NZLIST)) return -1;
     r.fill_asm_ctx();
     if (r.stage(b->enc.stage[0], true, false)) return -1;
diff --git a/caesium-clt_amd/csrc/k_aclist.hip b/caesium-clt_amd/csrc/k_aclist.hip
--- a/caesium-clt_amd/csrc/k_aclist.hip
+++ b/caesium-clt_amd/csrc/k_aclist.hip
@@ -416,8 +416,8 @@
 
 void launch_nzlist(hipStream_t st, const EncCtx &c) {
     if (!c.nnzchunks) return;
-    CSH_LAUNCH_PHASED(k_nzlist, 3, dim3(c.nnzchunks), dim3(2 * CSP_WAVE_THREADS), st, c);
-    CSH_LAUNCH(k_nzfilter, dim3(c.nnzchunks), dim3(CSP_WAVE_THREADS), st, c);
+    if (c.nz_build) CSH_LAUNCH_PHASED(k_nzlist, 3, dim3(c.nnzchunks), dim3(2 * CSP_WAVE_THREADS), st, c);
+    if (c.nz_filter) CSH_LAUNCH(k_nzfilter, dim3(c.nnzchunks), dim3(CSP_WAVE_THREADS), st, c);
 }
 void launch_list_stats(hipStream_t st, const EncCtx &c) { if (c.nlist_slots) CSH_LAUNCH(k_list_stats, dim3((c.nlist_slots + 3) / 4), dim3(4 * CSP_WAVE_THREADS), st, c); }
 void launch_list_pack(hipStream_t st, const EncCtx &c) { if (c.nlist_slots) CSH_LAUNCH(k_list_pack, dim3((c.nlist_slots + 3) / 4), dim3(4 * CSP_WAVE_THREADS), st, c); }
diff --git a/caesium-clt_amd/csrc/k_pixel.hip b/caesium-clt_amd/csrc/k_pixel.hip
--- a/caesium-clt_amd/csrc/k_pixel.hip
+++ b/caesium-clt_amd/csrc/k_pixel.hip
@@ -2,6 +2,9 @@
 #include <utility>
 
 #include "kernels.h"
+#ifndef CSH_EMUL
+#include "wave.h"
+#endif
 
 namespace csh {
 
@@ -136,17 +139,20 @@
     return float_bits(__builtin_fmaf(float(x[kZ2N[K]]), q.rcp[K], 12582912.0f));
 }
 template <int J>
-__device__ __forceinline__ static void quant_store_octet(const int x[64], const DevQuant &q, int16_t *__restrict__ blk) {
-    uint4 v;
+__device__ __forceinline__ static void quant_store_octet(const int x[64], const DevQuant &q, int16_t *__restrict__ blk , uint4 &v) {
     v.x = pack_halves(quant_one<8 * J + 0>(x, q), quant_one<8 * J + 1>(x, q));
     v.y = pack_halves(quant_one<8 * J + 2>(x, q), quant_one<8 * J + 3>(x, q));
     v.z = pack_halves(quant_one<8 * J + 4>(x, q), quant_one<8 * J + 5>(x, q));
     v.w = pack_halves(quant_one<8 * J + 6>(x, q), quant_one<8 * J + 7>(x, q));
-    nt_store16(blk + CSH_OCT_STRIDE * J, v);
+    nt_store16(blk + CSH_OCT_STRIDE * (J & 3), v);
 }
 template <int... J>
-__device__ __forceinline__ static void quant_store_all(const int x[64], const DevQuant &q, int16_t *__restrict__ blk, std::integer_sequence<int, J...>) {
-    ((quant_store_octet<J>(x, q, blk), CSH_SCHED_FENCE()), ...);
+__device__ __forceinline__ static void quant_store_all(const int x[64], const DevQuant &q, int16_t *__restrict__ blk, uint4 lv[8], std::integer_sequence<int, J...>) {
+    int16_t *hi = blk + 4 * CSH_OCT_STRIDE;
+#ifndef CSH_EMUL
+    asm volatile("" : "+v"(hi));
+#endif
+    ((quant_store_octet<J>(x, q, J < 4 ? blk : hi, lv[J]), CSH_SCHED_FENCE()), ...);
 }
 template <int J>
 __device__ __forceinline__ static void raw_store_octet(const int x[64], int16_t *__restrict__ raw) {
@@ -328,8 +334,9 @@
         pr[r][0] = pack_halves(at(0), at(1)); pr[r][1] = pack_halves(at(7), at(6)); pr[r][2] = pack_halves(at(2), at(3)); pr[r][3] = pack_halves(at(5), at(4));
     }
 }
+struct BlkOut { int16_t *coef_out; uint32_t tile_base; int b; int16_t *dct_raw; uint32_t raw_tile_base; };
 template <bool DERING, bool CENTRED>
-__device__ __forceinline__ static void fdct_quant_store_pk(uint32_t pr[8][4], const DevQuant &q, int16_t *__restrict__ blk, int16_t *__restrict__ raw, CSH_DERING_LDS) {
+__device__ __forceinline__ static void fdct_quant_store_pk(uint32_t pr[8][4], const DevQuant &q, const BlkOut &o, uint4 lv[8], CSH_DERING_LDS) {
     CSH_SCHED_FENCE();
     if (DERING) { dering_block_pk<CENTRED>(pr, int(q.q[0]), dr_col); CSH_SCHED_FENCE(); }
     int x[64];
@@ -348,10 +355,12 @@
         fdct1d_pk<false>(A, B, C, D, R2, (c == 0 && !CENTRED) ? RDC : TWO, TWO, x[c], x[8 + c], x[16 + c], x[24 + c], x[32 + c], x[40 + c], x[48 + c], x[56 + c]);
     }
     CSH_SCHED_FENCE();
-    if (raw) {
-        if (CSH_RAW_VIA_LDS) raw_put_all(x, dr_col, int(threadIdx.x), Oct()); else raw_store_all(x, raw, Oct());
-    }
-    quant_store_all(x, q, blk, Oct());
+    int b = o.b;
+    CSH_PIN(b);
+    if (o.dct_raw) {
+        if (CSH_RAW_VIA_LDS) raw_put_all(x, dr_col, int(threadIdx.x), Oct()); else raw_store_all(x, o.dct_raw + raw_index(o.raw_tile_base, b), Oct());
+    }
+    quant_store_all(x, q, o.coef_out + coef_index(o.tile_base, b, 0), lv, Oct());
 }
 __device__ __forceinline__ static void pack_rows(const int x[64], uint32_t pr[8][4]) {
     CSH_UNROLL
@@ -361,10 +370,15 @@
     }
 }
 template <bool DERING, bool CENTRED = false>
-__device__ __forceinline__ static void fdct_quant_store(int x[64], const DevQuant &q, int16_t *__restrict__ blk, int16_t *__restrict__ raw, CSH_DERING_LDS) {
+__device__ __forceinline__ static void fdct_quant_store(int x[64], const DevQuant &q, const BlkOut &o, uint4 lv[8], CSH_DERING_LDS) {
     uint32_t pr[8][4];
     pack_rows(x, pr);
-    fdct_quant_store_pk<DERING, CENTRED>(pr, q, blk, raw, dr_col);
+    fdct_quant_store_pk<DERING, CENTRED>(pr, q, o, lv, dr_col);
+}
+template <bool DERING, bool CENTRED = false>
+__device__ __forceinline__ static void fdct_quant_store(int x[64], const DevQuant &q, int16_t *__restrict__ blk, int16_t *__restrict__ raw, CSH_DERING_LDS) {
+    uint4 lv[8];
+    fdct_quant_store<DERING, CENTRED>(x, q, BlkOut{blk, 0u, 0, raw, 0u}, lv, dr_col);
 }
 
 template <int J, int... I>
@@ -376,7 +390,8 @@
     const uint4 v[8] = {*reinterpret_cast<const uint4 *>(raw + CSH_RAW_OCT * J)...};
     int x[64];
     (raw_to_nat<J>(x, v[J], Oct()), ...);
-    quant_store_all(x, q, blk, Oct());
+    uint4 lv[8];
+    quant_store_all(x, q, blk, lv, Oct());
 }
 
 __device__ __forceinline__ static void store_zero_block(int16_t *__restrict__ blk) {
@@ -385,10 +400,136 @@
     for (int j = 0; j < 8; j++) *reinterpret_cast<uint4 *>(blk + CSH_OCT_STRIDE * j) = z;
 }
 
+#define CSH_NZF_CAP 2040u
+#define CSH_NZF_CTL (4u * CSH_NZF_CAP)
+#define CSH_NZF_PHASES 4
+__device__ __forceinline__ static uint32_t nzf_ones(uint32_t w, uint32_t ones) {
+#ifdef CSH_EMUL
+    (void)ones;
+    return ((w & 0xFFFFu) ? 1u : 0u) | ((w >> 16) ? 0x10000u : 0u);
+#else
+    uint32_t r;
+    asm("v_pk_min_u16 %0, %1, %2" : "=v"(r) : "v"(w), "v"(ones));
+    return r;
+#endif
+}
+__device__ __forceinline__ static uint32_t nzf_count(const uint4 lv[8]) {
+    uint32_t ones = 0x00010001u;
+    CSH_PIN(ones);
+    uint32_t s = 0;
+    CSH_UNROLL
+    for (int j = 0; j < 8; j++) { s += nzf_ones(lv[j].x, ones); s += nzf_ones(lv[j].y, ones); s += nzf_ones(lv[j].z, ones); s += nzf_ones(lv[j].w, ones); }
+    s -= nzf_ones(lv[0].x, ones) & 1u;
+    return (s & 0xFFFFu) + (s >> 16);
+}
+template <int K>
+__device__ __forceinline__ static void nzf_put(uint32_t w, uint32_t kb, uint32_t *dst, uint32_t &o) {
+    const int h = (K & 1) ? (int(w) >> 16) : (int(w << 16) >> 16);
+    const uint32_t a = uint32_t(h < 0 ? -h : h);
+    dst[o] = (kb | uint32_t(K)) | (h < 0 ? 128u : 0u) | (a << 8);
+    o += h != 0 ? 1u : 0u;
+}
+template <int J>
+__device__ __forceinline__ static void nzf_octet(const uint4 &v, uint32_t kb, uint32_t *dst, uint32_t &o) {
+    uint32_t x = v.x, y = v.y, z = v.z, w = v.w;
+    if ((x | y | z | w) == 0u) return;
+    CSH_PIN(x); CSH_PIN(y); CSH_PIN(z); CSH_PIN(w);
+    if (J) nzf_put<8 * J>(x, kb, dst, o);
+    nzf_put<8 * J + 1>(x, kb, dst, o); nzf_put<8 * J + 2>(y, kb, dst, o); nzf_put<8 * J + 3>(y, kb, dst, o); nzf_put<8 * J + 4>(z, kb, dst, o);
+    nzf_put<8 * J + 5>(z, kb, dst, o); nzf_put<8 * J + 6>(w, kb, dst, o); nzf_put<8 * J + 7>(w, kb, dst, o);
+}
+template <int... J>
+__device__ __forceinline__ static void nzf_walk(const uint4 lv[8], uint32_t blk, bool real, uint32_t *dst, uint32_t o, std::integer_sequence<int, J...>) {
+    if (!real) return;
+    const uint32_t kb = blk << 23;
+    ((nzf_octet<J>(lv[J], kb, dst, o), CSH_SCHED_FENCE()), ...);
+    dst[o] = CSH_NZ_END | kb;
+}
+__device__ __forceinline__ static bool nzf_begin(const NzFuse &f, const PlaneWork &w, NzSet &S) {
+    if (!f.nz_pool || w.nzset == 0xFFFFFFFFu) return false;
+    S = f.nzsets[w.nzset];
+    return blockIdx.x * 256u < S.nunits;
+}
+__device__ __forceinline__ static void nzf_counted(const NzSet &S, const uint4 lv[8], uint32_t ns[2], uint32_t *cnt_lds) {
+    const uint32_t u = blockIdx.x * 256u + threadIdx.x;
+    ns[0] = u < S.nunits ? nzf_count(lv) + 1u : 0u;
+#ifdef CSH_EMUL
+    cnt_lds[threadIdx.x] = ns[0];
+#else
+    (void)cnt_lds;
+#endif
+}
+__device__ __forceinline__ static void nzf_phase(int phase, const NzFuse &f, const NzSet &S, const uint4 lv[8], uint32_t ns[2], uint32_t *lds, const uint32_t *cnt_lds) {
+    const uint32_t tid = threadIdx.x, wave = tid >> 6, lane = tid & 63u, u = blockIdx.x * 256u + tid;
+    const bool real = u < S.nunits;
+    if (phase == 1) {
+        uint32_t ex = 0, tot = 0;
+#ifdef CSH_EMUL
+        for (uint32_t i = 0; i < 64; i++) { const uint32_t n = cnt_lds[wave * 64u + i]; if (i < lane) ex += n; tot += n; }
+#else
+        (void)cnt_lds;
+        LV<uint32_t> c; c.v = ns[0];
+        ex = lscan(c, tot).v;
+#endif
+        ns[1] = ex;
+        if (lane == 0) lds[CSH_NZF_CTL + wave] = tot;
+        if (tot <= CSH_NZF_CAP) nzf_walk(lv, tid, real, lds + wave * CSH_NZF_CAP, ex, Oct());
+        return;
+    }
+    if (phase == 2) {
+        if (tid == 0) {
+            const NzList L0 = f.nzlists[S.list[0]];
+            const uint32_t n0 = lds[CSH_NZF_CTL] + lds[CSH_NZF_CTL + 1] + lds[CSH_NZF_CTL + 2] + lds[CSH_NZF_CTL + 3], n0a = (n0 + 3u) & ~3u, rec0 = L0.chunk0 + blockIdx.x;
+            const uint32_t rel = atomicAdd(&f.nz_cursor[S.list[0]], n0a);
+            const bool ok0 = uint64_t(rel) + n0a <= L0.cap;
+            f.nz_chunk_off[rec0] = rel; f.nz_chunk_cnt[rec0] = ok0 ? n0 : 0u;
+            if (!ok0) f.overflow[1] = 1;
+            lds[CSH_NZF_CTL + 4] = ok0 ? rel : 0xFFFFFFFFu;
+        }
+        return;
+    }
+    const uint32_t rel = lds[CSH_NZF_CTL + 4];
+    if (rel == 0xFFFFFFFFu) return;
+    const uint32_t t0 = lds[CSH_NZF_CTL], t1 = lds[CSH_NZF_CTL + 1], t2 = lds[CSH_NZF_CTL + 2], t3 = lds[CSH_NZF_CTL + 3];
+    const uint32_t wbase = uint32_t(CSH_UNIFORM((wave > 0 ? t0 : 0u) + (wave > 1 ? t1 : 0u) + (wave > 2 ? t2 : 0u)));
+    const uint32_t tot = uint32_t(CSH_UNIFORM(wave == 0 ? t0 : wave == 1 ? t1 : wave == 2 ? t2 : t3)), n0 = t0 + t1 + t2 + t3;
+    uint32_t *chunk = f.nz_pool + f.nzlists[S.list[0]].base + rel;
+    if (tot <= CSH_NZF_CAP) {
+        const uint32_t *src = lds + wave * CSH_NZF_CAP;
+        for (uint32_t i = lane; i < tot; i += 64u) chunk[wbase + i] = src[i];
+    } else {
+        nzf_walk(lv, tid, real, chunk + wbase, ns[1], Oct());
+    }
+    if (real && f.blk_cnt && S.cnt_base != 0xFFFFFFFFu) {
+        f.blk_cnt[S.cnt_base + u] = uint8_t(ns[0] - 1u);
+        if (f.blk_off) f.blk_off[S.cnt_base + u] = uint16_t(wbase + ns[1]);
+    }
+    if (wave == 3u && n0 + lane < ((n0 + 3u) & ~3u)) chunk[n0 + lane] = 0u;
+}
+#ifdef CSH_EMUL
+#define CSH_NZF_STATE CSH_SHARED uint32_t s_nzc[256]; CSH_PERSIST(uint4, lv, 8); CSH_PERSIST(uint32_t, ns, 2)
+#define CSH_NZF_LOOP CSH_PHASE_LOOP(CSH_NZF_PHASES)
+#define CSH_NZF_EARLY(x) x
+#define CSH_NZF_LATE(x) ((void)0)
+#define CSH_NZF_FINISH() ((void)0)
+#else
+#define CSH_NZF_STATE uint32_t *const s_nzc = nullptr; uint4 lv[8]; uint32_t ns[2] = {0u, 0u}
+#define CSH_NZF_LOOP for (int phase = 0, once_ = 1; once_; once_ = 0)
+#define CSH_NZF_EARLY(x) ((void)0)
+#define CSH_NZF_LATE(x) x
+#define CSH_NZF_FINISH()                                                                                                                  \
+    do {                                                                                                                                   \
+        if (!fuse) return;                                                                                                                 \
+        CSH_UNROLL                                                                                                                         \
+        for (int ph_ = 1; ph_ < CSH_NZF_PHASES; ph_++) { __syncthreads(); nzf_phase(ph_, nzf, S, lv, ns, reinterpret_cast<uint32_t *>(&s_dr[0][0]), s_nzc); } \
+    } while (0)
+#endif
+
 template <bool DERING>
 __global__ void __launch_bounds__(256) k_xform_direct(const ImgDesc *__restrict__ imgs, const PlaneWork *__restrict__ work, const DevQuant *__restrict__ quant,
-                                                       const int16_t *__restrict__ coef_in, int16_t *__restrict__ coef_out, int16_t *__restrict__ dct_raw, uint32_t raw_tile0) {
+                                                       const int16_t *__restrict__ coef_in, int16_t *__restrict__ coef_out, int16_t *__restrict__ dct_raw, uint32_t raw_tile0, NzFuse nzf) {
     CSH_SHARED int16_t s_dr[64][256];
+    CSH_NZF_STATE;
     const PlaneWork w = work[blockIdx.y];
     if (w.mode != 0) return;
     const ImgDesc &im = imgs[w.image];
@@ -396,20 +537,32 @@
     int tile = blockIdx.x * (blockDim.x >> 6) + (threadIdx.x >> 6);
     int lane = threadIdx.x & 63;
     int b = tile * 64 + lane;
+    NzSet S;
+    bool fuse = false;
+    CSH_NZF_EARLY(fuse = nzf_begin(nzf, w, S));
+    CSH_NZF_LOOP {
+    if (phase) {
+        if (!fuse) break;
+        nzf_phase(phase, nzf, S, lv, ns, reinterpret_cast<uint32_t *>(&s_dr[0][0]), s_nzc);
+        continue;
+    }
     bool has_raw = false;
     do {
         if (b >= go.bw * go.bh) break;
         int by = b / go.bw, bx = b - by * go.bw;
-        int16_t *dst = coef_out + coef_index(go.tile_base, b, 0);
-        if (by >= go.real_bh || bx >= go.real_bw) { store_zero_block(dst); break; }
+        if (by >= go.real_bh || bx >= go.real_bw) { store_zero_block(coef_out + coef_index(go.tile_base, b, 0)); break; }
         int x[64];
         load_idct<true>(coef_in + coef_index(gi.tile_base, by * gi.bw + bx, 0), quant[CSH_UNIFORM(im.qt_in[w.comp])], x);
         int vc = gi.comp_w - bx * 8, vr = gi.comp_h - by * 8;
         if (vc < 8 || vr < 8) replicate_edges(x, vc, vr);
-        fdct_quant_store<DERING, true>(x, quant[CSH_UNIFORM(im.qt_out[w.comp])], dst, dct_raw ? dct_raw + raw_index(go.tile_base - raw_tile0, b) : nullptr, s_dr);
+        fdct_quant_store<DERING, true>(x, quant[CSH_UNIFORM(im.qt_out[w.comp])], BlkOut{coef_out, go.tile_base, b, dct_raw, go.tile_base - raw_tile0}, lv, s_dr);
         has_raw = dct_raw != nullptr;
     } while (0);
     if (dct_raw) raw_copy_out(dct_raw + raw_index(go.tile_base - raw_tile0, tile * 64), has_raw, s_dr, int(threadIdx.x));
+    CSH_NZF_LATE(fuse = nzf_begin(nzf, w, S));
+    if (fuse) nzf_counted(S, lv, ns, s_nzc);
+    }
+    CSH_NZF_FINISH();
 }
 
 __global__ void __launch_bounds__(256) k_idct_plane(const ImgDesc *__restrict__ imgs, const PlaneWork *__restrict__ work, const DevQuant *__restrict__ quant,
@@ -651,8 +804,9 @@
 
 template <bool DERING>
 __global__ void __launch_bounds__(256) k_plane_fdct(const ImgDesc *__restrict__ imgs, const PlaneWork *__restrict__ work, const DevQuant *__restrict__ quant, const uint8_t *__restrict__ oplanes,
-                                                     int16_t *__restrict__ coef_out, int16_t *__restrict__ dct_raw, uint32_t raw_tile0) {
+                                                     int16_t *__restrict__ coef_out, int16_t *__restrict__ dct_raw, uint32_t raw_tile0, NzFuse nzf) {
     CSH_SHARED int16_t s_dr[64][256];
+    CSH_NZF_STATE;
     const PlaneWork w = work[blockIdx.y];
     if (w.mode == 0 || w.mode == 10) return;
     const ImgDesc &im = imgs[w.image];
@@ -660,12 +814,20 @@
     int tile = blockIdx.x * (blockDim.x >> 6) + (threadIdx.x >> 6);
     int lane = threadIdx.x & 63;
     int b = tile * 64 + lane;
+    NzSet S;
+    bool fuse = false;
+    CSH_NZF_EARLY(fuse = nzf_begin(nzf, w, S));
+    CSH_NZF_LOOP {
+    if (phase) {
+        if (!fuse) break;
+        nzf_phase(phase, nzf, S, lv, ns, reinterpret_cast<uint32_t *>(&s_dr[0][0]), s_nzc);
+        continue;
+    }
     bool has_raw = false;
     do {
     if (b >= go.bw * go.bh) break;
     int by = b / go.bw, bx = b - by * go.bw;
-    int16_t *dst = coef_out + coef_index(go.tile_base, b, 0);
-    if (by >= go.real_bh || bx >= go.real_bw) { store_zero_block(dst); break; }
+    if (by >= go.real_bh || bx >= go.real_bw) { store_zero_block(coef_out + coef_index(go.tile_base, b, 0)); break; }
     const int pitch = go.real_bw * 8;
     const uint8_t *p = oplanes + im.oplane_off[w.comp] + size_t(by * 8) * pitch + bx * 8;
     uint32_t pr[8][4];
@@ -674,10 +836,14 @@
         const uint2 v = *reinterpret_cast<const uint2 *>(p + size_t(r) * pitch);
         pr[r][0] = bytes_to_halves<0, 1>(v.x); pr[r][2] = bytes_to_halves<2, 3>(v.x); pr[r][1] = bytes_to_halves<3, 2>(v.y); pr[r][3] = bytes_to_halves<1, 0>(v.y);
     }
-    fdct_quant_store_pk<DERING, false>(pr, quant[CSH_UNIFORM(im.qt_out[w.comp])], dst, dct_raw ? dct_raw + raw_index(go.tile_base - raw_tile0, b) : nullptr, s_dr);
+    fdct_quant_store_pk<DERING, false>(pr, quant[CSH_UNIFORM(im.qt_out[w.comp])], BlkOut{coef_out, go.tile_base, b, dct_raw, go.tile_base - raw_tile0}, lv, s_dr);
     has_raw = dct_raw != nullptr;
     } while (0);
     if (dct_raw) raw_copy_out(dct_raw + raw_index(go.tile_base - raw_tile0, tile * 64), has_raw, s_dr, int(threadIdx.x));
+    CSH_NZF_LATE(fuse = nzf_begin(nzf, w, S));
+    if (fuse) nzf_counted(S, lv, ns, s_nzc);
+    }
+    CSH_NZF_FINISH();
 }
 
 struct Row16 { uint32_t a, b, c, d; };
@@ -694,8 +860,9 @@
 }
 template <bool DERING>
 __global__ void __launch_bounds__(256) k_resample_fdct_420(const ImgDesc *__restrict__ imgs, const PlaneWork *__restrict__ work, const DevQuant *__restrict__ quant, const uint8_t *__restrict__ planes,
-                                                            int16_t *__restrict__ coef_out, int16_t *__restrict__ dct_raw, uint32_t raw_tile0) {
+                                                            int16_t *__restrict__ coef_out, int16_t *__restrict__ dct_raw, uint32_t raw_tile0, NzFuse nzf) {
     CSH_SHARED int16_t s_dr[64][256];
+    CSH_NZF_STATE;
     const PlaneWork w = work[blockIdx.y];
     if (w.mode != 10) return;
     const ImgDesc &im = imgs[w.image];
@@ -703,12 +870,20 @@
     int tile = blockIdx.x * (blockDim.x >> 6) + (threadIdx.x >> 6);
     int lane = threadIdx.x & 63;
     int b = tile * 64 + lane;
+    NzSet S;
+    bool fuse = false;
+    CSH_NZF_EARLY(fuse = nzf_begin(nzf, w, S));
+    CSH_NZF_LOOP {
+    if (phase) {
+        if (!fuse) break;
+        nzf_phase(phase, nzf, S, lv, ns, reinterpret_cast<uint32_t *>(&s_dr[0][0]), s_nzc);
+        continue;
+    }
     bool has_raw = false;
     do {
     if (b >= go.bw * go.bh) break;
     int by = b / go.bw, bx = b - by * go.bw;
-    int16_t *dst = coef_out + coef_index(go.tile_base, b, 0);
-    if (by >= go.real_bh || bx >= go.real_bw) { store_zero_block(dst); break; }
+    if (by >= go.real_bh || bx >= go.real_bw) { store_zero_block(coef_out + coef_index(go.tile_base, b, 0)); break; }
     const int pitch = gi.real_bw * 8, rows_alloc = gi.real_bh * 8;
     const uint8_t *pl = planes + im.splane_off[w.comp];
     const int x0 = bx * 8, y0 = by * 8, W = im.enc_w, H = im.enc_h, och = go.comp_h;
@@ -785,10 +960,14 @@
                 for (int cc = 0; cc < 4; cc++) pr[r][cc] = pr[r - 1][cc];
             }
     }
-    fdct_quant_store_pk<DERING, false>(pr, quant[CSH_UNIFORM(im.qt_out[w.comp])], dst, dct_raw ? dct_raw + raw_index(go.tile_base - raw_tile0, b) : nullptr, s_dr);
+    fdct_quant_store_pk<DERING, false>(pr, quant[CSH_UNIFORM(im.qt_out[w.comp])], BlkOut{coef_out, go.tile_base, b, dct_raw, go.tile_base - raw_tile0}, lv, s_dr);
     has_raw = dct_raw != nullptr;
     } while (0);
     if (dct_raw) raw_copy_out(dct_raw + raw_index(go.tile_base - raw_tile0, tile * 64), has_raw, s_dr, int(threadIdx.x));
+    CSH_NZF_LATE(fuse = nzf_begin(nzf, w, S));
+    if (fuse) nzf_counted(S, lv, ns, s_nzc);
+    }
+    CSH_NZF_FINISH();
 }
 
 __global__ void __launch_bounds__(256) k_requant(const ImgDesc *__restrict__ imgs, const PlaneWork *__restrict__ work, const DevQuant *__restrict__ quant, const int16_t *__restrict__ dct_raw, uint32_t raw_tile0,
@@ -830,10 +1009,10 @@
 static dim3 tile_grid(int max_tiles, int nwork) { return dim3((max_tiles + 3) / 4, nwork); }
 
 void launch_xform_direct(hipStream_t st, const ImgDesc *imgs, const PlaneWork *work, int nwork, int max_tiles, const DevQuant *quant,
-                         const int16_t *coef_in, int16_t *coef_out, int16_t *dct_raw, uint32_t raw_tile0, bool dering) {
+                         const int16_t *coef_in, int16_t *coef_out, int16_t *dct_raw, uint32_t raw_tile0, bool dering, const NzFuse &nzf) {
     if (!nwork) return;
-    if (dering) CSH_LAUNCH(k_xform_direct<true>, tile_grid(max_tiles, nwork), dim3(256), st, imgs, work, quant, coef_in, coef_out, dct_raw, raw_tile0);
-    else CSH_LAUNCH(k_xform_direct<false>, tile_grid(max_tiles, nwork), dim3(256), st, imgs, work, quant, coef_in, coef_out, dct_raw, raw_tile0);
+    if (dering) CSH_LAUNCH_PHASED(k_xform_direct<true>, CSH_NZF_PHASES, tile_grid(max_tiles, nwork), dim3(256), st, imgs, work, quant, coef_in, coef_out, dct_raw, raw_tile0, nzf);
+    else CSH_LAUNCH_PHASED(k_xform_direct<false>, CSH_NZF_PHASES, tile_grid(max_tiles, nwork), dim3(256), st, imgs, work, quant, coef_in, coef_out, dct_raw, raw_tile0, nzf);
 }
 void launch_idct_plane(hipStream_t st, const ImgDesc *imgs, const PlaneWork *work, int nwork, int max_tiles, const DevQuant *quant,
                        const int16_t *coef_in, uint8_t *planes) {
@@ -846,16 +1025,16 @@
     if (nwork && max_quads) CSH_LAUNCH(k_resample_any, dim3((max_quads + 255) / 256, nwork), dim3(256), st, imgs, work, planes, oplanes);
 }
 void launch_plane_fdct(hipStream_t st, const ImgDesc *imgs, const PlaneWork *work, int nwork, int max_tiles, const DevQuant *quant,
-                       const uint8_t *oplanes, int16_t *coef_out, int16_t *dct_raw, uint32_t raw_tile0, bool dering) {
+                       const uint8_t *oplanes, int16_t *coef_out, int16_t *dct_raw, uint32_t raw_tile0, bool dering, const NzFuse &nzf) {
     if (!nwork) return;
-    if (dering) CSH_LAUNCH(k_plane_fdct<true>, tile_grid(max_tiles, nwork), dim3(256), st, imgs, work, quant, oplanes, coef_out, dct_raw, raw_tile0);
-    else CSH_LAUNCH(k_plane_fdct<false>, tile_grid(max_tiles, nwork), dim3(256), st, imgs, work, quant, oplanes, coef_out, dct_raw, raw_tile0);
+    if (dering) CSH_LAUNCH_PHASED(k_plane_fdct<true>, CSH_NZF_PHASES, tile_grid(max_tiles, nwork), dim3(256), st, imgs, work, quant, oplanes, coef_out, dct_raw, raw_tile0, nzf);
+    else CSH_LAUNCH_PHASED(k_plane_fdct<false>, CSH_NZF_PHASES, tile_grid(max_tiles, nwork), dim3(256), st, imgs, work, quant, oplanes, coef_out, dct_raw, raw_tile0, nzf);
 }
 void launch_resample_fdct_420(hipStream_t st, const ImgDesc *imgs, const PlaneWork *work, int nwork, int max_tiles, const DevQuant *quant,
-                              const uint8_t *planes, int16_t *coef_out, int16_t *dct_raw, uint32_t raw_tile0, bool dering) {
+                              const uint8_t *planes, int16_t *coef_out, int16_t *dct_raw, uint32_t raw_tile0, bool dering, const NzFuse &nzf) {
     if (!nwork) return;
-    if (dering) CSH_LAUNCH(k_resample_fdct_420<true>, tile_grid(max_tiles, nwork), dim3(256), st, imgs, work, quant, planes, coef_out, dct_raw, raw_tile0);
-    else CSH_LAUNCH(k_resample_fdct_420<false>, tile_grid(max_tiles, nwork), dim3(256), st, imgs, work, quant, planes, coef_out, dct_raw, raw_tile0);
+    if (dering) CSH_LAUNCH_PHASED(k_resample_fdct_420<true>, CSH_NZF_PHASES, tile_grid(max_tiles, nwork), dim3(256), st, imgs, work, quant, planes, coef_out, dct_raw, raw_tile0, nzf);
+    else CSH_LAUNCH_PHASED(k_resample_fdct_420<false>, CSH_NZF_PHASES, tile_grid(max_tiles, nwork), dim3(256), st, imgs, work, quant, planes, coef_out, dct_raw, raw_tile0, nzf);
 }
 void launch_requant(hipStream_t st, const ImgDesc *imgs, const PlaneWork *work, int nwork, int max_tiles, const DevQuant *quant, const int16_t *dct_raw,
                     uint32_t raw_tile0, int16_t *coef_out) {
diff --git a/caesium-clt_amd/csrc/kernels.h b/caesium-clt_amd/csrc/kernels.h
--- a/caesium-clt_amd/csrc/kernels.h
+++ b/caesium-clt_amd/csrc/kernels.h
@@ -69,17 +69,23 @@
 void launch_dc_scatter(hipStream_t st, const ParScan *ps, int nps, uint32_t max_blocks, const ImgDesc *imgs, const uint64_t *dc_off, int16_t *coef,
                        const uint32_t *need_seq, const uint32_t *cut_block);
 
+struct NzFuse {
+    const NzSet *nzsets; const NzList *nzlists;
+    uint32_t *nz_pool, *nz_cursor, *nz_chunk_off, *nz_chunk_cnt;
+    uint8_t *blk_cnt; uint16_t *blk_off;
+    uint32_t *overflow;
+};
 void launch_xform_direct(hipStream_t st, const ImgDesc *imgs, const PlaneWork *work, int nwork, int max_tiles, const DevQuant *quant,
-                         const int16_t *coef_in, int16_t *coef_out, int16_t *dct_raw, uint32_t raw_tile0, bool dering);
+                         const int16_t *coef_in, int16_t *coef_out, int16_t *dct_raw, uint32_t raw_tile0, bool dering, const NzFuse &nzf);
 void launch_requant(hipStream_t st, const ImgDesc *imgs, const PlaneWork *work, int nwork, int max_tiles, const DevQuant *quant, const int16_t *dct_raw,
                     uint32_t raw_tile0, int16_t *coef_out);
 void launch_idct_plane(hipStream_t st, const ImgDesc *imgs, const PlaneWork *work, int nwork, int max_tiles, const DevQuant *quant,
                        const int16_t *coef_in, uint8_t *planes);
 void launch_resample_plane(hipStream_t st, const ImgDesc *imgs, const PlaneWork *work, int nwork, uint32_t max_quads, const uint8_t *planes, uint8_t *oplanes);
 void launch_plane_fdct(hipStream_t st, const ImgDesc *imgs, const PlaneWork *work, int nwork, int max_tiles, const DevQuant *quant,
-                       const uint8_t *oplanes, int16_t *coef_out, int16_t *dct_raw, uint32_t raw_tile0, bool dering);
+                       const uint8_t *oplanes, int16_t *coef_out, int16_t *dct_raw, uint32_t raw_tile0, bool dering, const NzFuse &nzf);
 void launch_resample_fdct_420(hipStream_t st, const ImgDesc *imgs, const PlaneWork *work, int nwork, int max_tiles, const DevQuant *quant,
-                              const uint8_t *planes, int16_t *coef_out, int16_t *dct_raw, uint32_t raw_tile0, bool dering);
+                              const uint8_t *planes, int16_t *coef_out, int16_t *dct_raw, uint32_t raw_tile0, bool dering, const NzFuse &nzf);
 void launch_resample_any(hipStream_t st, const ImgDesc *imgs, const PlaneWork *work, int nwork, uint32_t max_quads, const uint8_t *planes, uint8_t *oplanes);
 void launch_fix_dummy(hipStream_t st, const ImgDesc *imgs, int nimg, int max_blocks, int16_t *coef_out);
 
@@ -138,6 +144,7 @@
     uint32_t nlist_slots;
     const uint32_t *tok_slots;
     uint32_t ntok_slots;
+    uint32_t nz_build, nz_filter;
 };
 void launch_tokens(hipStream_t st, const EncCtx &c);
 void launch_ac_runs(hipStream_t st, const EncCtx &c);
diff --git a/caesium-clt_amd/csrc/pipeline.cpp b/caesium-clt_amd/csrc/pipeline.cpp
--- a/caesium-clt_amd/csrc/pipeline.cpp
+++ b/caesium-clt_amd/csrc/pipeline.cpp
@@ -245,6 +245,7 @@
         for (uint32_t v : ns) { if (v == 4) { t->n_prog_decoded++; continue; } if (v) t->n_seq_decoded++; if (v == 2 || v == 3) t->n_par_fallback++; if (v == 3) t->n_par_short++; }
         t->n_images = uint32_t(b->nimg);
         t->n_search_extra = b->enc.search ? b->enc.n_gated_runs : 0u;
+        t->n_fused_lists = b->enc.last_run_fused;
         for (const Item &it : b->items) if (it.image < 0) t->n_failed++;
         for (int i = 0; i < b->nimg; i++) { t->out_bytes += b->out.h_img_size[i]; t->pixels += uint64_t(b->imgs[i].width) * b->imgs[i].height; }
         t->in_bytes = b->dec.bits_pool.size();
diff --git a/caesium-clt_amd/csrc/types.h b/caesium-clt_amd/csrc/types.h
--- a/caesium-clt_amd/csrc/types.h
+++ b/caesium-clt_amd/csrc/types.h
@@ -120,6 +120,7 @@
     int mode;
     UpDesc up;
     int dn;
+    uint32_t nzset;
 };
 
 #define CSH_RZ_ANY (-2)
diff --git a/include/caesium_hip.h b/include/caesium_hip.h
--- a/include/caesium_hip.h
+++ b/include/caesium_hip.h
@@ -89,6 +89,7 @@
     uint32_t n_prog_decoded;
     uint32_t n_refine_chains;
     uint32_t n_search_extra;
+    uint32_t n_fused_lists;
 } csh_timing;
 
 int csh_device_count(void);
```

Measured after the change: 41750, median of 6. +4.5%, better.
